# qiaozhijian/LPD-Net-Pytorch

Hardware: AMD Instinct MI355X
Metric: global descriptors/sec (4096-pt clouds) (higher is better)
Workload: dtype f32; 1 GPU; BASELINE configs[1]: LPD-Net (featnet=lpdnet, emb_dims=1024, no T-Nets) eval forward, N=4096, k=20, eval_batch_size=32 clouds/step/GPU; num_points=4096, batches_in_flight=2, parallelism=shard-by-cloud x1 (one process per GPU, no data-path collective)

## Files before the change

### include/lpd_hip.h

```cpp
#ifndef LPD_HIP_H
#define LPD_HIP_H

#include <stdint.h>

#ifdef __cplusplus
extern "C" {
#endif

#define LPD_OK 0
#define LPD_ERR_ARG (-1)
#define LPD_ERR_LAUNCH (-2)
#define LPD_ERR_UNSUPPORTED (-3)

#define LPD_ACT_NONE 0
#define LPD_ACT_RELU 1
#define LPD_ACT_LEAKY 2
#define LPD_ACT_SIGMOID 3

int lpd_version(void);
const char* lpd_last_error(void);
long long lpd_stat_ws_bytes(void);

int lpd_knn(const float* x, int B, int C, int N, int k, int32_t* idx, float* ws, int impl, void* stream);
long long lpd_knn_workspace_floats(int B, int C, int N, int k);
int lpd_knn_pm(const float* x_pm, int ld, int B, int C, int N, int k, int32_t* idx, float* ws, int impl, void* stream);
#define LPD_KNN_PM_PREPARED 256
int lpd_knn_pm_layout(int B, int C, int N, int k, float* ws, float** xx, float** xp, void** xb, float** tiles);

int lpd_lpdnet_front(const float* xyz, int ldx, const float* W1, const float* s1, const float* b1, const float* W2, const float* s2,
                     const float* b2, int act, float slope, float* F0, int B, int N, int k, float* knn_ws, void* stream);

int lpd_gemm(const float* A, const float* B, float* C, int M, int N, int K, int lda, int ldb, int ldc,
             int a_kmajor, int b_kmajor, int batch, long long sA, long long sB, long long sC, int splits,
             float* splitk_ws, const float* bias, const float* scale, const float* shift, int act, float slope,
             int accumulate, long long a_cloud, long long c_cloud, int panel_n, int panel_ld, void* stream);

int lpd_gemm_bf16x3(const float* A, const float* B, float* C, int M, int N, int K, int lda, int ldb, int ldc,
             int a_kmajor, int b_kmajor, int batch, long long sA, long long sB, long long sC, int splits,
             float* splitk_ws, const float* bias, const float* scale, const float* shift, int act, float slope,
             int accumulate, long long a_cloud, long long c_cloud, int panel_n, int panel_ld, void* stream);

int lpd_gemm_bf16x1(const float* A, const float* B, float* C, int M, int N, int K, int lda, int ldb, int ldc,
             int a_kmajor, int b_kmajor, int batch, long long sA, long long sB, long long sC, int splits,
             float* splitk_ws, const float* bias, const float* scale, const float* shift, int act, float slope,
             int accumulate, long long a_cloud, long long c_cloud, int panel_n, int panel_ld, void* stream);

long long lpd_gemm_prep_b_bytes(int N, int K);
int lpd_gemm_prep_b(const float* B, int ldb, int b_kmajor, int N, int K, void* frags, void* stream);
int lpd_gemm_prep_b_batch(const float* B, int ldb, int b_kmajor, int N, int K, int batch, long long sB, void* frags, void* stream);
int lpd_gemm_x3w(const float* A, int lda, const void* frags, float* C, int ldc, int M, int N, int K, const float* bias,
                 const float* scale, const float* shift, int act, float slope, int accumulate,
                 long long a_cloud, long long c_cloud, int panel_n, int panel_ld, int impl, void* stream);

int lpd_gemm_x3w_batched(const void* A, int lda, int a_bf16, const void* frags, long long frag_bytes, int batch_rows, float* C, int ldc, int M,
                         int N, int K, const float* a_scale, const float* a_shift, int a_act, float a_slope, int impl, void* stream);
int lpd_gemm_x3w_bf16a(const void* A16, int lda, const void* frags, float* C, int ldc, int M, int N, int K, int accumulate, int impl, void* stream);
int lpd_gemm_x3w_stats(const float* A, int lda, const void* frags, void* C, int ldc, int c_bf16, int M, int N, int K, const float* bias,
                       double* stat_sum, double* stat_sumsq, int impl, double* stat_ws, void* stream);
int lpd_gemm_x3w_act(const void* A, int lda, const void* frags, float* C, int ldc, int M, int N, int K, const float* bias,
                     const float* a_scale, const float* a_shift, int a_act, float a_slope, void* a_out, int a_ld, int flags, int impl, void* stream);

int lpd_gemm_x3t_applies(int M, int N, int K, int act, long long a_cloud, long long c_cloud, int panel_n);
int lpd_gemm_x3ts(const void* a_hi, long long a_lo, const void* frags, float* C, int M, int N, int K, const float* bias,
                  const float* scale, const float* shift, int act, float slope, long long a_cloud, long long c_cloud, int panel_n,
                  int panel_ld, void* stream);
int lpd_gemm_x3t_rows_applies(int M, int N, int K, int act, long long lda, long long ldc);
int lpd_gemm_x3t_rows(const float* A, long long lda, const void* frags, void* C, long long ldc, int c_bf16, int M, int N, int K, const float* bias,
                      const float* scale, const float* shift, int act, float slope, int batch, long long sA, long long sC,
                      long long frag_bytes, void* stream);

int lpd_gemm_x3t(const float* A, const void* frags, float* C, int M, int N, int K, const float* bias, const float* scale,
                 const float* shift, int act, float slope, long long a_cloud, long long c_cloud, int panel_n, int panel_ld,
                 void* stream);

int lpd_edge_gather_max(const float* P, int ldp, const float* Q, int ldq, const int32_t* idx, float* out, int ldo,
                        const float* scale, const float* shift, int M, int N, int C, int k, int act, float slope,
                        void* stream);

int lpd_edge_gather_max16(const float* P, int ldp, const float* Q, int ldq, const uint16_t* idx16, float* out, int ldo,
                          const float* scale, const float* shift, int M, int N, int C, int k, int act, float slope, long long p_cloud,
                          long long q_cloud, long long o_cloud, int panel_ld, void* stream);
int lpd_edge_gather_max16s(const float* P, int ldp, const float* Q, int ldq, const uint16_t* idx16, void* out_hi, long long o_lo,
                           const float* scale, const float* shift, int M, int N, int C, int k, int act, float slope, long long p_cloud,
                           long long q_cloud, long long o_cloud, int panel_ld, void* stream);

int lpd_pack_idx16(const int32_t* idx, uint16_t* idx16, long long M, int k, void* stream);

int lpd_pack_idx16w(const int32_t* idx, uint16_t* idx16, long long M, int k, int N, void* stream);
int lpd_edge_gather_maxw(const float* P, int ldp, const float* Q, int ldq, const uint16_t* idx16, float* out, int ldo,
                         const float* scale, const float* shift, int M, int N, int C, int k, int act, float slope, long long p_cloud,
                         long long q_cloud, long long o_cloud, int panel_ld, void* stream);

int lpd_edge_mlp(const float* P, int ldp, const float* Q, int ldq, const int32_t* idx, const float* s1,
                 const float* b1, const float* W2, const float* s2, const float* b2, float* out, int ldo, int M,
                 int N, int CM, int CO, int k, int act, float slope, long long out_cloud, int panel_ld, void* stream);
int lpd_edge_mlp_bf16x3(const float* P, int ldp, const float* Q, int ldq, const int32_t* idx, const float* s1,
                 const float* b1, const float* W2, const float* s2, const float* b2, float* out, int ldo, int M,
                 int N, int CM, int CO, int k, int act, float slope, long long out_cloud, int panel_ld, void* stream);
int lpd_edge_mlp_bf16x3s(const float* P, int ldp, const float* Q, int ldq, const int32_t* idx, const float* s1,
                 const float* b1, const float* W2, const float* s2, const float* b2, void* out_hi, long long out_lo, int M,
                 int N, int CM, int CO, int k, int act, float slope, long long out_cloud, int panel_ld, void* stream);
int lpd_edge_mlp_x1_bf16x3s(const float* P, int ldp, const float* Q, int ldq, const int32_t* idx, const float* s1,
                 const float* b1, const float* W2, const float* s2, const float* b2, void* out_hi, void* x1_hi, long long out_lo,
                 int M, int N, int k, int act, float slope, long long out_cloud, int panel_ld, void* stream);

int lpd_linear_smallk(const float* X, int ldx, const float* W, int w_sn, int w_sk, long long w_sb, int rows_per_w,
                      float* Y, int ldy, int M, int N, int K, const float* bias, const float* scale,
                      const float* shift, int act, float slope, void* stream);

int lpd_transpose(const float* in, float* out, int batch, int R, int C, int ldi, int ldo, long long si,
                  long long so, void* stream);

int lpd_softmax_affine(const float* in, float* out, int rows, int ncols, const float* scale, const float* shift,
                       int group_rows, float* colsum, int colsum_ld, float* part, void* stream);

int lpd_vlad_finalize(const float* vraw, const float* act, const float* cw2, float* out, float* ws, float* part, float* aux_asum,
                      float* aux_inv_c, float* aux_inv_g, int B, int N, int F, int KC, int asum_ready, void* stream);

int lpd_colmax(const float* in, int ldi, float* out, int B, int N, int C, void* stream);

int lpd_gating(const float* h, int ldh, const float* Wg, int ldw, const float* bias, const float* scale, const float* shift,
               float* out, int ldo, int B, int D, void* stream);

int lpd_mul(const float* a, const float* b, float* out, long long n, void* stream);

int lpd_metric_loss(const float* q, long long q_sb, const float* pos, long long pos_sb, long long pos_st,
                    const float* neg, long long neg_sb, long long neg_st, const float* other, long long other_sb,
                    int bq, int P, int Ng, int D, float m1, float m2, int use_min, int lazy, int ignore_zero, int quad,
                    float* loss, float* minmax, float* gq, float* gpos, float* gneg, float* gother, void* stream);

int lpd_best_pos_bwd(const float* q, long long q_sb, const float* pos, long long pos_sb, long long pos_st, const float* gmin,
                     const float* gmax, int bq, int P, int D, float* gq, float* gpos, void* stream);

int lpd_retrieval_topk(const float* S, const float* Q, int ldq, const float* D, int ldd, int nq, int ndb, int dim, int k,
                       int32_t* idx, float* dist, float* ws, void* stream);

int lpd_recall_pairs(const float* Q, int ldq, const float* D, int ldd, int dim, const int32_t* q_off, const int32_t* d_off, int rd,
                     int q_rows, int d_rows, const int32_t* pairs, const int32_t* out_off, int npairs, int max_qtiles,
                     const int32_t* truth_off, const int32_t* truth_idx, int k, int32_t* first, uint8_t* one_pct, float* top1_sim,
                     int32_t* topk_idx, int32_t* hist, int32_t* n_eval, int32_t* n_onepct, float* ws, void* stream);

int lpd_hard_negatives(const float* table, long long ldt, const float* Q, long long ldq, const int32_t* cand, int bq, int nc, int dim,
                       int k, int32_t* pos, float* dist, void* stream);

int lpd_f64_to_f32(const double* in, float* out, long long n, void* stream);

int lpd_morton_sort(const float* xyz, float* out, int32_t* perm, int B, int N, void* stream);

int lpd_local_features(const float* xyz, int ldx, const int32_t* idx, int B, int N, int K, const int32_t* cand, int ncand, unsigned sel,
                       int copy_xyz, float* out, int ldo, int32_t* kopt, void* stream);

int lpd_make_submaps(const float* points, int ld, const int32_t* offsets, int B, int N, int normalize, float* out, int32_t* info,
                     float* xform, int32_t* counts, void* stream);

int lpd_sample_items(const int32_t* off, const int32_t* idx, int n_lists, int nnz, int T, const int32_t* lists, int L, const int32_t* extra,
                     int X, int R, int invert, int m, unsigned long long seed, int32_t* out, int32_t* count, void* stream);
int lpd_gather_tuples(const float* table, int T, int N, const int32_t* items, int B, const float* rot, float sigma, float clip,
                      unsigned long long seed, float* out, void* stream);

int lpd_radius_count(const double* qpos, int Q, const double* dpos, int D, const int32_t* seg_off, int S, double r, const int32_t* skip_seg,
                     const int32_t* self_item, int32_t* counts, void* stream);
int lpd_radius_fill(const double* qpos, int Q, const double* dpos, int D, const int32_t* seg_off, int S, double r, const int32_t* skip_seg,
                    const int32_t* self_item, const int32_t* row_off, int32_t* idx, int nnz, void* stream);

#define LPD_CLEAN_CHUNK 1024
typedef struct LpdCleanParams {
    float r_min, r_max, z_lo, z_hi, seed_z_lo, seed_z_hi, tau, min_det, max_slope, clearance;
    int32_t H, min_inliers, refine;
    uint32_t seed_lo, seed_hi;
    int32_t reserved;
} LpdCleanParams;
long long lpd_road_planes_workspace_bytes(int B, int H);
int lpd_road_planes(const float* points, int ld, int rows, const int32_t* offsets, int B, int max_len, const LpdCleanParams* prm,
                    float* plane, int32_t* info, void* ws, void* stream);
int lpd_clean_count(const float* points, int ld, int rows, const int32_t* offsets, int B, int max_len, const LpdCleanParams* prm,
                    const float* plane, const int32_t* info, int32_t* counts, void* stream);
int lpd_clean_fill(const float* points, int ld, int rows, const int32_t* offsets, int B, int max_len, const LpdCleanParams* prm,
                   const float* plane, const int32_t* info, const int32_t* block_off, float* out, int32_t* out_offsets,
                   unsigned char* mask, void* stream);


int lpd_colstats(const float* X, long long ld, long long R, int C, double* sum, double* sumsq, double* stat_ws, void* stream);

int lpd_bn_finalize(const double* sum, const double* sumsq, double count, int C, const float* gamma, const float* beta,
                    float* running_mean, float* running_var, float momentum, float eps, float* scale, float* shift,
                    float* mean, float* invstd, void* stream);

int lpd_affine_act(const float* X, long long ldx, float* Y, long long ldy, long long R, int C, const float* scale,
                   const float* shift, int act, float slope, void* stream);
int lpd_affine_act2(const float* X, long long ldx, float* Y, long long ldy, void* Y16, long long ld16, long long R, int C, const float* scale,
                    const float* shift, int act, float slope, void* stream);

int lpd_bn_act_bwd(const float* dY, long long lddy, const float* X, long long ldx, float* dX, long long lddx, long long R,
                   int C, const float* scale, const float* shift, const float* mean, const float* invstd, int act,
                   float slope, int has_bn, double* dbeta, double* dgamma, double* stat_ws, void* stream);
int lpd_bn_act_bwd_bf16(const void* dY, long long lddy, const void* X, long long ldx, void* dX, long long lddx, long long R, int C,
                        const float* scale, const float* shift, const float* mean, const float* invstd, int act, float slope, int has_bn,
                        double* dbeta, double* dgamma, double* stat_ws, void* stream);

int lpd_edge_build(const float* P, long long ldp, const float* Q, long long ldq, const int32_t* idx, float* U, long long M,
                   int N, int C, int k, double* sum, double* sumsq, double* stat_ws, void* stream);

int lpd_group_max(const float* X, long long ldx, int k, const float* scale, const float* shift, int act, float slope,
                  float* out, long long ldo, uint8_t* arg, long long M, int C, void* stream);
int lpd_group_max_sel(const float* X, long long ldx, int k, const float* scale, const float* shift, int act, float slope,
                      float* out, long long ldo, uint8_t* arg, float* xsel, long long ldsel, long long M, int C, void* stream);

int lpd_group_max_bwd(const float* dOut, long long ldo, const uint8_t* arg, int k, float* dX, long long M, int C,
                      int accumulate, void* stream);

int lpd_edge_bn_bwd(const float* dOut, long long ldo, const uint8_t* arg, const float* dDense, const float* X, float* dX,
                    float* dQ, long long ldq, int k, long long M, int C, const float* scale, const float* shift,
                    const float* mean, const float* invstd, int act, float slope, float inv_ns, double* dbeta, double* dgamma,
                    double* stat_ws, void* stream);
int lpd_edge_bn_bwd_sel(const float* dOut, long long ldo, const uint8_t* arg, const float* X, const float* Xsel, long long ldsel,
                        float* dX, int k, long long M, int C, const float* scale, const float* shift, const float* mean,
                        const float* invstd, int act, float slope, double* dbeta, double* dgamma, double* stat_ws, void* stream);

int lpd_group_sum(const float* dU, int k, float* dQ, long long ldq, long long M, int C, void* stream);

int lpd_scatter_add_rows(const float* dU, const int32_t* idx, float* dP, long long ldp, long long M, int N, int k, int C,
                         void* stream);

int lpd_graph_transpose(const int32_t* idx, long long M, int N, int k, int32_t* rowptr, int32_t* edges, int32_t* ws,
                        void* stream);
int lpd_gather_sum_rows(const float* dU, const int32_t* rowptr, const int32_t* edges, float* dP, long long ldp, long long M,
                        int C, int accumulate, void* stream);

int lpd_dw_smallk(const float* dY, long long lddy, const float* X, long long ldx, long long M, int Co, int Kin, float* dW,
                  void* stream);

int lpd_colmax_arg(const float* in, long long ld, float* out, int32_t* arg, int B, int N, int C, void* stream);

int lpd_colmax_bwd(const float* dOut, const int32_t* arg, float* dIn, long long ld, int B, int N, int C, void* stream);

int lpd_cloud_outer(const float* X, long long ldx, const float* dY, long long ldy, float* dT, int B, int N, int KD, void* stream);

int lpd_softmax_bwd(const float* A, const float* dA, const float* dasum, float* dS, long long rows, int ncols,
                    int rows_per_cloud, void* stream);

int lpd_vlad_finalize_bwd(const float* dOut, const float* v, const float* inv_c, const float* inv_g, const float* asum,
                          const float* cw2, float* dVraw, float* dasum, float* dcw2, int B, int F, int KC, void* stream);


int lpd_edge_split_fwd(const float* P, long long ldp, const float* Q, long long ldq, const int32_t* idx, const float* gamma,
                       float* S, float* usel, uint8_t* arg, long long M, int N, int C, int k, double* sum, double* sumsq,
                       double* stat_ws, void* stream);
int lpd_edge_mlp_train(const float* P, int ldp, const float* Q, int ldq, const int32_t* idx, const float* s1, const float* b1,
                       const float* W2, const float* gamma2, void* Y1e, void* Z, int bf16, int z_bf16, float* zsel, int ldsel, uint8_t* arg2,
                       double* sum, double* sumsq, int M, int N, int k, int act, float slope, double* stat_ws, void* stream);
int lpd_edge_mlp_train_bwd(const void* Z, const uint8_t* arg2, const void* dpre2, const float* W2, const float* scale2, const float* mean2,
                           const float* invstd2, const double* dbeta2, const double* dgamma2, const void* Y1e, const uint8_t* arg1,
                           const float* dx1, int lddx1, const float* beta1, const float* rgamma1, int bf16, int z_bf16, void* G, float* gsum,
                           double* dbeta1, double* dgamma1, int M, int k, int act, float slope, float inv_ns, float* kws, double* stat_ws, void* stream);
int lpd_edge_dense_bwd_apply(const void* G, int bf16, const float* gsum, const float* S, const float* P, long long ldp, const float* Q,
                             long long ldq, const int32_t* rowptr, const int32_t* edges, float* dP, long long lddp, float* dQ, long long lddq,
                             long long M, int C, int k, const float* scale, const float* mean, const float* invstd, const double* dbeta,
                             const double* dgamma, void* stream);
int lpd_edge_split_fwd16_applies(int N, int C, int k);
int lpd_edge_split_fwd16(const float* P, long long ldp, const float* Q, long long ldq, const uint16_t* idx16, const float* gamma, float* S,
                         float* usel, uint8_t* arg, long long M, int N, int C, int k, double* sum, double* sumsq, double* stat_ws, void* stream);

int lpd_edge_split_bwd(const float* dOut, long long ldo, const float* usel, const uint8_t* arg, const float* S, const float* P,
                       long long ldp, const float* Q, long long ldq, const int32_t* rowptr, const int32_t* edges, float* G,
                       float* dP, long long lddp, float* dQ, long long lddq, long long M, int C, int k, const float* scale,
                       const float* shift, const float* mean, const float* invstd, int act, float slope, int half, double* dbeta,
                       double* dgamma, double* stat_ws, void* stream);

int lpd_edge_build_bf16(const float* P, long long ldp, const float* Q, long long ldq, const int32_t* idx, uint16_t* U, long long M,
                        int N, int C, int k, double* sum, double* sumsq, double* stat_ws, void* stream);
int lpd_edge_act_max(const float* U, int k, const float* scale, const float* shift, int act, float slope, float* Y, float* out,
                     long long ldo, uint8_t* arg, long long M, int C, void* stream);
int lpd_edge_act_max_bf16(const uint16_t* U, int k, const float* scale, const float* shift, int act, float slope, uint16_t* Y,
                          float* out, long long ldo, uint8_t* arg, long long M, int C, void* stream);
int lpd_group_sel_stats_bf16(const uint16_t* Z, int k, const float* gamma, float* sel, long long lds, uint8_t* arg, long long M, int C,
                             double* sum, double* sumsq, double* stat_ws, void* stream);
int lpd_edge_bn_bwd_bf16(const float* dOut, long long ldo, const uint8_t* arg, const uint16_t* dDense, const uint16_t* X, uint16_t* dX,
                         float* dQ, long long ldq, int k, long long M, int C, const float* scale, const float* shift,
                         const float* mean, const float* invstd, int act, float slope, float inv_ns, double* dbeta, double* dgamma,
                         double* stat_ws, void* stream);
int lpd_edge_bn_bwd_bf16_sel(const float* dOut, long long ldo, const uint8_t* arg, const uint16_t* X, const float* Xsel, long long ldsel,
                             uint16_t* dX, int k, long long M, int C, const float* scale, const float* shift, const float* mean,
                             const float* invstd, int act, float slope, double* dbeta, double* dgamma, double* stat_ws, void* stream);
int lpd_bn_sel_bwd_reduce(const float* dOut, long long ldo, const float* Xsel, long long ldsel, long long M, int C, const float* scale,
                          const float* shift, const float* mean, const float* invstd, int act, float slope, uint16_t* dpre16,
                          double* dbeta, double* dgamma, double* stat_ws, void* stream);
long long lpd_edge_dw_sel_bf16_ws_bytes(long long E);
int lpd_edge_dw_sel_bf16(const uint16_t* Y, const uint8_t* arg, const uint16_t* dpre16, int k, long long M, const float* W2, long long ldw,
                         const float* scale, const float* mean, const float* invstd, const double* dbeta, const double* dgamma, float* dW2,
                         void* ws, void* stream);
int lpd_gemm_bf16s_bnbwd(const uint16_t* Z, const uint8_t* arg, const uint16_t* dpre16, int k, long long M, const float* W2, int ldw,
                         const float* scale, const float* mean, const float* invstd, const double* dbeta, const double* dgamma, uint16_t* dY,
                         void* stream);
int lpd_bn_sel_bwd_reduce_f32(const float* dOut, long long ldo, const float* Xsel, long long ldsel, long long M, int C, const float* scale,
                              const float* shift, const float* mean, const float* invstd, int act, float slope, float* dpre, double* dbeta,
                              double* dgamma, double* stat_ws, void* stream);
int lpd_edge_dw_sel_f32(const float* Y, const uint8_t* arg, const float* dpre, int k, long long M, const float* W2, long long ldw,
                        const float* scale, const float* mean, const float* invstd, const double* dbeta, const double* dgamma, float* dW2,
                        void* ws, void* stream);
int lpd_gemm_f32s_bnbwd(const float* Z, const uint8_t* arg, const float* dpre, int k, long long M, const float* W2, int ldw,
// ... 32 lines not shown
```

### lpd-net-pytorch_amd/csrc/lpd_knn.hip

```cpp
#include "lpd_common.h"
#include <math.h>
#include <type_traits>

namespace {

constexpr int KNN_WAVES = 4;
constexpr int KNN_THREADS = KNN_WAVES * 64;
constexpr int KNN_QPB = KNN_WAVES * 32;

template <int CP>
struct KnnCfg {
    static constexpr int CHUNK = (CP <= 32) ? 128 : (CP <= 64 ? 64 : 32);
    static constexpr int ROWS = 2 * CP;
    static constexpr int FLOATS = ROWS * CHUNK;
    static constexpr int PER_THREAD = FLOATS / KNN_THREADS;
};

__global__ void knn_sumsq_kernel(const float* __restrict__ x, float* __restrict__ xx, int C, int N)
{
    int n = blockIdx.x * blockDim.x + threadIdx.x;
    int b = blockIdx.y;
    if (n >= N) return;
    const float* p = x + (size_t)b * C * N + n;
    float total = 0.0f;
// ... 955 lines not shown
#define KNN_SUB_(n)  "v_sub_co_u32_e64 %[t], %[m" #n "], %[xl" #n "], %[yl" #n "]\n\t"
#define KNN_SBB_(n)  "v_subb_co_u32_e64 %[t], %[m" #n "], %[xh" #n "], %[yh" #n "], %[m" #n "]\n\t"
#define KNN_SELX_(n) "v_cndmask_b32_e64 %[nl" #n "], %[xl" #n "], %[yl" #n "], %[m" #n "]\n\t" \
                     "v_cndmask_b32_e64 %[nh" #n "], %[xh" #n "], %[yh" #n "], %[m" #n "]\n\t"
#define KNN_SELY_(n) "v_cndmask_b32_e64 %[yl" #n "], %[yl" #n "], %[xl" #n "], %[m" #n "]\n\t" \
                     "v_cndmask_b32_e64 %[yh" #n "], %[yh" #n "], %[xh" #n "], %[m" #n "]\n\t"
#define KNN_SELM_(n) "v_cndmask_b32_e64 %[xl" #n "], %[xl" #n "], %[yl" #n "], %[m" #n "]\n\t" \
                     "v_cndmask_b32_e64 %[xh" #n "], %[xh" #n "], %[yh" #n "], %[m" #n "]\n\t"
#define KNN_CXOUT_(n) [nl##n] "=&v"(nl##n), [nh##n] "=&v"(nh##n), [yl##n] "+v"(yl##n), [yh##n] "+v"(yh##n), [m##n] "=&s"(m##n)
#define KNN_CXIN_(n)  [xl##n] "v"(xl##n), [xh##n] "v"(xh##n)
#define KNN_MXOUT_(n) [xl##n] "+v"(xl##n), [xh##n] "+v"(xh##n), [m##n] "=&s"(m##n)
#define KNN_MXIN_(n)  [yl##n] "v"(yl##n), [yh##n] "v"(yh##n)
#define KNN_KEYREF_(n) unsigned &xh##n, unsigned &xl##n, unsigned &yh##n, unsigned &yl##n

__device__ __forceinline__ void knn_cx3(KNN_KEYREF_(0), KNN_KEYREF_(1), KNN_KEYREF_(2))
{
    unsigned long long m0, m1, m2;
    unsigned t, nl0, nh0, nl1, nh1, nl2, nh2;
    asm(KNN_SUB_(0) KNN_SUB_(1) KNN_SUB_(2) KNN_SBB_(0) KNN_SBB_(1) KNN_SBB_(2)
        KNN_SELX_(0) KNN_SELY_(0) KNN_SELX_(1) KNN_SELY_(1) KNN_SELX_(2) KNN_SELY_(2)
        : KNN_CXOUT_(0), KNN_CXOUT_(1), KNN_CXOUT_(2), [t] "=&v"(t)
        : KNN_CXIN_(0), KNN_CXIN_(1), KNN_CXIN_(2));
    xl0 = nl0; xh0 = nh0; xl1 = nl1; xh1 = nh1; xl2 = nl2; xh2 = nh2;
}
__device__ __forceinline__ void knn_cx2(KNN_KEYREF_(0), KNN_KEYREF_(1))
{
    unsigned long long m0, m1;
    unsigned t, nl0, nh0, nl1, nh1;
    asm(KNN_SUB_(0) KNN_SUB_(1) "s_nop 0\n\t" KNN_SBB_(0) KNN_SBB_(1) "s_nop 0\n\t"
        KNN_SELX_(0) KNN_SELY_(0) KNN_SELX_(1) KNN_SELY_(1)
        : KNN_CXOUT_(0), KNN_CXOUT_(1), [t] "=&v"(t)
        : KNN_CXIN_(0), KNN_CXIN_(1));
    xl0 = nl0; xh0 = nh0; xl1 = nl1; xh1 = nh1;
}
__device__ __forceinline__ void knn_cx1(KNN_KEYREF_(0))
{
    unsigned long long m0;
    unsigned t, nl0, nh0;
    asm(KNN_SUB_(0) "s_nop 1\n\t" KNN_SBB_(0) "s_nop 1\n\t" KNN_SELX_(0) KNN_SELY_(0)
        : KNN_CXOUT_(0), [t] "=&v"(t)
        : KNN_CXIN_(0));
    xl0 = nl0; xh0 = nh0;
}
__device__ __forceinline__ void knn_mx3(KNN_KEYREF_(0), KNN_KEYREF_(1), KNN_KEYREF_(2))
{
    unsigned long long m0, m1, m2;
    unsigned t;
    asm(KNN_SUB_(0) KNN_SUB_(1) KNN_SUB_(2) KNN_SBB_(0) KNN_SBB_(1) KNN_SBB_(2) KNN_SELM_(0) KNN_SELM_(1) KNN_SELM_(2)
        : KNN_MXOUT_(0), KNN_MXOUT_(1), KNN_MXOUT_(2), [t] "=&v"(t)
        : KNN_MXIN_(0), KNN_MXIN_(1), KNN_MXIN_(2));
}
__device__ __forceinline__ void knn_mx2(KNN_KEYREF_(0), KNN_KEYREF_(1))
{
    unsigned long long m0, m1;
    unsigned t;
    asm(KNN_SUB_(0) KNN_SUB_(1) "s_nop 0\n\t" KNN_SBB_(0) KNN_SBB_(1) "s_nop 0\n\t" KNN_SELM_(0) KNN_SELM_(1)
        : KNN_MXOUT_(0), KNN_MXOUT_(1), [t] "=&v"(t)
        : KNN_MXIN_(0), KNN_MXIN_(1));
}
__device__ __forceinline__ void knn_mx1(KNN_KEYREF_(0))
{
    unsigned long long m0;
    unsigned t;
    asm(KNN_SUB_(0) "s_nop 1\n\t" KNN_SBB_(0) "s_nop 1\n\t" KNN_SELM_(0)
        : KNN_MXOUT_(0), [t] "=&v"(t)
        : KNN_MXIN_(0));
}
#define KNN_K_(a, i) a##h[i], a##l[i]
#define KNN_CX3(a, i, b, j, c, k, d, l, e, m, f, n) knn_cx3(KNN_K_(a, i), KNN_K_(b, j), KNN_K_(c, k), KNN_K_(d, l), KNN_K_(e, m), KNN_K_(f, n))
#define KNN_CX2(a, i, b, j, c, k, d, l) knn_cx2(KNN_K_(a, i), KNN_K_(b, j), KNN_K_(c, k), KNN_K_(d, l))
#define KNN_CX1(a, i, b, j) knn_cx1(KNN_K_(a, i), KNN_K_(b, j))
#define KNN_MX3(a, i, b, j, c, k, d, l, e, m, f, n) knn_mx3(KNN_K_(a, i), KNN_K_(b, j), KNN_K_(c, k), KNN_K_(d, l), KNN_K_(e, m), KNN_K_(f, n))
#define KNN_MX2(a, i, b, j, c, k, d, l) knn_mx2(KNN_K_(a, i), KNN_K_(b, j), KNN_K_(c, k), KNN_K_(d, l))
#define KNN_MX1(a, i, b, j) knn_mx1(KNN_K_(a, i), KNN_K_(b, j))
#define KNN_PLACE(...) { constexpr int pl[20] = {__VA_ARGS__}; unsigned th[20], tl[20]; \
    _Pragma("unroll") for (int s = 0; s < 20; ++s) { th[s] = kh[pl[s]]; tl[s] = kl[pl[s]]; } \
    _Pragma("unroll") for (int s = 0; s < 20; ++s) { kh[s] = th[s]; kl[s] = tl[s]; } }

template <int NB> __device__ __forceinline__ void knn_merge_batch(unsigned (&kh)[20], unsigned (&kl)[20], unsigned (&bh)[NB], unsigned (&bl)[NB]);
template <> __device__ __forceinline__ void knn_merge_batch<8>(unsigned (&kh)[20], unsigned (&kl)[20], unsigned (&bh)[8], unsigned (&bl)[8])
{
    KNN_CX3(b, 0, b, 1,  b, 2, b, 3,  b, 4, b, 5);
    KNN_CX3(b, 6, b, 7,  b, 0, b, 2,  b, 1, b, 3);
    KNN_CX3(b, 4, b, 6,  b, 5, b, 7,  b, 1, b, 2);
    KNN_CX3(b, 5, b, 6,  b, 0, b, 4,  b, 3, b, 7);
    KNN_CX2(b, 1, b, 5,  b, 2, b, 6);
    KNN_CX2(b, 2, b, 4,  b, 3, b, 5);
    KNN_CX3(b, 1, b, 2,  b, 3, b, 4,  b, 5, b, 6);
    KNN_MX3(k, 12, b, 7,  k, 13, b, 6,  k, 14, b, 5);
    KNN_MX3(k, 15, b, 4,  k, 16, b, 3,  k, 17, b, 2);
    KNN_MX2(k, 18, b, 1,  k, 19, b, 0);
    KNN_CX3(k, 0, k, 16,  k, 1, k, 17,  k, 2, k, 18);
    KNN_CX3(k, 3, k, 19,  k, 16, k, 8,  k, 17, k, 9);
    KNN_CX3(k, 18, k, 10,  k, 19, k, 11,  k, 4, k, 12);
    KNN_CX3(k, 5, k, 13,  k, 6, k, 14,  k, 7, k, 15);
    KNN_CX3(k, 16, k, 4,  k, 17, k, 5,  k, 18, k, 6);
    KNN_CX3(k, 19, k, 7,  k, 8, k, 12,  k, 9, k, 13);
    KNN_CX3(k, 10, k, 14,  k, 11, k, 15,  k, 0, k, 2);
    KNN_CX3(k, 1, k, 3,  k, 16, k, 18,  k, 17, k, 19);
    KNN_CX3(k, 4, k, 6,  k, 5, k, 7,  k, 8, k, 10);
    KNN_CX3(k, 9, k, 11,  k, 12, k, 14,  k, 13, k, 15);
    KNN_CX3(k, 0, k, 1,  k, 2, k, 3,  k, 16, k, 17);
    KNN_CX3(k, 18, k, 19,  k, 4, k, 5,  k, 6, k, 7);
    KNN_CX3(k, 8, k, 9,  k, 10, k, 11,  k, 12, k, 13);
    KNN_CX1(k, 14, k, 15);
    KNN_PLACE(0, 1, 2, 3, 16, 17, 18, 19, 4, 5, 6, 7, 8, 9, 10, 11, 12, 13, 14, 15);
}
template <> __device__ __forceinline__ void knn_merge_batch<16>(unsigned (&kh)[20], unsigned (&kl)[20], unsigned (&bh)[16], unsigned (&bl)[16])
{
    KNN_CX3(b, 0, b, 1,  b, 2, b, 3,  b, 4, b, 5);
    KNN_CX3(b, 6, b, 7,  b, 8, b, 9,  b, 10, b, 11);
    KNN_CX3(b, 12, b, 13,  b, 14, b, 15,  b, 0, b, 2);
    KNN_CX3(b, 1, b, 3,  b, 4, b, 6,  b, 5, b, 7);
    KNN_CX3(b, 8, b, 10,  b, 9, b, 11,  b, 12, b, 14);
    KNN_CX3(b, 13, b, 15,  b, 1, b, 2,  b, 5, b, 6);
    KNN_CX3(b, 9, b, 10,  b, 13, b, 14,  b, 0, b, 4);
    KNN_CX3(b, 1, b, 5,  b, 2, b, 6,  b, 3, b, 7);
    KNN_CX3(b, 8, b, 12,  b, 9, b, 13,  b, 10, b, 14);
    KNN_CX3(b, 11, b, 15,  b, 2, b, 4,  b, 3, b, 5);
    KNN_CX3(b, 10, b, 12,  b, 11, b, 13,  b, 1, b, 2);
    KNN_CX3(b, 3, b, 4,  b, 5, b, 6,  b, 9, b, 10);
    KNN_CX3(b, 11, b, 12,  b, 13, b, 14,  b, 0, b, 8);
    KNN_CX3(b, 1, b, 9,  b, 2, b, 10,  b, 3, b, 11);
    KNN_CX3(b, 4, b, 12,  b, 5, b, 13,  b, 6, b, 14);
    KNN_CX3(b, 7, b, 15,  b, 4, b, 8,  b, 5, b, 9);
    KNN_CX3(b, 6, b, 10,  b, 7, b, 11,  b, 2, b, 4);
    KNN_CX3(b, 3, b, 5,  b, 6, b, 8,  b, 7, b, 9);
    KNN_CX3(b, 10, b, 12,  b, 11, b, 13,  b, 1, b, 2);
    KNN_CX3(b, 3, b, 4,  b, 5, b, 6,  b, 7, b, 8);
    KNN_CX3(b, 9, b, 10,  b, 11, b, 12,  b, 13, b, 14);
    KNN_MX3(k, 4, b, 15,  k, 5, b, 14,  k, 6, b, 13);
    KNN_MX3(k, 7, b, 12,  k, 8, b, 11,  k, 9, b, 10);
    KNN_MX3(k, 10, b, 9,  k, 11, b, 8,  k, 12, b, 7);
    KNN_MX3(k, 13, b, 6,  k, 14, b, 5,  k, 15, b, 4);
    KNN_MX3(k, 16, b, 3,  k, 17, b, 2,  k, 18, b, 1);
    KNN_MX1(k, 19, b, 0);
    KNN_CX3(k, 0, k, 16,  k, 1, k, 17,  k, 2, k, 18);
    KNN_CX3(k, 3, k, 19,  k, 16, k, 8,  k, 17, k, 9);
    KNN_CX3(k, 18, k, 10,  k, 19, k, 11,  k, 4, k, 12);
    KNN_CX3(k, 5, k, 13,  k, 6, k, 14,  k, 7, k, 15);
    KNN_CX3(k, 16, k, 4,  k, 17, k, 5,  k, 18, k, 6);
    KNN_CX3(k, 19, k, 7,  k, 8, k, 12,  k, 9, k, 13);
    KNN_CX3(k, 10, k, 14,  k, 11, k, 15,  k, 0, k, 2);
    KNN_CX3(k, 1, k, 3,  k, 16, k, 18,  k, 17, k, 19);
    KNN_CX3(k, 4, k, 6,  k, 5, k, 7,  k, 8, k, 10);
    KNN_CX3(k, 9, k, 11,  k, 12, k, 14,  k, 13, k, 15);
    KNN_CX3(k, 0, k, 1,  k, 2, k, 3,  k, 16, k, 17);
    KNN_CX3(k, 18, k, 19,  k, 4, k, 5,  k, 6, k, 7);
    KNN_CX3(k, 8, k, 9,  k, 10, k, 11,  k, 12, k, 13);
    KNN_CX1(k, 14, k, 15);
    KNN_PLACE(0, 1, 2, 3, 16, 17, 18, 19, 4, 5, 6, 7, 8, 9, 10, 11, 12, 13, 14, 15);
}

template <int CP, int KMAX, int WAVES, bool ONFLY, bool FULLT = false, int SPLIT = 1>
__global__ __launch_bounds__(WAVES * SPLIT * 64, ((SPLIT > 1 && CP == 2) ? 3 : Knn7Cfg<CP, KMAX, ONFLY>::WAVES_PER_SIMD)) void knn7_kernel(const float* __restrict__ xp, const float* __restrict__ xx,
                                                             const float* __restrict__ cenp, const float* __restrict__ cnorm,
                                                             const float* __restrict__ rad, const float* __restrict__ txmax,
                                                             int32_t* __restrict__ idx, const int32_t* __restrict__ order,
                                                             int N, int k, int nt, int C, int blocks_per_cloud, int dbg,
                                                             const uint16_t* __restrict__ ubq)
{
    extern __shared__ __attribute__((aligned(16))) unsigned char smem7[];
    if constexpr (FULLT) dbg = 0;
    const int tid = threadIdx.x;
    const int lane = tid & 63;
    const int wave = __builtin_amdgcn_readfirstlane(tid >> 6);
    const int h = lane >> 5;
    const int col = lane & 31;
    int vb = lpd_xcd_remap(blockIdx.x, gridDim.x);
    if (order) vb = order[vb];
    const int b = vb / blocks_per_cloud;
    const int qb = vb - b * blocks_per_cloud;
    static_assert(SPLIT == 1 || (WAVES == 1 && FULLT && KMAX <= 20 && !(ONFLY && CP == 32)), "SPLIT: whole tiles, short lists, bounds from the LDS table or from centroids");
    const int sw = SPLIT > 1 ? wave : 0;
    const int q0 = SPLIT > 1 ? qb * 32 : qb * (WAVES * 32) + wave * 32;
    const int W = q0 >> 5;
    const bool wave_ok = q0 < N;
    const int q = q0 + col;
    const bool q_ok = q < N;
    const float* xpb = xp + (size_t)b * N * (2 * CP);
    const float* xxb = xx + (size_t)b * N;
    const float* cenb = cenp + (size_t)b * nt * (2 * CP);
    const float* cnb = cnorm + (size_t)b * nt;
    const float* radb = rad + (size_t)b * nt;
    const bool vec_ok = (N & 3) == 0;
    const bool vec_ok_t = (nt & 3) == 0;
    using L = Knn7Cfg<CP, KMAX, ONFLY>;
    static_assert(CP != 2 || ONFLY, "three coordinates: bounds on the fly");
    uint16_t* ubt = reinterpret_cast<uint16_t*>(smem7 + (SPLIT > 1 ? (size_t)0 : (size_t)wave * L::WAVE));
    unsigned char* qreg_base = SPLIT > 1 ? smem7 + L::TBYTES + (size_t)wave * L::QBYTES : smem7 + (size_t)wave * L::WAVE + L::QOFF;
    float2* myq = reinterpret_cast<float2*>(qreg_base) + lane;
    volatile float* thr_sh = reinterpret_cast<volatile float*>(smem7 + L::TBYTES + (size_t)SPLIT * L::QBYTES);
    static_assert(SPLIT == 1 || L::QBYTES >= 64 * KMAX * 8, "SPLIT: a wave's queue region holds its two half-lists for the merge");
    if constexpr (SPLIT > 1) {
        thr_sh[(sw * 2 + 0) * 64 + lane] = -INFINITY;
        thr_sh[(sw * 2 + 1) * 64 + lane] = -INFINITY;
    }

    float qreg[CP];
    knn3_ld_ops<CP>(xpb, N, q, h, qreg);
    const float xq = xxb[min(q, N - 1)];

    float smax = 0.f;
    for (int t = lane; t < nt; t += 64) smax = fmaxf(smax, txmax[(size_t)b * nt + t]);
#pragma unroll
    for (int m = 32; m >= 1; m >>= 1) smax = fmaxf(smax, __shfl_xor(smax, m, 64));
    const float E0 = 8.0f * (float)(C + 8) * 1.1920929e-7f * smax + 1e-30f;
    float4 qc3 = make_float4(0.f, 0.f, 0.f, 0.f);
    if constexpr (CP == 2) qc3 = *reinterpret_cast<const float4*>(xpb + (size_t)min(q, N - 1) * 4);

    float a[CP];
    float4 x4[4];
    float pd[16];

    if (wave_ok && !ONFLY && ubq) {
        const uint16_t* src = ubq + ((size_t)b * nt + W) * nt * 32;
        for (int e = (SPLIT > 1 ? tid : lane) * 8; e < nt * 32; e += SPLIT * 64 * 8)
            *reinterpret_cast<uint4*>(ubt + e) = *reinterpret_cast<const uint4*>(src + e);
    }
    if (wave_ok && !ONFLY && !ubq) {
        const int nct = (nt + 31) / 32;
        for (int ct = sw; ct < nct; ct += SPLIT) {
            float4 r4[4];
            knn3_ld_ops<CP>(cenb, nt, ct * 32 + col, h, a);
            knn3_ld_xx(cnb, nt, ct * 32, h, vec_ok_t, x4);
            knn3_ld_xx(radb, nt, ct * 32, h, vec_ok_t, r4);
            knn3_tile<CP>(a, x4, qreg, xq, cenb, cnb, nt, 0, false, col, h, vec_ok_t, pd);
#pragma unroll
            for (int r = 0; r < 16; ++r) {
                const int T = ct * 32 + (r & 3) + 8 * (r >> 2) + 4 * h;
                const float4 rv = r4[r >> 2];
                const float rT = (r & 3) == 0 ? rv.x : (r & 3) == 1 ? rv.y : (r & 3) == 2 ? rv.z : rv.w;
                const float dq = sqrtf(fmaxf(-pd[r] - E0, 0.0f)) * 0.99999f;
                const float lb = fmaxf(dq - rT, 0.0f);
                const float ub = -(lb * lb) * 0.99999f + E0;
                uint32_t bits = __float_as_uint(ub);
                bits = (ub <= 0.0f) ? (bits >> 16) : 0x7f80u;
                if (T < nt) ubt[T * 32 + col] = (uint16_t)bits;
            }
        }
    }

    if constexpr (SPLIT > 1) __syncthreads();

    float lv[KMAX];
    int li[KMAX];
#pragma unroll
    for (int s = 0; s < KMAX; ++s) {
        lv[s] = -INFINITY;
        li[s] = 0x7fffffff;
    }
    constexpr bool BATCHED = KMAX <= 20;
    constexpr int NB = CP == 2 ? 8 : 16;
    static_assert(!BATCHED || KMAX == 20, "the generated networks merge into a list of 20");
    unsigned kh[20], kl[20];
#pragma unroll
    for (int s = 0; s < 20; ++s) { kh[s] = KNN_IMG_EMPTY; kl[s] = KNN_LOW_EMPTY; }
    bool drained = false;
    float t3v = -INFINITY;
    float thrv = q_ok ? -INFINITY : INFINITY;
    int cnt = 0;
    constexpr int M3 = (KMAX + 2 * SPLIT - 1) / (2 * SPLIT);
    auto refresh = [&]() {
        if constexpr (SPLIT > 1) {
            float best = thr_sh[(sw * 2 + 0) * 64 + lane];
            const float t3 = t3v;
            float m3 = fminf(t3, __shfl_xor(t3, 32, 64));
#pragma unroll
            for (int o = 1; o < SPLIT; ++o) {
                const int s2 = (sw + o) % SPLIT;
                best = fmaxf(best, thr_sh[(s2 * 2 + 0) * 64 + lane]);
                m3 = fminf(m3, fminf(thr_sh[(s2 * 2 + 1) * 64 + lane], thr_sh[(s2 * 2 + 1) * 64 + (lane ^ 32)]));
            }
            thrv = q_ok ? fmaxf(best, m3) : INFINITY;
        }
    };
    int stat_tiles = 0, stat_it = 0, stat_adm = 0, stat_drains = 0, stat_fn = 0, stat_pass = 0;

    int spos = 0;
    int vcount = 0;
    auto find_next_walk = [&]() -> int {
        while (spos < 2 * nt) {
            const int T = (spos & 1) ? W + ((spos + 1) >> 1) : W - (spos >> 1);
            ++spos;
            if (T < 0 || T >= nt) continue;
            if constexpr (SPLIT > 1) {
                const bool mine = (vcount % SPLIT) == sw;
                ++vcount;
                if (!mine) continue;
            }
            if constexpr ((CP == 32) && !ONFLY && !FULLT) ++stat_fn;
            float ub;
            if constexpr (CP == 2) {
                const float4 cen = *reinterpret_cast<const float4*>(cenb + (size_t)T * 4);
                const float e0 = qc3.x - cen.x, e1 = qc3.y - cen.y, e2 = qc3.z - cen.z;
                const float d2 = fmaf(e2, e2, fmaf(e1, e1, e0 * e0));
                const float dq = sqrtf(fmaxf(d2 - E0, 0.0f)) * 0.99999f;
                const float lb = fmaxf(dq - radb[T], 0.0f);
                ub = -(lb * lb) * 0.99999f + E0;
            } else if constexpr (ONFLY) {
                if (ubq) {
                    ub = __uint_as_float((uint32_t)ubq[(((size_t)b * nt + W) * nt + T) * 32 + col] << 16);
                    if (__any(ub >= thrv)) return T;
                    continue;
                }
                const float* ct = cenb + (size_t)T * (2 * CP) + h * CP;
                float part = 0.0f;
#pragma unroll
                for (int g4 = 0; g4 < CP / 4; ++g4) {
                    const float4 cv = *reinterpret_cast<const float4*>(ct + 4 * g4);
                    const float e0 = qreg[4 * g4] - cv.x, e1 = qreg[4 * g4 + 1] - cv.y, e2 = qreg[4 * g4 + 2] - cv.z, e3 = qreg[4 * g4 + 3] - cv.w;
                    part = fmaf(e3, e3, fmaf(e2, e2, fmaf(e1, e1, fmaf(e0, e0, part))));
                }
// ... 178 lines not shown
            make_room();
            if (BATCHED || cur >= W) {
#pragma unroll
                for (int r = 0; r < 16; ++r) {
                    if (pd[r] >= thrv) {
                        const int row = (r & 3) + 8 * (r >> 2) + 4 * h;
                        myq[cnt * 64] = make_float2(pd[r], __int_as_float(cur * 32 + row));
                        ++cnt;
                    }
                }
            } else {
#pragma unroll
                for (int r = 15; r >= 0; --r) {
                    if (pd[r] >= thrv) {
                        const int row = (r & 3) + 8 * (r >> 2) + 4 * h;
                        myq[cnt * 64] = make_float2(pd[r], __int_as_float(cur * 32 + row));
                        ++cnt;
                    }
                }
            }
            if (TIMERS && dbg) { const long long t = tick(); tm_sel += t - tm0; tm0 = t; }
            if (__any(cnt > L::QCAP - 16) && !(LAZY && drained)) drain();
            if (TIMERS && dbg) { const long long t = tick(); tm_drain += t - tm0; tm0 = t; }
        }
        cur = nxt;
        if constexpr (TWO_AHEAD) {
            nxt = nxt2;
            nxt2 = nxt >= 0 ? find_next() : -1;
        } else nxt = cur >= 0 ? find_next() : -1;
        if (TIMERS && dbg) { const long long t = tick(); tm_adv += t - tm0; tm0 = t; }
    };
    if constexpr (TWO_AHEAD) {
        while (cur >= 0) {
            visit(a, x4);
            if (cur < 0) break;
            visit(a2, x42);
        }
    } else {
        while (cur >= 0) {
            if constexpr (!FULLT) ++stat_tiles;
            tm0 = tick();
            const int pf = nxt;
            knn3_tile<CP, FULLT>(a, x4, qreg, xq, xpb, xxb, N, (pf >= 0 ? pf : 0) * 32, pf >= 0, col, h, vec_ok, pd);
            float mx = fmaxf(fmaxf(fmaxf(pd[0], pd[1]), fmaxf(pd[2], pd[3])), fmaxf(fmaxf(pd[4], pd[5]), fmaxf(pd[6], pd[7])));
            mx = fmaxf(mx, fmaxf(fmaxf(fmaxf(pd[8], pd[9]), fmaxf(pd[10], pd[11])), fmaxf(fmaxf(pd[12], pd[13]), fmaxf(pd[14], pd[15]))));
            if (TIMERS && dbg) { const long long t = tick(); tm_tile += t - tm0; tm0 = t; }
            refresh();
            if (__any(mx >= thrv)) {
                make_room();
                if (BATCHED || cur >= W) {
    #pragma unroll
                    for (int r = 0; r < 16; ++r) {
                        if (pd[r] >= thrv) {
                            const int row = (r & 3) + 8 * (r >> 2) + 4 * h;
                            myq[cnt * 64] = make_float2(pd[r], __int_as_float(cur * 32 + row));
                            ++cnt;
                        }
                    }
                } else {
    #pragma unroll
                    for (int r = 15; r >= 0; --r) {
                        if (pd[r] >= thrv) {
                            const int row = (r & 3) + 8 * (r >> 2) + 4 * h;
                            myq[cnt * 64] = make_float2(pd[r], __int_as_float(cur * 32 + row));
                            ++cnt;
                        }
                    }
                }
                if (TIMERS && dbg) { const long long t = tick(); tm_sel += t - tm0; tm0 = t; }
                if (__any(cnt > L::QCAP - 16) && !(LAZY && drained)) drain();
                if (TIMERS && dbg) { const long long t = tick(); tm_drain += t - tm0; tm0 = t; }
            }
            cur = nxt;
            nxt = cur >= 0 ? find_next() : -1;
            if (TIMERS && dbg) { const long long t = tick(); tm_adv += t - tm0; tm0 = t; }
    }
    }
    tm0 = tick();
    drain();
    tm_drain += tick() - tm0;
    if constexpr (BATCHED) {
#pragma unroll
        for (int s = 0; s < KMAX; ++s) {
            lv[s] = knn_img_inv(kh[KMAX > 20 ? 0 : s]);
            li[s] = kh[KMAX > 20 ? 0 : s] == KNN_IMG_EMPTY ? 0x7fffffff : (int)~kl[KMAX > 20 ? 0 : s];
        }
    }
    if constexpr (KMAX == 64) {
        if (dbg && q_ok) {
            int32_t* o = idx + ((size_t)b * N + q) * k;
            if (h == 0) { o[0] = stat_tiles; o[1] = stat_it; o[2] = stat_adm; o[3] = stat_drains; }
            else o[4] = stat_adm;
            return;
        }
        knn_merge_halves_bitonic(lv, li);
        if (h == 0 && q_ok) {
            int32_t* out = idx + ((size_t)b * N + q) * k;
#pragma unroll
            for (int s = 0; s < 64; ++s)
                if (s < k) out[s] = li[s];
        }
        return;
    } else {
    float* mv = reinterpret_cast<float*>(SPLIT > 1 ? qreg_base : smem7 + (size_t)wave * L::WAVE);
    int* mi = reinterpret_cast<int*>(mv + 64 * KMAX);
#pragma unroll
    for (int s = 0; s < KMAX; ++s) {
        mv[lane * KMAX + s] = lv[s];
        mi[lane * KMAX + s] = li[s];
    }
    __syncthreads();
    if constexpr (SPLIT > 1) {
        {
            const float* av = mv + lane * KMAX;
            const int* ai = mi + lane * KMAX;
            const float* bv = mv + (lane ^ 32) * KMAX;
            const int* bi = mi + (lane ^ 32) * KMAX;
            int pa = 0, pb = 0;
#pragma unroll
            for (int s = 0; s < KMAX; ++s) {
                const float va = av[pa], vb2 = bv[pb];
                const int ia = ai[pa], ib = bi[pb];
                const bool take_a = knn_before(va, ia, vb2, ib);
                lv[s] = take_a ? va : vb2;
                li[s] = take_a ? ia : ib;
                pa += take_a ? 1 : 0;
                pb += take_a ? 0 : 1;
                pa = min(pa, KMAX - 1);
                pb = min(pb, KMAX - 1);
            }
        }
        float* gv = mv;
        int* gi = reinterpret_cast<int*>(gv + 32 * KMAX);
        if (h == 0) {
#pragma unroll
            for (int s = 0; s < KMAX; ++s) {
                gv[col * KMAX + s] = lv[s];
                gi[col * KMAX + s] = li[s];
            }
        }
        __syncthreads();
        if (wave == 0 && h == 0 && q_ok) {
            float hv[SPLIT];
            int hi[SPLIT], pos[SPLIT];
            const float* mbase = reinterpret_cast<const float*>(smem7 + L::TBYTES) + col * KMAX;
            constexpr int WSTRIDE = L::QBYTES / 4, IOFF = 32 * KMAX;
#pragma unroll
            for (int w2 = 0; w2 < SPLIT; ++w2) {
                hv[w2] = mbase[w2 * WSTRIDE];
                hi[w2] = __float_as_int(mbase[w2 * WSTRIDE + IOFF]);
                pos[w2] = 0;
            }
            int32_t* out = idx + ((size_t)b * N + q) * k;
            for (int s = 0; s < k; ++s) {
                int bw = 0;
                float bvv = hv[0];
                int bii = hi[0];
#pragma unroll
                for (int w2 = 1; w2 < SPLIT; ++w2) {
                    const bool better = knn_before(hv[w2], hi[w2], bvv, bii);
                    bw = better ? w2 : bw;
                    bvv = better ? hv[w2] : bvv;
                    bii = better ? hi[w2] : bii;
                }
                out[s] = bii;
#pragma unroll
                for (int w2 = 0; w2 < SPLIT; ++w2) {
                    if (bw == w2) {
                        pos[w2] += 1;
                        const bool more = pos[w2] < KMAX;
                        const int pp = pos[w2] < KMAX ? pos[w2] : KMAX - 1;
                        hv[w2] = more ? mbase[w2 * WSTRIDE + pp] : -INFINITY;
                        hi[w2] = more ? __float_as_int(mbase[w2 * WSTRIDE + IOFF + pp]) : 0x7fffffff;
                    }
                }
            }
        }
        return;
    }
    if (dbg && q_ok) {
        int32_t* o = idx + ((size_t)b * N + q) * k;
        if (h == 0) {
            o[0] = stat_tiles; o[1] = stat_it; o[2] = stat_adm; o[3] = stat_drains;
            if (k >= 12) { o[5] = stat_pass; o[6] = (int)tm_adv; o[7] = (int)tm_tile; o[8] = (int)tm_sel; o[9] = (int)tm_drain; o[10] = (int)(tick() - tm_start); o[11] = stat_fn; }
        } else o[4] = stat_adm;
    } else
    if (h == 0 && q_ok) {
        const float* av = mv + lane * KMAX;
        const int* ai = mi + lane * KMAX;
        const float* bv = mv + (lane + 32) * KMAX;
        const int* bi = mi + (lane + 32) * KMAX;
        int pa = 0, pb = 0;
        int32_t* out = idx + ((size_t)b * N + q) * k;
        for (int s = 0; s < k; ++s) {
            bool take_a;
            if (pa >= KMAX) take_a = false;
            else if (pb >= KMAX) take_a = true;
            else {
                const float va = av[pa], vb2 = bv[pb];
                take_a = (va > vb2) || (va == vb2 && ai[pa] < bi[pb]);
            }
            if (take_a) out[s] = ai[pa++];
            else out[s] = bi[pb++];
        }
    }
    }
}

template <int CP, int KMAX>
int knn3_launch(const float* x, const float* xx, int32_t* idx, int B, int C, int N, int k, hipStream_t stream, int dbg = 0)
{
    float* xp = const_cast<float*>(xx) + (size_t)B * N;
    if (x) {
        hipLaunchKernelGGL(knn_pack_kernel<CP>, dim3((N + 255) / 256, B), dim3(256), 0, stream, x, xp, C, N);
        LPD_CHECK_LAUNCH("lpd_knn(pack)");
    }
    size_t lds = (size_t)KNN3_WAVES * knn3_wave_floats<KMAX>() * sizeof(float);
    const int bpc = (N + KNN3_WAVES * 32 - 1) / (KNN3_WAVES * 32);
    auto kern = knn3_kernel<CP, KMAX>;
    (void)hipFuncSetAttribute((const void*)kern, hipFuncAttributeMaxDynamicSharedMemorySize, (int)lds);
    hipLaunchKernelGGL(kern, dim3(bpc * B), dim3(KNN3_THREADS), lds, stream, (const float*)xp, xx, idx, N, k, bpc, dbg);
    LPD_CHECK_LAUNCH("lpd_knn");
    return LPD_OK;
}

inline bool knn7_tight();
inline size_t knn7_extra_floats(int B, int N, int CP)
{
    const size_t nt = (size_t)(N + 31) / 32;
    size_t n = (size_t)B * nt * (2 * CP + 3 + 2) + 16;
    if (CP == 32 && nt <= (size_t)KNN7_PRE_MAXT && knn7_tight())
        n += (size_t)B * nt * 32 * (KNN7_XB / 2) + (size_t)B * nt * nt * 16 + 16;
    return n;
}

inline bool knn7_tight()
{
    static const bool tight = lpd_debug("knn-pre", 1) != 0;
    return tight;
}
inline __bf16* knn7_xb_of(const float* xx, int B, int N)
{
    const int nt = (N + 31) / 32;
    const float* txmax = xx + (size_t)B * N * (1 + 64) + (size_t)B * nt * (64 + 2);
    const int32_t* order = reinterpret_cast<const int32_t*>(txmax + (size_t)B * nt + 4) + (size_t)B * nt;
    const uintptr_t a0 = (reinterpret_cast<uintptr_t>(order + (size_t)nt * B + 4) + 15) & ~(uintptr_t)15;
    return reinterpret_cast<__bf16*>(a0);
}

template <int CP, int KMAX, bool ONFLY>
int knn7_launch(const float* x, const float* xx, int32_t* idx, int B, int C, int N, int k, hipStream_t stream, int dbg = 0, bool xb_ready = false,
                bool stats_ready = false)
{
    using L = Knn7Cfg<CP, KMAX, ONFLY>;
    static_assert(L::WAVE >= L::MERGE, "merge region must fit the wave's LDS region");
    const int nt = (N + 31) / 32;
    float* xp = const_cast<float*>(xx) + (size_t)B * N;
    float* cenp = xp + (size_t)B * N * 2 * CP;
    float* cnorm = cenp + (size_t)B * nt * 2 * CP;
    float* rad = cnorm + (size_t)B * nt;
    float* txmax = rad + (size_t)B * nt;
    if (x) hipLaunchKernelGGL(knn_pack_kernel<CP>, dim3((N + 255) / 256, B), dim3(256), 0, stream, x, xp, C, N);
    if (!stats_ready)
        hipLaunchKernelGGL(knn7_tile_stats_kernel<CP>, dim3(nt, B), dim3(64), 0, stream, (const float*)xp, xx, cenp, cnorm, rad, txmax, N, nt);
    LPD_CHECK_LAUNCH("lpd_knn(tile pre-pass)");
    constexpr int WAVES = 1;
    const int bpc = (N + WAVES * 32 - 1) / (WAVES * 32);
    static const bool lpt = lpd_debug("knn-order", 1) != 0;
    int32_t* pred = reinterpret_cast<int32_t*>(txmax + (size_t)B * nt + 4);
    int32_t* order = pred + (size_t)B * nt;
    const int nitems = bpc * B;
    uint16_t* ubq = nullptr;
    if constexpr (CP == 32) {
        if (knn7_tight() && nt <= KNN7_PRE_MAXT) {
            __bf16* xb = knn7_xb_of(xx, B, N);
            ubq = reinterpret_cast<uint16_t*>(xb + (size_t)B * nt * 32 * KNN7_XB);
            if (!xb_ready) hipLaunchKernelGGL(knn7_bf16_kernel, dim3((nt * 64 + 255) / 256, B), dim3(256), 0, stream, (const float*)xp, xx, xb, N, nt);
            const int bx = (nt + 4 * KNN7_BQT - 1) / (4 * KNN7_BQT);
            int zs = 1;
            while (zs < 8 && (long long)bx * B * zs < 512 && (nt + 2 * zs - 1) / (2 * zs) >= 8) zs *= 2;
            const int tchunk = (((nt + zs - 1) / zs) + 3) & ~3;
            hipLaunchKernelGGL(knn7_bound_kernel, dim3(bx, B, (nt + tchunk - 1) / tchunk), dim3(256), 0, stream, (const __bf16*)xb, xx,
                               (const float*)txmax, ubq, N, nt, C, tchunk);
            LPD_CHECK_LAUNCH("lpd_knn(low-precision bounds)");
        }
    }
    static const bool branchy = lpd_debug("knn-fullt", 1) == 0;
    constexpr int KNN7_SPLIT = 4;
    constexpr bool split_built = KMAX <= 20 && !(ONFLY && CP == 32);
    static const int split_env = lpd_debug("knn-split", -1);
    const int split_wps = CP == 2 ? 3 : L::WAVES_PER_SIMD;
    const bool split = split_built && N % 32 == 0 && !branchy && !dbg && split_env != 0 &&
                       (split_env == 1 || (long long)nitems * KNN7_SPLIT <= 1024ll * split_wps);
    const bool use_order = lpt && !(split && (long long)nitems * KNN7_SPLIT <= 1024ll * split_wps);
    if (use_order) {
        const size_t plds = ((size_t)nt * (2 * CP + 1) + nt) * sizeof(float);
        if (plds <= 65536) {
            auto pk = knn7_predict_lds_kernel<CP>;
            (void)hipFuncSetAttribute((const void*)pk, hipFuncAttributeMaxDynamicSharedMemorySize, (int)plds);
            hipLaunchKernelGGL(pk, dim3((nt + KNN7_PRED_WPB - 1) / KNN7_PRED_WPB, B), dim3(256), plds, stream, (const float*)cenp, (const float*)rad, pred, nt);
        } else
            hipLaunchKernelGGL(knn7_predict_kernel<CP>, dim3(nt, B), dim3(128), 0, stream, (const float*)cenp, (const float*)rad, pred, nt);
        hipLaunchKernelGGL(knn7_order_kernel, dim3((nitems / 8 + 1 + 1023) / 1024, 8), dim3(1024), 0, stream, (const int32_t*)pred, order, nitems);
        LPD_CHECK_LAUNCH("lpd_knn(launch order)");
    }
    {
        size_t lds = (size_t)WAVES * L::WAVE;
        int threads = WAVES * 64;
        auto go = [&](auto kern) {
            (void)hipFuncSetAttribute((const void*)kern, hipFuncAttributeMaxDynamicSharedMemorySize, (int)lds);
            hipLaunchKernelGGL(kern, dim3(bpc * B), dim3(threads), lds, stream, (const float*)xp, xx, (const float*)cenp,
                               (const float*)cnorm, (const float*)rad, (const float*)txmax, idx, (const int32_t*)(use_order ? order : nullptr),
                               N, k, nt, C, bpc, dbg, (const uint16_t*)ubq);
        };
        if constexpr (split_built) {
            if (split) {
                lds = (size_t)L::TBYTES + (size_t)KNN7_SPLIT * L::QBYTES + (size_t)KNN7_SPLIT * 2 * 64 * sizeof(float);
                threads = KNN7_SPLIT * 64;
                go(knn7_kernel<CP, KMAX, WAVES, ONFLY, true, KNN7_SPLIT>);
                LPD_CHECK_LAUNCH("lpd_knn(best-first, split)");
                return LPD_OK;
            }
        }
        if (N % 32 == 0 && !branchy && !dbg) go(knn7_kernel<CP, KMAX, WAVES, ONFLY, true>);
        else go(knn7_kernel<CP, KMAX, WAVES, ONFLY, false>);
        LPD_CHECK_LAUNCH("lpd_knn(best-first)");
    }
    return LPD_OK;
}

constexpr int KNN7_MAXN = 65536;
inline bool knn7_applies(int C, int N, int k) { return C <= 64 && k <= 64 && N <= KNN7_MAXN; }
inline int knn7_dispatch(const float* x, const float* xx, int32_t* idx, int B, int C, int N, int k, hipStream_t stream, int dbg, bool xb_ready = false,
                         bool stats_ready = false)
{
    const bool small = k <= 20 && N <= KNN7_MAXT * 32;
    if (C <= 4) return k <= 20 ? knn7_launch<2, 20, true>(x, xx, idx, B, C, N, k, stream, dbg) : knn7_launch<2, 64, true>(x, xx, idx, B, C, N, k, stream, dbg);
    if (small) return knn7_launch<32, 20, false>(x, xx, idx, B, C, N, k, stream, dbg, xb_ready, stats_ready);
    return k <= 20 ? knn7_launch<32, 20, true>(x, xx, idx, B, C, N, k, stream, dbg, xb_ready, stats_ready)
                   : knn7_launch<32, 64, true>(x, xx, idx, B, C, N, k, stream, dbg, xb_ready, stats_ready);
}

template <int CP>
int knn_dispatch_k(const float* x, const float* xx, int32_t* idx, int B, int C, int N, int k, int impl, hipStream_t stream);

template <int CP>
int knn3_dispatch_k(const float* x, const float* xx, int32_t* idx, int B, int C, int N, int k, hipStream_t stream)
{
    if (k <= 20) return knn3_launch<CP, 20>(x, xx, idx, B, C, N, k, stream);
    if (k <= 32) return knn3_launch<CP, 32>(x, xx, idx, B, C, N, k, stream);
    if (k <= 64) return knn3_launch<CP, 64>(x, xx, idx, B, C, N, k, stream);
    if (!x) { lpd_set_error("lpd_knn_pm: k=%d > 64 unsupported on the point-major entry", k); return LPD_ERR_UNSUPPORTED; }
    return knn_dispatch_k<CP>(x, xx, idx, B, C, N, k, 0, stream);
}

template <int CP, int KMAX>
int knn_launch(const float* x, const float* xx, int32_t* idx, int B, int C, int N, int k, int impl,
               hipStream_t stream)
{
    using Cfg = KnnCfg<CP>;
    size_t stage_bytes = (size_t)(2 * Cfg::FLOATS + 2 * Cfg::CHUNK) * sizeof(float);
    size_t merge_bytes = (size_t)KNN_WAVES * 2 * 32 * KMAX * sizeof(float);
    size_t lds = stage_bytes > merge_bytes ? stage_bytes : merge_bytes;
    dim3 grid((N + KNN_QPB - 1) / KNN_QPB, B);
    if (impl == 1) {
        if constexpr (KMAX == 20) {
            auto kern = knn_kernel<CP, KMAX, false>;
            (void)hipFuncSetAttribute((const void*)kern, hipFuncAttributeMaxDynamicSharedMemorySize, (int)lds);
            hipLaunchKernelGGL(kern, grid, dim3(KNN_THREADS), lds, stream, x, xx, idx, C, N, k);
        } else {
            lpd_set_error("lpd_knn: impl=1 (VALU cross-check) supports k <= 20 only");
            return LPD_ERR_UNSUPPORTED;
        }
    } else {
        auto kern = knn_kernel<CP, KMAX, true>;
        (void)hipFuncSetAttribute((const void*)kern, hipFuncAttributeMaxDynamicSharedMemorySize, (int)lds);
        hipLaunchKernelGGL(kern, grid, dim3(KNN_THREADS), lds, stream, x, xx, idx, C, N, k);
    }
    LPD_CHECK_LAUNCH("lpd_knn");
    return LPD_OK;
}

template <int CP>
int knn_dispatch_k(const float* x, const float* xx, int32_t* idx, int B, int C, int N, int k, int impl,
                   hipStream_t stream)
{
    if (k <= 20) return knn_launch<CP, 20>(x, xx, idx, B, C, N, k, impl, stream);
    if (k <= 32) return knn_launch<CP, 32>(x, xx, idx, B, C, N, k, impl, stream);
    if (k <= 64) return knn_launch<CP, 64>(x, xx, idx, B, C, N, k, impl, stream);
    lpd_set_error("lpd_knn: k=%d > 64 unsupported", k);
    return LPD_ERR_UNSUPPORTED;
}

}

extern "C" long long lpd_knn_workspace_floats(int B, int C, int N, int k)
{
    (void)k;
    if (B <= 0 || C <= 0 || N <= 0) return 0;
    const int cp = C <= 4 ? 2 : (C <= 64 ? 32 : 0);
    long long n = (long long)B * N * (1 + 2 * cp);
    if (cp) n += (long long)knn7_extra_floats(B, N, cp);
    return n;
}

extern "C" int lpd_knn(const float* x, int B, int C, int N, int k, int32_t* idx, float* xx_ws, int impl,
                       void* stream_)
{
    hipStream_t stream = (hipStream_t)stream_;
    LPD_CHECK_ARG(x && idx && xx_ws, "lpd_knn: null pointer");
    LPD_CHECK_ARG(B > 0 && C > 0 && N > 0, "lpd_knn: bad dims B=%d C=%d N=%d", B, C, N);
    LPD_CHECK_ARG(k > 0 && k <= N, "lpd_knn: need 0 < k <= N (k=%d N=%d)", k, N);
    LPD_CHECK_ARG(B <= 65535, "lpd_knn: B=%d exceeds grid.y", B);
    LPD_CHECK_ARG(impl == 0 || impl == 1 || impl == 2 || impl == 4 || impl == 5 || impl == 6, "lpd_knn: impl=%d (0 product; 4 / 6 force the ascending / best-first kernel; 5 statistics; 1 VALU cross-check; 2 first-generation kernel)", impl);
    hipLaunchKernelGGL(knn_sumsq_kernel, dim3((N + 255) / 256, B), dim3(256), 0, stream, x, xx_ws, C, N);
    LPD_CHECK_LAUNCH("lpd_knn(sumsq)");
    if (((impl == 0 && KNN7_DEFAULT) || (impl == 5 || impl == 6)) && knn7_applies(C, N, k))
        return knn7_dispatch(x, xx_ws, idx, B, C, N, k, stream, impl == 5);
    if (impl == 0 || impl == 4) {
        if (C <= 4) return knn3_dispatch_k<2>(x, xx_ws, idx, B, C, N, k, stream);
        if (C <= 64) return knn3_dispatch_k<32>(x, xx_ws, idx, B, C, N, k, stream);
        if (C <= 256) return knn_dispatch_k<128>(x, xx_ws, idx, B, C, N, k, 0, stream);
    } else {
        const int v1impl = impl == 1 ? 1 : 0;
        if (C <= 4) return knn_dispatch_k<2>(x, xx_ws, idx, B, C, N, k, v1impl, stream);
        if (C <= 64) return knn_dispatch_k<32>(x, xx_ws, idx, B, C, N, k, v1impl, stream);
        if (C <= 256) return knn_dispatch_k<128>(x, xx_ws, idx, B, C, N, k, v1impl, stream);
    }
    lpd_set_error("lpd_knn: C=%d > 256 unsupported", C);
    return LPD_ERR_UNSUPPORTED;
}

namespace {
inline bool knn_pm_wants_xb(int C, int N, int k, int impl)
{
    const bool best_first = ((impl == 0 && KNN7_DEFAULT) || (impl == 5 || impl == 6)) && knn7_applies(C, N, k);
    return best_first && C == 64 && knn7_tight() && N <= KNN7_PRE_MAXT * 32 && N % 32 == 0;
}
}

extern "C" int lpd_knn_pm_layout(int B, int C, int N, int k, float* ws, float** xx, float** xp, void** xb, float** tiles)
{
    LPD_CHECK_ARG(ws && xx && xp && xb && tiles && B > 0 && N > 0 && C > 0 && C <= 64, "lpd_knn_pm_layout: bad arguments");
    const int cp = C <= 4 ? 2 : 32;
    *xx = ws;
    *xp = ws + (size_t)B * N;
    *xb = (C == 64 && knn_pm_wants_xb(C, N, k, 0)) ? (void*)knn7_xb_of(ws, B, N) : nullptr;
    *tiles = (KNN7_DEFAULT && knn7_applies(C, N, k)) ? *xp + (size_t)B * N * 2 * cp : nullptr;
    return LPD_OK;
}

extern "C" int lpd_knn_pm(const float* x_pm, int ld, int B, int C, int N, int k, int32_t* idx, float* ws, int impl, void* stream_)
{
    hipStream_t stream = (hipStream_t)stream_;
    LPD_CHECK_ARG((x_pm || (impl & LPD_KNN_PM_PREPARED)) && idx && ws, "lpd_knn_pm: null pointer");
    LPD_CHECK_ARG(B > 0 && C > 0 && N > 0 && ld >= C, "lpd_knn_pm: bad dims B=%d C=%d N=%d ld=%d", B, C, N, ld);
    LPD_CHECK_ARG(k > 0 && k <= N, "lpd_knn_pm: need 0 < k <= N (k=%d N=%d)", k, N);
    LPD_CHECK_ARG(C <= 64 && k <= 64, "lpd_knn_pm: built for C <= 64, k <= 64 (got C=%d k=%d); use lpd_knn on the channel-major tensor", C, k);
    LPD_CHECK_ARG(C <= 4 || (impl & LPD_KNN_PM_PREPARED) || ((uintptr_t)x_pm & 15) == 0, "lpd_knn_pm: x_pm must be 16-byte aligned");
    const long long M = (long long)B * N;
    float* xp = ws + M;
    const bool prepped = (impl & LPD_KNN_PM_PREPARED) != 0;
    impl &= ~LPD_KNN_PM_PREPARED;
    LPD_CHECK_ARG(impl == 0 || impl == 4 || impl == 5 || impl == 6, "lpd_knn_pm: impl=%d (0 product; 4 / 6 force the ascending / best-first kernel; 5 statistics)", impl);
    const bool best_first = ((impl == 0 && KNN7_DEFAULT) || (impl == 5 || impl == 6)) && knn7_applies(C, N, k);
    const bool xb_ready = knn_pm_wants_xb(C, N, k, impl) && (prepped || ld % 4 == 0);
    LPD_CHECK_ARG(!prepped || C == 64, "lpd_knn_pm: prepared operands are a 64-channel affair (C=%d)", C);
    if (prepped) {  }
    else if (C <= 4) hipLaunchKernelGGL(knn_prep_pm_kernel<2>, dim3((unsigned)((M + 255) / 256)), dim3(256), 0, stream, x_pm, ld, ws, xp, C, M);
    else if (C == 64 && ld % 4 == 0) {
        hipLaunchKernelGGL(knn_prep_pm4_kernel, dim3((unsigned)((4 * M + 255) / 256)), dim3(256), 0, stream, x_pm, ld, ws, xp,
                           xb_ready ? knn7_xb_of(ws, B, N) : (__bf16*)nullptr, M, N, (N + 31) / 32);
    } else hipLaunchKernelGGL(knn_prep_pm_kernel<32>, dim3((unsigned)((M + 255) / 256)), dim3(256), 0, stream, x_pm, ld, ws, xp, C, M);
    LPD_CHECK_LAUNCH("lpd_knn_pm(prep)");
    if (best_first) return knn7_dispatch(nullptr, ws, idx, B, C, N, k, stream, impl == 5, xb_ready, prepped);
    if (C <= 4) return knn3_dispatch_k<2>(nullptr, ws, idx, B, C, N, k, stream);
    return knn3_dispatch_k<32>(nullptr, ws, idx, B, C, N, k, stream);
}
```

### lpd-net-pytorch_amd/csrc/lpd_morton.hip

```cpp
#include "lpd_common.h"
#include <math.h>

namespace {

__device__ __forceinline__ uint32_t spread10(uint32_t v)
{
    v &= 0x3ff;
    v = (v | (v << 16)) & 0x030000ff;
    v = (v | (v << 8)) & 0x0300f00f;
    v = (v | (v << 4)) & 0x030c30c3;
    v = (v | (v << 2)) & 0x09249249;
    return v;
}

__device__ __forceinline__ uint32_t bitonic_keep(uint32_t v, uint32_t o, bool lower, bool up)
{
    const uint32_t mn = v < o ? v : o, mx = v < o ? o : v;
    return (lower == up) ? mn : mx;
}

template <int E, int T = 1024>
__global__ __launch_bounds__(T) void morton_sort_kernel(const float* __restrict__ xyz, float* __restrict__ out,
                                                         int32_t* __restrict__ perm, int N)
{
    constexpr int NP = T * E;
    constexpr int IB = NP == 1024 ? 10 : NP == 2048 ? 11 : NP == 4096 ? 12 : NP == 8192 ? 13 : 14;
    static_assert(NP >= 1024 && NP <= 16384 && (NP & (NP - 1)) == 0, "1024 .. 16384 keys");
    extern __shared__ __attribute__((aligned(16))) uint32_t lds[];
    __shared__ float red[6][16];
    __shared__ float box[6];
    const int b = blockIdx.x, tid = threadIdx.x;
    const float* p = xyz + (size_t)b * N * 3;
    float mn[3] = {INFINITY, INFINITY, INFINITY}, mx[3] = {-INFINITY, -INFINITY, -INFINITY};
    for (int i = tid; i < N; i += T)
#pragma unroll
        for (int c = 0; c < 3; ++c) {
            float v = p[i * 3 + c];
            mn[c] = fminf(mn[c], v);
            mx[c] = fmaxf(mx[c], v);
        }
#pragma unroll
    for (int c = 0; c < 3; ++c) {
#pragma unroll
        for (int o = 32; o > 0; o >>= 1) {
            mn[c] = fminf(mn[c], __shfl_xor(mn[c], o, 64));
            mx[c] = fmaxf(mx[c], __shfl_xor(mx[c], o, 64));
        }
        if ((tid & 63) == 0) { red[c][tid >> 6] = mn[c]; red[3 + c][tid >> 6] = mx[c]; }
    }
    __syncthreads();
    if (tid < 3) {
        float a = red[tid][0], z = red[3 + tid][0];
        for (int w = 1; w < T / 64; ++w) { a = fminf(a, red[tid][w]); z = fmaxf(z, red[3 + tid][w]); }
        box[tid] = a;
        box[3 + tid] = z > a ? 1023.0f / (z - a) : 0.0f;
    }
    __syncthreads();
    uint32_t v[E];
#pragma unroll
    for (int e = 0; e < E; ++e) {
        const int i = tid * E + e;
        uint32_t word = 0xffffffffu;
        if (i < N) {
            uint32_t q[3];
#pragma unroll
            for (int c = 0; c < 3; ++c) {
                float t = (p[i * 3 + c] - box[c]) * box[3 + c];
                t = fminf(fmaxf(t, 0.0f), 1023.0f);
                q[c] = (uint32_t)t;
            }
            const uint32_t key = spread10(q[0]) | (spread10(q[1]) << 1) | (spread10(q[2]) << 2);
            word = ((key >> (IB - 2)) << IB) | (uint32_t)i;
        }
        v[e] = word;
    }
#pragma unroll
    for (int k = 2; k <= NP; k <<= 1) {
#pragma unroll
        for (int j = k >> 1; j > 0; j >>= 1) {
            if (j < E) {
#pragma unroll
                for (int e = 0; e < E; ++e)
                    if ((e & j) == 0) {
                        const bool up = ((tid * E + e) & k) == 0;
                        const uint32_t a = v[e], c = v[e | j];
                        const bool sw = (a > c) == up;
                        v[e] = sw ? c : a;
                        v[e | j] = sw ? a : c;
                    }
            } else if (j < 64 * E) {
                const int lj = j / E;
                const bool lower = (tid & lj) == 0;
#pragma unroll
                for (int e = 0; e < E; ++e)
                    v[e] = bitonic_keep(v[e], __shfl_xor(v[e], lj, 64), lower, ((tid * E + e) & k) == 0);
            } else {
                const int tj = j / E;
                const bool lower = (tid & tj) == 0;
#pragma unroll
                for (int e = 0; e < E; ++e) lds[e * T + tid] = v[e];
                __syncthreads();
#pragma unroll
                for (int e = 0; e < E; ++e)
                    v[e] = bitonic_keep(v[e], lds[e * T + (tid ^ tj)], lower, ((tid * E + e) & k) == 0);
                __syncthreads();
            }
        }
    }
    float* o = out + (size_t)b * N * 3;
#pragma unroll
    for (int e = 0; e < E; ++e) {
        const int r = tid * E + e;
        if (r < N) {
            const uint32_t src = v[e] & ((1u << IB) - 1u);
            o[r * 3 + 0] = p[src * 3 + 0];
            o[r * 3 + 1] = p[src * 3 + 1];
            o[r * 3 + 2] = p[src * 3 + 2];
            if (perm) perm[(size_t)b * N + r] = (int32_t)src;
        }
    }
}

template <int E, int T = 1024>
void morton_launch(const float* xyz, float* out, int32_t* perm, int B, int N, hipStream_t stream)
{
    const size_t lds = (size_t)E * T * sizeof(uint32_t);
    auto kern = morton_sort_kernel<E, T>;
    (void)hipFuncSetAttribute((const void*)kern, hipFuncAttributeMaxDynamicSharedMemorySize, (int)lds);
    hipLaunchKernelGGL(kern, dim3(B), dim3(T), lds, stream, xyz, out, perm, N);
}

}

extern "C" int lpd_morton_sort(const float* xyz, float* out, int32_t* perm, int B, int N, void* stream_)
{
    hipStream_t stream = (hipStream_t)stream_;
    LPD_CHECK_ARG(xyz && out && B > 0 && N > 0, "lpd_morton_sort: bad arguments");
    LPD_CHECK_ARG(xyz != out, "lpd_morton_sort: in-place reordering is not supported");
    if (N > 16384) {
        lpd_set_error("lpd_morton_sort: N=%d > 16384 unsupported", N);
        return LPD_ERR_UNSUPPORTED;
    }
    if (N <= 1024) morton_launch<1>(xyz, out, perm, B, N, stream);
    else if (N <= 2048) morton_launch<2>(xyz, out, perm, B, N, stream);
    else if (N <= 4096) morton_launch<4>(xyz, out, perm, B, N, stream);
    else if (N <= 8192) morton_launch<8>(xyz, out, perm, B, N, stream);
    else morton_launch<16>(xyz, out, perm, B, N, stream);
    LPD_CHECK_LAUNCH("lpd_morton_sort");
    return LPD_OK;
}
```

### lpd-net-pytorch_amd/lpdnet_hip/_lib.py

```python
import ctypes
import os

import torch

_HERE = os.path.dirname(os.path.abspath(__file__))
LIB_PATH = os.environ.get("LPD_HIP_LIB") or os.path.join(_HERE, "liblpd_hip.so")

_c_int = ctypes.c_int
_c_ll = ctypes.c_longlong
_c_f = ctypes.c_float
_c_p = ctypes.c_void_p

SIGNATURES = {
    "lpd_version": [],
    "lpd_last_error": [],
    "lpd_stat_ws_bytes": [],
    "lpd_knn": [_c_p, _c_int, _c_int, _c_int, _c_int, _c_p, _c_p, _c_int, _c_p],
    "lpd_gemm": [_c_p, _c_p, _c_p, _c_int, _c_int, _c_int, _c_int, _c_int, _c_int, _c_int, _c_int, _c_int,
                 _c_ll, _c_ll, _c_ll, _c_int, _c_p, _c_p, _c_p, _c_p, _c_int, _c_f, _c_int, _c_ll, _c_ll, _c_int, _c_int, _c_p],
"lpd_gemm_bf16x3": [_c_p, _c_p, _c_p, _c_int, _c_int, _c_int, _c_int, _c_int, _c_int, _c_int, _c_int, _c_int,
                 _c_ll, _c_ll, _c_ll, _c_int, _c_p, _c_p, _c_p, _c_p, _c_int, _c_f, _c_int, _c_ll, _c_ll, _c_int, _c_int, _c_p],
    "lpd_gemm_bf16x1": [_c_p, _c_p, _c_p, _c_int, _c_int, _c_int, _c_int, _c_int, _c_int, _c_int, _c_int, _c_int,
                 _c_ll, _c_ll, _c_ll, _c_int, _c_p, _c_p, _c_p, _c_p, _c_int, _c_f, _c_int, _c_ll, _c_ll, _c_int, _c_int, _c_p],
    "lpd_gemm_prep_b_bytes": [_c_int, _c_int],
    "lpd_gemm_prep_b": [_c_p, _c_int, _c_int, _c_int, _c_int, _c_p, _c_p],
    "lpd_gemm_prep_b_batch": [_c_p, _c_int, _c_int, _c_int, _c_int, _c_int, _c_ll, _c_p, _c_p],
    "lpd_gemm_x3t_applies": [_c_int, _c_int, _c_int, _c_int, _c_ll, _c_ll, _c_int],
    "lpd_gemm_x3t_rows_applies": [_c_int, _c_int, _c_int, _c_int, _c_ll, _c_ll],
    "lpd_gemm_x3t_rows": [_c_p, _c_ll, _c_p, _c_p, _c_ll, _c_int, _c_int, _c_int, _c_int, _c_p, _c_p, _c_p, _c_int, _c_f, _c_int, _c_ll, _c_ll, _c_ll,
                          _c_p],
    "lpd_gemm_x3t": [_c_p, _c_p, _c_p, _c_int, _c_int, _c_int, _c_p, _c_p, _c_p, _c_int, _c_f, _c_ll, _c_ll, _c_int, _c_int, _c_p],
    "lpd_gemm_x3w": [_c_p, _c_int, _c_p, _c_p, _c_int, _c_int, _c_int, _c_int, _c_p, _c_p, _c_p, _c_int, _c_f, _c_int,
                     _c_ll, _c_ll, _c_int, _c_int, _c_int, _c_p],
    "lpd_gemm_p8_applies": [_c_int, _c_int, _c_int, _c_int],
    "lpd_gemm_p8": [_c_p, _c_p, _c_ll, _c_int, _c_p, _c_p, _c_int, _c_ll, _c_int, _c_int, _c_int, _c_int, _c_int, _c_p,
                    _c_int, _c_f, _c_int, _c_p],
    "lpd_gemm_p8_fused": [_c_p, _c_p, _c_ll, _c_int, _c_p, _c_p, _c_int, _c_ll, _c_int, _c_int, _c_int, _c_int, _c_int, _c_p,
                          _c_int, _c_f, _c_p, _c_p, _c_ll, _c_p],
    "lpd_softmax_affine_parts": [_c_p, _c_int, _c_ll, _c_p, _c_int, _c_p, _c_p, _c_int, _c_p, _c_int, _c_p, _c_p],
    "lpd_split_panels": [_c_p, _c_ll, _c_int, _c_p, _c_p, _c_ll, _c_int, _c_int, _c_int, _c_int, _c_p],
    "lpd_gemm_x3w_batched": [_c_p, _c_int, _c_int, _c_p, _c_ll, _c_int, _c_p, _c_int, _c_int, _c_int, _c_int, _c_p, _c_p, _c_int, _c_f, _c_int, _c_p],
    "lpd_gemm_x3w_bf16a": [_c_p, _c_int, _c_p, _c_p, _c_int, _c_int, _c_int, _c_int, _c_int, _c_int, _c_p],
    "lpd_gemm_x3w_act": [_c_p, _c_int, _c_p, _c_p, _c_int, _c_int, _c_int, _c_int, _c_p, _c_p, _c_p, _c_int, _c_f, _c_p, _c_int, _c_int, _c_int, _c_p],
    "lpd_gemm_x3w_stats": [_c_p, _c_int, _c_p, _c_p, _c_int, _c_int, _c_int, _c_int, _c_int, _c_p, _c_p, _c_p, _c_int, _c_p, _c_p],
    "lpd_retrieval_topk": [_c_p, _c_p, _c_int, _c_p, _c_int, _c_int, _c_int, _c_int, _c_int, _c_p, _c_p, _c_p, _c_p],
    "lpd_recall_pairs": [_c_p, _c_int, _c_p, _c_int, _c_int, _c_p, _c_p, _c_int, _c_int, _c_int, _c_p, _c_p, _c_int, _c_int, _c_p, _c_p,
                         _c_int, _c_p, _c_p, _c_p, _c_p, _c_p, _c_p, _c_p, _c_p, _c_p],
    "lpd_f64_to_f32": [_c_p, _c_p, _c_ll, _c_p],
    "lpd_best_pos_bwd": [_c_p, _c_ll, _c_p, _c_ll, _c_ll, _c_p, _c_p, _c_int, _c_int, _c_int, _c_p, _c_p, _c_p],
    "lpd_hard_negatives": [_c_p, _c_ll, _c_p, _c_ll, _c_p, _c_int, _c_int, _c_int, _c_int, _c_p, _c_p, _c_p],
    "lpd_knn_pm_layout": [_c_int, _c_int, _c_int, _c_int, _c_p, _c_p, _c_p, _c_p, _c_p],
    "lpd_lpdnet_front": [_c_p, _c_int, _c_p, _c_p, _c_p, _c_p, _c_p, _c_p, _c_int, _c_f, _c_p, _c_int, _c_int, _c_int, _c_p, _c_p],
    "lpd_knn_pm": [_c_p, _c_int, _c_int, _c_int, _c_int, _c_int, _c_p, _c_p, _c_int, _c_p],
    "lpd_knn_workspace_floats": [_c_int, _c_int, _c_int, _c_int],
    "lpd_edge_gather_max": [_c_p, _c_int, _c_p, _c_int, _c_p, _c_p, _c_int, _c_p, _c_p, _c_int, _c_int, _c_int,
                            _c_int, _c_int, _c_f, _c_p],
    "lpd_edge_gather_max16": [_c_p, _c_int, _c_p, _c_int, _c_p, _c_p, _c_int, _c_p, _c_p, _c_int, _c_int, _c_int,
                              _c_int, _c_int, _c_f, _c_ll, _c_ll, _c_ll, _c_int, _c_p],
    "lpd_edge_gather_max16s": [_c_p, _c_int, _c_p, _c_int, _c_p, _c_p, _c_ll, _c_p, _c_p, _c_int, _c_int, _c_int,
                               _c_int, _c_int, _c_f, _c_ll, _c_ll, _c_ll, _c_int, _c_p],
    "lpd_edge_mlp_x1_bf16x3s": [_c_p, _c_int, _c_p, _c_int, _c_p, _c_p, _c_p, _c_p, _c_p, _c_p, _c_p, _c_p, _c_ll, _c_int, _c_int, _c_int, _c_int,
                                _c_f, _c_ll, _c_int, _c_p],
    "lpd_edge_mlp_bf16x3s": [_c_p, _c_int, _c_p, _c_int, _c_p, _c_p, _c_p, _c_p, _c_p, _c_p, _c_p, _c_ll, _c_int, _c_int,
                             _c_int, _c_int, _c_int, _c_int, _c_f, _c_ll, _c_int, _c_p],
    "lpd_gemm_x3ts": [_c_p, _c_ll, _c_p, _c_p, _c_int, _c_int, _c_int, _c_p, _c_p, _c_p, _c_int, _c_f, _c_ll, _c_ll, _c_int, _c_int, _c_p],
    "lpd_pack_idx16": [_c_p, _c_p, ctypes.c_longlong, _c_int, _c_p],
    "lpd_pack_idx16w": [_c_p, _c_p, ctypes.c_longlong, _c_int, _c_int, _c_p],
    "lpd_edge_gather_maxw": [_c_p, _c_int, _c_p, _c_int, _c_p, _c_p, _c_int, _c_p, _c_p, _c_int, _c_int, _c_int,
                             _c_int, _c_int, _c_f, _c_ll, _c_ll, _c_ll, _c_int, _c_p],
    "lpd_edge_mlp": [_c_p, _c_int, _c_p, _c_int, _c_p, _c_p, _c_p, _c_p, _c_p, _c_p, _c_p, _c_int, _c_int, _c_int,
                     _c_int, _c_int, _c_int, _c_int, _c_f, _c_ll, _c_int, _c_p],
    "lpd_edge_mlp_bf16x3": [_c_p, _c_int, _c_p, _c_int, _c_p, _c_p, _c_p, _c_p, _c_p, _c_p, _c_p, _c_int, _c_int, _c_int,
                     _c_int, _c_int, _c_int, _c_int, _c_f, _c_ll, _c_int, _c_p],
    "lpd_linear_smallk": [_c_p, _c_int, _c_p, _c_int, _c_int, _c_ll, _c_int, _c_p, _c_int, _c_int, _c_int, _c_int,
                          _c_p, _c_p, _c_p, _c_int, _c_f, _c_p],
    "lpd_transpose": [_c_p, _c_p, _c_int, _c_int, _c_int, _c_int, _c_int, _c_ll, _c_ll, _c_p],
    "lpd_softmax_affine": [_c_p, _c_p, _c_int, _c_int, _c_p, _c_p, _c_int, _c_p, _c_int, _c_p, _c_p],
    "lpd_vlad_finalize": [_c_p, _c_p, _c_p, _c_p, _c_p, _c_p, _c_p, _c_p, _c_p, _c_int, _c_int, _c_int, _c_int, _c_int, _c_p],
    "lpd_colmax": [_c_p, _c_int, _c_p, _c_int, _c_int, _c_int, _c_p],
    "lpd_mul": [_c_p, _c_p, _c_p, _c_ll, _c_p],
    "lpd_gating": [_c_p, _c_int, _c_p, _c_int, _c_p, _c_p, _c_p, _c_p, _c_int, _c_int, _c_int, _c_p],
    "lpd_morton_sort": [_c_p, _c_p, _c_p, _c_int, _c_int, _c_p],
    "lpd_local_features": [_c_p, _c_int, _c_p, _c_int, _c_int, _c_int, _c_p, _c_int, ctypes.c_uint, _c_int, _c_p, _c_int, _c_p, _c_p],
    "lpd_make_submaps": [_c_p, _c_int, _c_p, _c_int, _c_int, _c_int, _c_p, _c_p, _c_p, _c_p, _c_p],
    "lpd_sample_items": [_c_p, _c_p, _c_int, _c_int, _c_int, _c_p, _c_int, _c_p, _c_int, _c_int, _c_int, _c_int, ctypes.c_ulonglong, _c_p, _c_p,
                         _c_p],
    "lpd_gather_tuples": [_c_p, _c_int, _c_int, _c_p, _c_int, _c_p, _c_f, _c_f, ctypes.c_ulonglong, _c_p, _c_p],
    "lpd_radius_count": [_c_p, _c_int, _c_p, _c_int, _c_p, _c_int, ctypes.c_double, _c_p, _c_p, _c_p, _c_p],
    "lpd_radius_fill": [_c_p, _c_int, _c_p, _c_int, _c_p, _c_int, ctypes.c_double, _c_p, _c_p, _c_p, _c_p, _c_int, _c_p],
    "lpd_road_planes_workspace_bytes": [_c_int, _c_int],
    "lpd_road_planes": [_c_p, _c_int, _c_int, _c_p, _c_int, _c_int, _c_p, _c_p, _c_p, _c_p, _c_p],
    "lpd_clean_count": [_c_p, _c_int, _c_int, _c_p, _c_int, _c_int, _c_p, _c_p, _c_p, _c_p, _c_p],
    "lpd_clean_fill": [_c_p, _c_int, _c_int, _c_p, _c_int, _c_int, _c_p, _c_p, _c_p, _c_p, _c_p, _c_p, _c_p, _c_p],
    "lpd_colstats": [_c_p, _c_ll, _c_ll, _c_int, _c_p, _c_p, _c_p, _c_p],
    "lpd_bn_finalize": [_c_p, _c_p, ctypes.c_double, _c_int, _c_p, _c_p, _c_p, _c_p, _c_f, _c_f, _c_p, _c_p, _c_p, _c_p, _c_p],
    "lpd_affine_act": [_c_p, _c_ll, _c_p, _c_ll, _c_ll, _c_int, _c_p, _c_p, _c_int, _c_f, _c_p],
    "lpd_affine_act2": [_c_p, _c_ll, _c_p, _c_ll, _c_p, _c_ll, _c_ll, _c_int, _c_p, _c_p, _c_int, _c_f, _c_p],
    "lpd_bn_act_bwd": [_c_p, _c_ll, _c_p, _c_ll, _c_p, _c_ll, _c_ll, _c_int, _c_p, _c_p, _c_p, _c_p, _c_int, _c_f, _c_int,
                       _c_p, _c_p, _c_p, _c_p],
    "lpd_bn_act_bwd_bf16": [_c_p, _c_ll, _c_p, _c_ll, _c_p, _c_ll, _c_ll, _c_int, _c_p, _c_p, _c_p, _c_p, _c_int, _c_f, _c_int,
                       _c_p, _c_p, _c_p, _c_p],
    "lpd_edge_build": [_c_p, _c_ll, _c_p, _c_ll, _c_p, _c_p, _c_ll, _c_int, _c_int, _c_int, _c_p, _c_p, _c_p, _c_p],
    "lpd_group_max": [_c_p, _c_ll, _c_int, _c_p, _c_p, _c_int, _c_f, _c_p, _c_ll, _c_p, _c_ll, _c_int, _c_p],
    "lpd_group_max_sel": [_c_p, _c_ll, _c_int, _c_p, _c_p, _c_int, _c_f, _c_p, _c_ll, _c_p, _c_p, _c_ll, _c_ll, _c_int, _c_p],
    "lpd_edge_bn_bwd_sel": [_c_p, _c_ll, _c_p, _c_p, _c_p, _c_ll, _c_p, _c_int, _c_ll, _c_int, _c_p, _c_p, _c_p, _c_p, _c_int, _c_f,
                            _c_p, _c_p, _c_p, _c_p],
    "lpd_edge_bn_bwd_bf16_sel": [_c_p, _c_ll, _c_p, _c_p, _c_p, _c_ll, _c_p, _c_int, _c_ll, _c_int, _c_p, _c_p, _c_p, _c_p, _c_int, _c_f,
                                 _c_p, _c_p, _c_p, _c_p],
    "lpd_group_max_bwd": [_c_p, _c_ll, _c_p, _c_int, _c_p, _c_ll, _c_int, _c_int, _c_p],
    "lpd_edge_bn_bwd": [_c_p, _c_ll, _c_p, _c_p, _c_p, _c_p, _c_p, _c_ll, _c_int, _c_ll, _c_int, _c_p, _c_p, _c_p, _c_p, _c_int,
                        _c_f, _c_f, _c_p, _c_p, _c_p, _c_p],
    "lpd_edge_mlp_train_bwd": [_c_p, _c_p, _c_p, _c_p, _c_p, _c_p, _c_p, _c_p, _c_p, _c_p, _c_p, _c_p, _c_int, _c_p, _c_p, _c_int, _c_int, _c_p, _c_p,
                               _c_p, _c_p, _c_int, _c_int, _c_int, _c_f, _c_f, _c_p, _c_p, _c_p],
    "lpd_edge_dense_bwd_apply": [_c_p, _c_int, _c_p, _c_p, _c_p, _c_ll, _c_p, _c_ll, _c_p, _c_p, _c_p, _c_ll, _c_p, _c_ll, _c_ll, _c_int, _c_int,
                                 _c_p, _c_p, _c_p, _c_p, _c_p, _c_p],
    "lpd_edge_mlp_train": [_c_p, _c_int, _c_p, _c_int, _c_p, _c_p, _c_p, _c_p, _c_p, _c_p, _c_p, _c_int, _c_int, _c_p, _c_int, _c_p, _c_p, _c_p,
                           _c_int, _c_int, _c_int, _c_int, _c_f, _c_p, _c_p],
    "lpd_group_sum": [_c_p, _c_int, _c_p, _c_ll, _c_ll, _c_int, _c_p],
    "lpd_scatter_add_rows": [_c_p, _c_p, _c_p, _c_ll, _c_ll, _c_int, _c_int, _c_int, _c_p],
    "lpd_graph_transpose": [_c_p, _c_ll, _c_int, _c_int, _c_p, _c_p, _c_p, _c_p],
    "lpd_gather_sum_rows": [_c_p, _c_p, _c_p, _c_p, _c_ll, _c_ll, _c_int, _c_int, _c_p],
    "lpd_dw_smallk": [_c_p, _c_ll, _c_p, _c_ll, _c_ll, _c_int, _c_int, _c_p, _c_p],
    "lpd_colmax_arg": [_c_p, _c_ll, _c_p, _c_p, _c_int, _c_int, _c_int, _c_p],
    "lpd_colmax_bwd": [_c_p, _c_p, _c_p, _c_ll, _c_int, _c_int, _c_int, _c_p],
    "lpd_cloud_outer": [_c_p, _c_ll, _c_p, _c_ll, _c_p, _c_int, _c_int, _c_int, _c_p],
    "lpd_softmax_bwd": [_c_p, _c_p, _c_p, _c_p, _c_ll, _c_int, _c_int, _c_p],
    "lpd_vlad_finalize_bwd": [_c_p, _c_p, _c_p, _c_p, _c_p, _c_p, _c_p, _c_p, _c_p, _c_int, _c_int, _c_int, _c_p],
    "lpd_edge_split_fwd": [_c_p, _c_ll, _c_p, _c_ll, _c_p, _c_p, _c_p, _c_p, _c_p, _c_ll, _c_int, _c_int, _c_int, _c_p, _c_p, _c_p, _c_p],
    "lpd_edge_split_bwd": [_c_p, _c_ll, _c_p, _c_p, _c_p, _c_p, _c_ll, _c_p, _c_ll, _c_p, _c_p, _c_p, _c_p, _c_ll, _c_p, _c_ll, _c_ll,
                           _c_int, _c_int, _c_p, _c_p, _c_p, _c_p, _c_int, _c_f, _c_int, _c_p, _c_p, _c_p, _c_p],
    "lpd_edge_split_fwd16_applies": [_c_int, _c_int, _c_int],
    "lpd_edge_split_fwd16": [_c_p, _c_ll, _c_p, _c_ll, _c_p, _c_p, _c_p, _c_p, _c_p, _c_ll, _c_int, _c_int, _c_int, _c_p, _c_p, _c_p, _c_p],
    "lpd_edge_build_bf16": [_c_p, _c_ll, _c_p, _c_ll, _c_p, _c_p, _c_ll, _c_int, _c_int, _c_int, _c_p, _c_p, _c_p, _c_p],
    "lpd_edge_act_max": [_c_p, _c_int, _c_p, _c_p, _c_int, _c_f, _c_p, _c_p, _c_ll, _c_p, _c_ll, _c_int, _c_p],
    "lpd_edge_act_max_bf16": [_c_p, _c_int, _c_p, _c_p, _c_int, _c_f, _c_p, _c_p, _c_ll, _c_p, _c_ll, _c_int, _c_p],
    "lpd_group_sel_stats_bf16": [_c_p, _c_int, _c_p, _c_p, _c_ll, _c_p, _c_ll, _c_int, _c_p, _c_p, _c_p, _c_p],
    "lpd_edge_bn_bwd_bf16": [_c_p, _c_ll, _c_p, _c_p, _c_p, _c_p, _c_p, _c_ll, _c_int, _c_ll, _c_int, _c_p, _c_p, _c_p, _c_p, _c_int,
                             _c_f, _c_f, _c_p, _c_p, _c_p, _c_p],
    "lpd_bn_sel_bwd_reduce": [_c_p, _c_ll, _c_p, _c_ll, _c_ll, _c_int, _c_p, _c_p, _c_p, _c_p, _c_int, _c_f, _c_p, _c_p, _c_p, _c_p, _c_p],
    "lpd_edge_dw_sel_bf16": [_c_p, _c_p, _c_p, _c_int, _c_ll, _c_p, _c_ll, _c_p, _c_p, _c_p, _c_p, _c_p, _c_p, _c_p, _c_p],
    "lpd_gemm_bf16s_bnbwd": [_c_p, _c_p, _c_p, _c_int, _c_ll, _c_p, _c_int, _c_p, _c_p, _c_p, _c_p, _c_p, _c_p, _c_p],
    "lpd_bn_sel_bwd_reduce_f32": [_c_p, _c_ll, _c_p, _c_ll, _c_ll, _c_int, _c_p, _c_p, _c_p, _c_p, _c_int, _c_f, _c_p, _c_p, _c_p, _c_p, _c_p],
    "lpd_edge_dw_sel_f32": [_c_p, _c_p, _c_p, _c_int, _c_ll, _c_p, _c_ll, _c_p, _c_p, _c_p, _c_p, _c_p, _c_p, _c_p, _c_p],
    "lpd_gemm_f32s_bnbwd": [_c_p, _c_p, _c_p, _c_int, _c_ll, _c_p, _c_int, _c_p, _c_p, _c_p, _c_p, _c_p, _c_p, _c_p],
    "lpd_gather_sum_rows_bf16": [_c_p, _c_p, _c_p, _c_p, _c_ll, _c_ll, _c_int, _c_int, _c_p],
    "lpd_gemm_bf16s": [_c_p, _c_p, _c_int, _c_int, _c_p, _c_ll, _c_int, _c_int, _c_p],
    "lpd_gemm_tn_bf16_ws_floats": [_c_ll, _c_int, _c_int],
    "lpd_edge_dw_sel_bf16_ws_bytes": [_c_ll],
    "lpd_gemm_tn_bf16": [_c_p, _c_p, _c_p, _c_p, _c_ll, _c_int, _c_int, _c_p],
    "lpd_gemm_tn_ws_floats": [_c_ll, _c_int, _c_int, _c_int],
    "lpd_gemm_tn": [_c_p, _c_ll, _c_p, _c_ll, _c_p, _c_p, _c_ll, _c_int, _c_int, _c_int, _c_ll, _c_ll, _c_int, _c_p],
    "lpd_gemm_tn_act": [_c_p, _c_ll, _c_p, _c_ll, _c_p, _c_p, _c_ll, _c_int, _c_int, _c_int, _c_ll, _c_ll, _c_int, _c_p, _c_p, _c_int, _c_f, _c_p],
    "lpd_gemm_tn_act_ws_floats": [_c_ll, _c_int, _c_int, _c_int, _c_int],
    "lpd_metric_loss": [_c_p, _c_ll, _c_p, _c_ll, _c_ll, _c_p, _c_ll, _c_ll, _c_p, _c_ll, _c_int, _c_int, _c_int,
                        _c_int, _c_f, _c_f, _c_int, _c_int, _c_int, _c_int, _c_p, _c_p, _c_p, _c_p, _c_p, _c_p, _c_p],
}
_RESTYPES = {"lpd_last_error": ctypes.c_char_p, "lpd_stat_ws_bytes": ctypes.c_longlong, "lpd_knn_workspace_floats": ctypes.c_longlong,
             "lpd_gemm_prep_b_bytes": ctypes.c_longlong, "lpd_gemm_tn_bf16_ws_floats": ctypes.c_longlong, "lpd_gemm_tn_ws_floats": ctypes.c_longlong,
             "lpd_gemm_tn_act_ws_floats": ctypes.c_longlong,
             "lpd_edge_dw_sel_bf16_ws_bytes": ctypes.c_longlong, "lpd_road_planes_workspace_bytes": ctypes.c_longlong}

_lib = None


class LpdHipError(RuntimeError):
    pass


def load():
    global _lib
    if _lib is not None:
        return _lib
    if not os.path.exists(LIB_PATH):
        raise LpdHipError(
            f"{LIB_PATH} not found: the HIP extension is not built. Run `python -c 'import __graft_entry__ as g; "
            "g.build()'` at the repo root (needs hipcc). There is no CPU/PyTorch fallback for this path.")
    lib = ctypes.CDLL(LIB_PATH)
    for name, argtypes in SIGNATURES.items():
        fn = getattr(lib, name)
        fn.argtypes = argtypes
        fn.restype = _RESTYPES.get(name, ctypes.c_int)
    _lib = lib
    return lib


def check(rc, what):
    if rc != 0:
        msg = load().lpd_last_error()
        raise LpdHipError(f"{what} failed (rc={rc}): {msg.decode() if msg else '?'}")
```

### lpd-net-pytorch_amd/lpdnet_hip/engine.py

```python
import torch

from . import _debug, ops

LEAKY_SLOPE = 0.01

class _PerThread(__import__("threading").local):
    DEBUG_AUX = None
    MORTON_ORDER = None
    PIPELINED = False


_TLS = _PerThread()
_MORTON_DEFAULT = [True]


def _morton_order():
    v = _TLS.MORTON_ORDER
    return _MORTON_DEFAULT[0] if v is None else v


def _set_morton_order(v):
    th = __import__("threading")
    if th.current_thread() is th.main_thread():
        _MORTON_DEFAULT[0] = bool(v)
    _TLS.MORTON_ORDER = bool(v)


class _EngineModule(__import__("types").ModuleType):
    DEBUG_AUX = property(lambda self: _TLS.DEBUG_AUX, lambda self, v: setattr(_TLS, "DEBUG_AUX", v))
    MORTON_ORDER = property(lambda self: _morton_order(), lambda self, v: _set_morton_order(v))


__import__("sys").modules[__name__].__class__ = _EngineModule
MORTON_MAX_POINTS = 16384
EVAL_CHUNK = int(__import__("os").environ.get("LPD_EVAL_CHUNK", "32"))


def reorder_points(x, reorder=True):
    if reorder and _morton_order() and 64 <= x.shape[2] <= MORTON_MAX_POINTS:
        return ops.morton_sort(x)
    return x


_CACHES = __import__("weakref").WeakKeyDictionary()


def _cache_of(module):
    c = _CACHES.get(module)
    if c is None:
        c = _CACHES[module] = {}
    return c


def _cached(module, key, tensors, build, extra=None):
    sig = tuple((t.data_ptr(), t._version, t.device) for t in tensors) + (extra,)
    c = _cache_of(module)
    hit = c.get(key)
    if hit is not None and hit[0] == sig:
        if hit[2] is not None:
            ops.consumer_sync(hit[2], *(hit[1] if isinstance(hit[1], tuple) else (hit[1],)))
        return hit[1]
    with torch.no_grad():
        val = build()
    if isinstance(val, torch.Tensor):
        val._lpd_stable = True
    cuda = any(t.is_cuda for t in tensors)
    c[key] = (sig, val, ops.producer_mark() if cuda else None)
    return val


def bn_affine(bn):
    def build():
        scale = bn.weight / torch.sqrt(bn.running_var + bn.eps)
        shift = bn.bias - bn.running_mean * scale
        return scale.contiguous(), shift.contiguous()
    src = (bn.weight, bn.bias, bn.running_mean, bn.running_var)
    if bn.num_batches_tracked is not None:
        src = src + (bn.num_batches_tracked,)
    return _cached(bn, "affine", src, build, extra=bn.eps)


def _w2d(conv):
    w = conv.weight
    return w.reshape(w.shape[0], -1)


def split_edge_weight(seq, mode):
    conv = seq[0]

    def build():
        w = _w2d(conv)
        if mode == "nbr":
            return w.contiguous()
        c = w.shape[1] // 2
        if mode == "cat_nc":
            wn, wc = w[:, :c], w[:, c:]
        else:
            wn, wc = w[:, c:], w[:, :c] - w[:, c:]
        return torch.cat((wn, wc), dim=0).contiguous()
    return _cached(seq, "split_" + mode, (conv.weight,), build)


def conv3_folded(net):
    bn, conv = net.bn3_lpd, net.conv3_lpd
    src = (conv.weight, bn.weight, bn.bias, bn.running_mean, bn.running_var)
    if bn.num_batches_tracked is not None:
        src = src + (bn.num_batches_tracked,)
    return _cached(net, "conv3_folded", src, lambda: (_w2d(conv) * bn_affine(bn)[0].unsqueeze(1)).contiguous(), extra=bn.eps)


def _check_input(x, dims=3):
    if not isinstance(x, torch.Tensor) or x.dim() != 4 or x.shape[1] != 1 or x.shape[3] != dims:
        raise ValueError(f"expected input [B,1,N,{dims}], got {tuple(x.shape) if isinstance(x, torch.Tensor) else type(x)}")
    if not x.is_cuda:
        raise ops._lib.LpdHipError(
            f"input is on {x.device}: the LPD-Net HIP path runs on MI355X only (no CPU fallback)")
    return x.float().contiguous()


def _tnet_common(net, h, B, N, kdim, bns):
    with ops.exact_gemm():
        return _tnet_layers(net, h, B, N, kdim, bns)


def _tnet_layers(net, h, B, N, kdim, bns):
    def layer(x, lin, bn):
        sc, sh = bn_affine(bn) if bn is not None else (None, None)
        return ops.linear(x, _w2d(lin), bias=lin.bias, scale=sc, shift=sh, act=ops.ACT_RELU)
    h = layer(h, net.conv1, bns[0])
    h = layer(h, net.conv2, bns[1])
    h = layer(h, net.conv3, bns[2])
    g = ops.colmax(h, B, N)
    g = layer(g, net.fc1, bns[3])
    g = layer(g, net.fc2, bns[4])
    eye_bias = _cached(net, "fc3_bias_eye", (net.fc3.bias,),
                       lambda: (net.fc3.bias + torch.eye(kdim, device=net.fc3.bias.device).flatten()).contiguous())
    t = ops.linear(g, net.fc3.weight, bias=eye_bias)
    return t.view(B, kdim, kdim)


def transform_net_eval(net, h, B, N):
    return _tnet_common(net, h, B, N, net.k, (net.bn1, net.bn2, net.bn3, net.bn4, net.bn5))


def stn3d_eval(net, h, B, N):
    bns = (net.bn1, net.bn2, net.bn3, net.bn4, net.bn5) if net.use_bn else (None,) * 5
    return _tnet_common(net, h, B, N, net.k, bns)


def _knn_rows(rows, B, N, C, k):
    rows = rows.reshape(B * N, C)
    if C <= 64 and k <= 64:
        return ops.knn_pm(rows, B, N, k)
    return ops.knn(ops.transpose(rows.view(B, N, C).contiguous()), k)


PANEL_LAYOUT = _debug.on("panels")
_side_env = __import__("os").environ.get("LPD_SIDE_STREAM", "auto")
SIDE_STREAM = "auto" if _side_env == "auto" else (_side_env != "0")
SIDE_SMALL_POINTS = 24 * 4096


def _dev_key(device):
    return (device.type, device.index if device.index is not None else torch.cuda.current_device())


_SIDE_FORCE = __import__("threading").local()


def _side_mode(device, points=None, light_side=False):
    forced = getattr(_SIDE_FORCE, "mode", None)
    if forced is not None:
        return forced
    if SIDE_STREAM != "auto":
        return bool(SIDE_STREAM)
    if torch.cuda.is_current_stream_capturing():
        return False
    return (light_side and not _TLS.PIPELINED) or (points is not None and points <= SIDE_SMALL_POINTS)


def side_stream_report(device=None):
    if SIDE_STREAM != "auto":
        return "two streams (LPD_SIDE_STREAM=1)" if SIDE_STREAM else "one stream (LPD_SIDE_STREAM=0)"
    return ("two streams: the xyz kNN and the DG1 projection run on a second (high-priority) stream next to the per-point layers and the "
            "feature-space kNN; paths that still launch the DG1 K-agg by itself use it only up to %d points" % SIDE_SMALL_POINTS)


def _join(waiter, signaller):
    waiter.wait_stream(signaller)
    tape = ops._TLS.TAPE
    if tape is not None:
        tape.actions.append((ops.Tape.JOIN, waiter, signaller, torch.cuda.Event()))


# ... 23 lines not shown

for _reg in ("register_module_parameter_registration_hook", "register_module_buffer_registration_hook", "register_module_module_registration_hook"):
    getattr(torch.nn.modules.module, _reg)(_bump_epoch)


def invalidate(model=None):
    with _PLANS_LOCK:
        if model is None:
            _PLANS.clear()
            _SIG_TENSORS.clear()
        else:
            _PLANS.pop(model, None)
            _SIG_TENSORS.pop(model, None)
    _EPOCH[0] += 1


def _model_sig(model):
    ent = _SIG_TENSORS.get(model)
    if ent is None or ent[0] != _EPOCH[0]:
        mods = list(model.modules())
        ent = _SIG_TENSORS[model] = (_EPOCH[0], list(model.parameters()) + list(model.buffers()), mods)
    attrs = tuple((getattr(m, "eps", None), getattr(m, "use_relu", None), getattr(m, "k", None), getattr(m, "training", None)) for m in ent[2])
    return ent[0], tuple((t.data_ptr(), t._version) for t in ent[1]), attrs


def _switch_sig():
    g = globals()
    return (_morton_order(), SIDE_STREAM, getattr(_SIDE_FORCE, "mode", None), _TLS.PIPELINED, PANEL_LAYOUT, g["FUSED_FRONT"], g["FUSE_ASSIGN"], g["CONV3_P8"],
            g["KAGG_WINDOW"], EVAL_CHUNK, ops.GEMM_BF16X3, ops._EXACT.depth, ops._FAST.depth, ops.KNN_IMPL, ops.BF16_SINGLE_PRODUCT,
            ops.X3W_FORWARD, ops.X3W_IMPL, ops.X3W_BATCHED, ops.X3T_PANELS, ops.X3T_ROWS, ops.P8_IMPL, ops.KAGGW_PERMUTE, ops.EDGE_MLP_X1)


def replay_eval(model, x, eager):
    if (not REPLAY or _TLS.DEBUG_AUX is not None or ops._TLS.PROFILE is not None or ops._TLS.TAPE is not None
            or not isinstance(x, torch.Tensor) or not x.is_cuda or x.dtype != torch.float32 or x.dim() != 4
            or x.shape[0] * x.shape[2] > REPLAY_MAX_POINTS or torch.cuda.is_current_stream_capturing()
            or getattr(model, "_is_replica", False) or x.shape[1] != 1 or x.shape[3] != 3
            or getattr(model.emb_nn, "t3d", True) or getattr(model.emb_nn, "tfea", True) or getattr(model.emb_nn, "use_mFea", True)):
        return eager(x)
    stream = torch.cuda.current_stream(x.device)
    key = (tuple(x.shape), x.device.index, stream.cuda_stream)
    with _PLANS_LOCK:
        sig = (_model_sig(model), _switch_sig())
        mp = _PLANS.get(model)
        if mp is None or mp.sig != sig:
            mp = _PLANS[model] = _ModelPlans()
            mp.sig, mp.plans = sig, {}
        ent = mp.plans.get(key)
        if ent is None:
            if len(mp.plans) >= REPLAY_MAX_PLANS:
                mp.plans.pop(next(iter(mp.plans)))
            ent = _Plan()
            ent.actions, ent.keep, ent.x_in, ent.out, ent.hits, ent.lock = None, None, None, None, 0, __import__("threading").Lock()
            mp.plans[key] = ent
            return_eager = True
        else:
            return_eager = False
    if return_eager:
        return eager(x)
    if not ent.lock.acquire(blocking=False):
        return eager(x)
    try:
        if ent.actions is not None:
            return _replay(ent, x)
        return _record(ent, x, eager)
    finally:
        ent.lock.release()


def _record(ent, x, eager):
    x_in = x.detach().clone().contiguous()
    tape = ops.Tape()
    ops._TLS.TAPE = tape
    try:
        out = eager(x_in)
    finally:
        ops._TLS.TAPE = None
    ent.x_in, ent.out, ent.actions, ent.keep = x_in, out, tape.actions, tape.keep
    return out.clone()


def _replay(ent, x):
    ent.x_in.copy_(x)
    CALL, ZERO = ops.Tape.CALL, ops.Tape.ZERO
    for a in ent.actions:
        kind = a[0]
        if kind == CALL:
            rc = a[1](*a[2])
            if rc != 0:
                ent.actions = None
                ops._lib.check(rc, a[1].__name__)
        elif kind == ZERO:
            a[1].zero_()
        else:
            a[3].record(a[2])
            a[1].wait_event(a[3])
    ent.hits += 1
    return ent.out.clone()


FUSED_FRONT = _debug.on("fused-front")
_SIDE = {}
_SIDE_LOCK = __import__("threading").Lock()


def _side_stream(device):
    key = _dev_key(device) + (torch.cuda.current_stream(device).cuda_stream,)
    with _SIDE_LOCK:
        st = _SIDE.get(key)
        if st is None:
            if len(_SIDE) >= 32:
                _SIDE.pop(next(iter(_SIDE)))
            st = _SIDE[key] = torch.cuda.Stream(device=device, priority=_debug.value("side-prio", -1))
    return st


def _resident_shape(k, N, M, act):
    return k == 20 and N <= 4096 and act in (ops.ACT_NONE, ops.ACT_RELU, ops.ACT_LEAKY) and M * 512 * 4 < 2 ** 32


def _kagg_cloud_resident(idx, N, M, act):
    return _resident_shape(idx.shape[-1], N, M, act)


KAGG_WINDOW = _debug.on("kagg-window")
CONV3_P8 = _debug.on("p8")


def _kagg_windowed(idx, N, act):
    return (KAGG_WINDOW and idx.shape[-1] in (20, 32, 64) and 64 <= N <= 57344
            and act in (ops.ACT_NONE, ops.ACT_RELU, ops.ACT_LEAKY))


def kagg(P, Q, idx, N, *, scale, shift, act, slope, out, idx16w=None):
    if _kagg_cloud_resident(idx, N, P.shape[0], act):
        return ops.edge_gather_max16(P, Q, ops.pack_idx16(idx), N, scale=scale, shift=shift, act=act, slope=slope, out=out)
    if _kagg_windowed(idx, N, act):
        if idx16w is None:
            idx16w = ops.pack_idx16w(idx)
        return ops.edge_gather_maxw(P, Q, idx16w, N, scale=scale, shift=shift, act=act, slope=slope, out=out)
    return ops.edge_gather_max(P, Q, idx, N, scale=scale, shift=shift, act=act, slope=slope, out=out)


def split_mfea(x):
    rows = x.view(-1, 8)
    return rows[:, :3].contiguous(), rows


FUSE_ASSIGN = _debug.on("fuse-assign")


def lpdnet_features_eval(net, x, reorder=True, assign=None):
    mfea = getattr(net, "use_mFea", False)
    x = _check_input(x, 8) if mfea else reorder_points(_check_input(x), reorder)
    B, N = x.shape[0], x.shape[2]
    act = ops.ACT_RELU if net.use_relu else ops.ACT_LEAKY
    side_ok = PANEL_LAYOUT and N % 128 == 0 and _resident_shape(net.k, N, B * N, act)
    light = side_ok and _x1_rides(net, B * N, N)
    out = _lpdnet_features_eval_body(net, x, mfea, side_ok and _side_mode(x.device, B * N, light), assign)
    return out if assign is not None else out[:3]


def _split_planes(net, N):
    return bool(CONV3_P8 and ops.GEMM_BF16X3 and ops._EXACT.depth == 0 and N % 256 == 0 and net.conv3_lpd.weight.shape[0] % 256 == 0)


def _x1_rides(net, M, N):
    return bool(net.k == 20 and N <= 4096 and _split_planes(net, N) and ops.edge_mlp_x1_applies(M, N, 128, net.convDG2[0].weight.shape[0]))


def _lpdnet_features_eval_body(net, x, mfea, use_side, assign=None):
    B, N = x.shape[0], x.shape[2]
    M = B * N
    k = net.k
    act, slope = (ops.ACT_RELU, 0.0) if net.use_relu else (ops.ACT_LEAKY, LEAKY_SLOPE)
    if mfea:
        xyz, p = split_mfea(x)
        x = xyz.view(B, 1, N, 3)
    else:
        xyz = x.view(M, 3)
        p = xyz
    side_job = None
    if use_side:
        main, side = torch.cuda.current_stream(), _side_stream(x.device)
        _join(side, main)
        with torch.cuda.stream(side):
            idx_x = _knn_rows(xyz, B, N, 3, k)
            i16_x = ops.pack_idx16(idx_x)
        side_job = (side, idx_x, i16_x)
    knn_ws = None
    if FUSED_FRONT and not (mfea or net.t3d or net.tfea) and N % 128 == 0 and k <= 64:
        s, b = bn_affine(net.bn1_lpd)
        s2_, b2_ = bn_affine(net.bn2_lpd)
        f, knn_ws = ops.lpdnet_front(xyz, _w2d(net.conv1_lpd), s, b, _w2d(net.conv2_lpd), s2_, b2_, B, N, k, act=act, slope=slope)
    else:
        with ops.exact_gemm():
            if net.t3d:
                trans = transform_net_eval(net.t_net3d, xyz, B, N)
                p = _aligned_input(ops.apply_transform(xyz, trans, N), p, mfea)
            s, b = bn_affine(net.bn1_lpd)
            f = ops.linear(p, _w2d(net.conv1_lpd), scale=s, shift=b, act=act, slope=slope)
            s, b = bn_affine(net.bn2_lpd)
            f = ops.linear(f, _w2d(net.conv2_lpd), scale=s, shift=b, act=act, slope=slope)
            if net.tfea:
                tf = transform_net_eval(net.t_net_fea, f, B, N)
                f = ops.apply_transform(f, tf, N)
    s1, b1 = bn_affine(net.convDG1[1])
    s2, b2 = bn_affine(net.convDG2[1])
    s3, b3 = bn_affine(net.convSN1[1])
    sc, bc = bn_affine(net.bn3_lpd)
    wdg1 = split_edge_weight(net.convDG1, "cat_nc")
    pq = None
    if side_job is not None:
        main, side = torch.cuda.current_stream(), side_job[0]
        _join(side, main)
        f.record_stream(side)
        with torch.cuda.stream(side):
            pq = ops.linear(f, wdg1)
    idx_f = ops.knn_prepared(knn_ws, B, N, k) if knn_ws is not None else _knn_rows(f, B, N, 64, k)
    if pq is None:
        pq = ops.linear(f, wdg1)
    resident = _kagg_cloud_resident(idx_f, N, M, act)
    if PANEL_LAYOUT and N % 128 == 0 and (resident or _kagg_windowed(idx_f, N, act)):
        pack = ops.pack_idx16 if resident else ops.pack_idx16w
        kagg_p = ops.edge_gather_max16 if resident else ops.edge_gather_maxw
        split = resident and _split_planes(net, N)
        if split:
            cat = ops.split_panels_empty(B, N, 512, x.device)
            x1v, x2v, x3v = cat[:, :, 0:16], cat[:, :, 16:32], cat[:, :, 32:64]
        else:
            cat = ops.panels_empty(B, N, 512, x.device)
            x1v, x2v, x3v = cat[:, 0:16], cat[:, 16:32], cat[:, 32:64]
        x1_fused = split and _x1_rides(net, M, N)
        if x1_fused:
            if side_job is not None:
                main, side = torch.cuda.current_stream(), side_job[0]
                _join(main, side)
                pq.record_stream(main)
        elif side_job is not None:
            main, side = torch.cuda.current_stream(), side_job[0]
            _join(main, side)
            pq.record_stream(main)
            _join(side, main)
            for t in (idx_f, cat):
                t.record_stream(side)
            with torch.cuda.stream(side):
                kagg_p(pq[:, :128], pq[:, 128:], pack(idx_f), N, scale=s1, shift=b1, act=act, slope=slope, out=x1v)
        else:
            kagg_p(pq[:, :128], pq[:, 128:], pack(idx_f), N, scale=s1, shift=b1, act=act, slope=slope, out=x1v)
        ops.edge_mlp(pq[:, :128], pq[:, 128:], idx_f, N, s1, b1, _w2d(net.convDG2[0]), s2, b2, act=act, slope=slope, out=x2v,
                     x1_out=x1v if x1_fused else None)
        if split:
            pq3 = ops.gemm_x3t_split(x2v, split_edge_weight(net.convSN1, "cat_nc"))
        else:
            pq3 = ops.gemm(x2v, split_edge_weight(net.convSN1, "cat_nc"), b_kmajor=False, a_panels=True, out_panels=True)
        if side_job is not None:
            side, idx_x, i16_x = side_job
            main = torch.cuda.current_stream()
            _join(main, side)
            idx_x.record_stream(main)
            i16_x.record_stream(main)
        else:
            idx_x = _knn_rows(xyz, B, N, 3, k)
            i16_x = pack(idx_x)
        kagg_p(pq3[:, 0:32], pq3[:, 32:64], i16_x, N, scale=s3, shift=b3, act=act, slope=slope, out=x3v)
        if _TLS.DEBUG_AUX is not None:
            _TLS.DEBUG_AUX.update(F0=f, idx_feat=idx_f, idx_xyz=idx_x, cat=ops.split_to_rows(cat) if split else ops.panels_to_rows(cat))
        parts = None
        if split:
            if (FUSE_ASSIGN and assign is not None and assign.cluster_size == 64 and N % 64 == 0
                    and assign.feature_size == net.conv3_lpd.weight.shape[0] and net.conv3_lpd.weight.shape[0] // 256 in (1, 2, 4, 8)):
                feat, parts = ops.gemm_p8(cat, conv3_folded(net), shift=bc, act=act, slope=slope, assign_w=assign.cluster_weights)
            else:
                feat = ops.gemm_p8(cat, conv3_folded(net), shift=bc, act=act, slope=slope)
        else:
            feat = ops.gemm(cat, _w2d(net.conv3_lpd), b_kmajor=False, a_panels=True, scale=sc, shift=bc, act=act, slope=slope)
        return feat, B, N, parts
    if side_job is not None:
        _join(torch.cuda.current_stream(), side_job[0])
        pq.record_stream(torch.cuda.current_stream())
    cat = torch.empty((M, 512), dtype=torch.float32, device=x.device)
    kagg(pq[:, :128], pq[:, 128:], idx_f, N, scale=s1, shift=b1, act=act, slope=slope, out=cat[:, 0:128])
    ops.edge_mlp(pq[:, :128], pq[:, 128:], idx_f, N, s1, b1, _w2d(net.convDG2[0]), s2, b2, act=act, slope=slope,
                 out=cat[:, 128:256])
    if side_job is not None:
        side, idx_x, _ = side_job
        _join(torch.cuda.current_stream(), side)
        idx_x.record_stream(torch.cuda.current_stream())
    else:
        idx_x = _knn_rows(x.view(B * N, 3), B, N, 3, k)
    pq = ops.linear(cat[:, 128:256], split_edge_weight(net.convSN1, "cat_nc"))
    kagg(pq[:, :256], pq[:, 256:], idx_x, N, scale=s3, shift=b3, act=act, slope=slope, out=cat[:, 256:512])
    if _TLS.DEBUG_AUX is not None:
        _TLS.DEBUG_AUX.update(F0=f, idx_feat=idx_f, idx_xyz=idx_x, cat=cat)
    return ops.linear(cat, _w2d(net.conv3_lpd), scale=sc, shift=bc, act=act, slope=slope), B, N, None


def _aligned_input(xyz_t, p_all, mfea):
    return torch.cat((xyz_t, p_all[:, 3:]), dim=1).contiguous() if mfea else xyz_t


def lpdnet_origin_features_eval(net, x, reorder=True):
    mfea = getattr(net, "use_mFea", False)
    x = _check_input(x, 8) if mfea else reorder_points(_check_input(x), reorder)
    B, N = x.shape[0], x.shape[2]
    M = B * N
    k = net.k
    act, slope = (ops.ACT_RELU, 0.0) if net.use_relu else (ops.ACT_LEAKY, LEAKY_SLOPE)

    def seq(h, block):
        s, b = bn_affine(block[1])
        return ops.linear(h, _w2d(block[0]), scale=s, shift=b, act=act, slope=slope)
    if mfea:
        xyz, p = split_mfea(x)
        x = xyz.view(B, 1, N, 3)
    else:
        xyz = x.view(M, 3)
        p = xyz
    with ops.exact_gemm():
        if net.t3d:
            trans = transform_net_eval(net.t_net3d, xyz, B, N)
            p = _aligned_input(ops.apply_transform(xyz, trans, N), p, mfea)
        f = seq(seq(p, net.conv1_lpd), net.conv2_lpd)
        if net.tfea:
            tf = transform_net_eval(net.t_net_fea, f, B, N)
            f = ops.apply_transform(f, tf, N)
    idx_f = _knn_rows(f, B, N, 64, k)
    pq = ops.linear(f, split_edge_weight(net.convDG1, "cat_cd"))
    s1, b1 = bn_affine(net.convDG1[1])
    s2, b2 = bn_affine(net.convDG2[1])
    g = ops.edge_mlp(pq[:, :64], pq[:, 64:], idx_f, N, s1, b1, _w2d(net.convDG2[0]), s2, b2, act=act, slope=slope)
    idx_x = _knn_rows(x.view(B * N, 3), B, N, 3, k)
    pn = ops.linear(g, split_edge_weight(net.convSN1, "nbr"))
    s1, b1 = bn_affine(net.convSN1[1])
    s2, b2 = bn_affine(net.convSN2[1])
    h = ops.edge_mlp(pn, None, idx_x, N, s1, b1, _w2d(net.convSN2[0]), s2, b2, act=act, slope=slope)
    if _TLS.DEBUG_AUX is not None:
        _TLS.DEBUG_AUX.update(F0=f, idx_feat=idx_f, idx_xyz=idx_x)
    h = seq(seq(seq(h, net.conv3_lpd), net.conv4_lpd), net.conv5_lpd)
    return h, B, N


def pointnet_features_eval(net, x):
    x = _check_input(x)
    B, N = x.shape[0], x.shape[2]
    if N != net.num_points:
        raise ValueError(f"PointNetfeat was built for num_points={net.num_points}, got N={N} (MaxPool2d((num_points,1)))")
    M = B * N
    xyz = x.view(M, 3)
    trans = stn3d_eval(net.stn, xyz, B, N)
    p = ops.apply_transform(xyz, trans, N)

    def layer(h, conv, bn, act):
        s, b = bn_affine(bn)
        return ops.linear(h, _w2d(conv), bias=conv.bias, scale=s, shift=b, act=act)
    h = layer(p, net.conv1, net.bn1, ops.ACT_RELU)
    h = layer(h, net.conv2, net.bn2, ops.ACT_RELU)
    if net.apply_feature_trans:
        ft = stn3d_eval(net.feature_trans, h, B, N)
        h = ops.apply_transform(h, ft, N)
    h = layer(h, net.conv3, net.bn3, ops.ACT_RELU)
    h = layer(h, net.conv4, net.bn4, ops.ACT_RELU)
    h = layer(h, net.conv5, net.bn5, ops.ACT_NONE)
    return h, B, N, trans


def _head_splits(K):
    s = 1
    while s < 512 and K // (s * 2) >= 128:
        s *= 2
    return s


def _pool_splits(B, N, E):
    blocks = B * ((E + 127) // 128)
    s = 1
    while blocks * s < 1024 and N // (s * 2) >= 256:
        s *= 2
    return s


def netvlad_eval(vlad, feat, B, N, logit_parts=None):
    if N != vlad.max_samples:
        raise ValueError(f"NetVLADLoupe was built for max_samples={vlad.max_samples}, got N={N}")
    E, K = vlad.feature_size, vlad.cluster_size
    if vlad.add_batch_norm:
        s, b = bn_affine(vlad.bn1)
    else:
        s = _cached(vlad, "ones", (vlad.cluster_biases,), lambda: torch.ones_like(vlad.cluster_biases))
        b = vlad.cluster_biases
    ws = None
    if logit_parts is not None:
        a, ws = ops.softmax_affine_parts(logit_parts, s, b, colsum_rows=N)
    else:
        a = ops.gemm(feat, vlad.cluster_weights, b_kmajor=True)
        if N % 16 == 0:
            a, ws = ops.softmax_affine(a, s, b, out=a, colsum_rows=N)
        else:
            a = ops.softmax_affine(a, s, b, out=a)
    vraw = ops.pool_tn(feat.view(B, N, E), a.view(B, N, K))
    if vraw is None:
        vraw = ops.gemm(feat.view(B, N, E), a.view(B, N, K), a_kmajor=True, b_kmajor=True, splits=_pool_splits(B, N, E))
    v = ops.vlad_finalize(vraw, a.view(B, N, K), vlad.cluster_weights2.view(E, K), ws=ws)
    s, b = bn_affine(vlad.bn2)
    h = ops.gemm(v, vlad.hidden1_weights, b_kmajor=True, scale=s, shift=b, splits=_head_splits(E * K))
    if not vlad.gating:
        return h
    return gating_eval(vlad.context_gating, h)


def gating_eval(gc, h):
    if gc.add_batch_norm:
        s, b = bn_affine(gc.bn1)
        return ops.gating(h, gc.gating_weights, scale=s, shift=b)
    return ops.gating(h, gc.gating_weights, bias=gc.gating_biases)


def to_channel_major(feat, B, N):
    return ops.transpose(feat.view(B, N, feat.shape[1])).unsqueeze(-1)


def to_point_major(x4):
    B, E, N = x4.shape[0], x4.shape[1], x4.shape[2]
    return ops.transpose(x4.reshape(B, E, N).float().contiguous()).view(B * N, E), B, N
```

### lpd-net-pytorch_amd/lpdnet_hip/ops.py

```python
import ctypes
import os

import torch

from . import _debug, _lib

ACT_NONE, ACT_RELU, ACT_LEAKY, ACT_SIGMOID = 0, 1, 2, 3

class _PerThread(__import__("threading").local):
    PROFILE = None
    PROFILE_ONLY = None
    TAPE = None


class Tape:
    CALL, ZERO, JOIN = 0, 1, 2

    def __init__(self):
        self.actions = []
        self.keep = []


_TLS = _PerThread()

# ... 1 lines not shown
class _OpsModule(__import__("types").ModuleType):
    PROFILE = property(lambda self: _TLS.PROFILE, lambda self, v: setattr(_TLS, "PROFILE", v))
    PROFILE_ONLY = property(lambda self: _TLS.PROFILE_ONLY, lambda self, v: setattr(_TLS, "PROFILE_ONLY", v))


__import__("sys").modules[__name__].__class__ = _OpsModule


def _call(label, fn, *args):
    if _TLS.TAPE is not None:
        _TLS.TAPE.actions.append((Tape.CALL, fn, args))
    prof, only = _TLS.PROFILE, _TLS.PROFILE_ONLY
    if prof is None or (only is not None and not label.startswith(only)):
        rc = fn(*args)
        if rc != 0:
            _stat_ws_drop()
        _lib.check(rc, fn.__name__)
        return
    a = torch.cuda.Event(enable_timing=True)
    b = torch.cuda.Event(enable_timing=True)
    a.record()
    rc = fn(*args)
    b.record()
    if rc != 0:
        _stat_ws_drop()
    _lib.check(rc, fn.__name__)
    prof.setdefault(label, []).append((a, b))


def _ptr(t):
    if t is None:
        return None
    if _TLS.TAPE is not None:
        _TLS.TAPE.keep.append(t)
    return ctypes.c_void_p(t.data_ptr())


def _zeros(shape, dtype, device):
    t = torch.zeros(shape, dtype=dtype, device=device)
    if _TLS.TAPE is not None:
        _TLS.TAPE.actions.append((Tape.ZERO, t))
    return t


_raw_stream = getattr(torch._C, "_cuda_getCurrentRawStream", None)
_cur_device = getattr(torch._C, "_cuda_getDevice", None)


def _stream():
    if _raw_stream is not None and _cur_device is not None:
        return ctypes.c_void_p(_raw_stream(_cur_device()))
    return ctypes.c_void_p(torch.cuda.current_stream().cuda_stream)


_STAT_WS = {}
_STAT_LOCK = __import__("threading").Lock()


def _stat_ws():
    dev = _cur_device() if _cur_device is not None else torch.cuda.current_device()
    raw = _raw_stream(dev) if _raw_stream is not None else torch.cuda.current_stream().cuda_stream
    t = _STAT_WS.get((dev, raw))
    if t is None:
        n = int(_lib.load().lpd_stat_ws_bytes()) // 8
        t = torch.zeros(n, dtype=torch.float64, device=torch.device("cuda", dev))
        if torch.cuda.is_current_stream_capturing():
            keep = _TLS.__dict__.setdefault("capture_keep", [])
            keep.append(t)
            return ctypes.c_void_p(t.data_ptr())
        with _STAT_LOCK:
            t = _STAT_WS.setdefault((dev, raw), t)
    if _TLS.__dict__.get("capture_keep") and not torch.cuda.is_current_stream_capturing():
        _TLS.__dict__["capture_keep"] = []
    return ctypes.c_void_p(t.data_ptr())


def _stat_ws_drop():
    dev = _cur_device() if _cur_device is not None else torch.cuda.current_device()
    raw = _raw_stream(dev) if _raw_stream is not None else torch.cuda.current_stream().cuda_stream
    with _STAT_LOCK:
        _STAT_WS.pop((dev, raw), None)


def _req(t, name, dtype=torch.float32):
    if t is None:
        return
    if not isinstance(t, torch.Tensor):
        raise TypeError(f"{name}: expected a tensor")
    if not t.is_cuda:
        raise _lib.LpdHipError(
            f"{name}: tensor is on {t.device}; the LPD-Net HIP path runs on MI355X only (no CPU fallback)")
    if t.dtype != dtype:
        raise TypeError(f"{name}: expected {dtype}, got {t.dtype}")


def _rows(t, name):
    _req(t, name)
    if t.dim() != 2 or t.stride(1) != 1:
        raise ValueError(f"{name}: expected a 2-D tensor with contiguous rows, got shape {tuple(t.shape)} strides {t.stride()}")
    return t.stride(0)


def _vec(t, name, n):
    if t is None:
        return None
    _req(t, name)
    if t.numel() != n:
        raise ValueError(f"{name}: expected {n} elements, got {t.numel()}")
    return t.contiguous()


KNN_IMPL = _debug.value("knn-impl", 0)


def knn_workspace_floats(B, C, N, k=20):
    return int(_lib.load().lpd_knn_workspace_floats(B, C, N, k))


def knn(x_cm, k, impl=None):
    if impl is None:
        impl = KNN_IMPL
    _req(x_cm, "x")
    if x_cm.dim() != 3:
        raise ValueError("knn: expected [B,C,N]")
    x_cm = x_cm.contiguous()
    B, C, N = x_cm.shape
    idx = torch.empty((B, N, k), dtype=torch.int32, device=x_cm.device)
    ws = torch.empty((knn_workspace_floats(B, C, N),), dtype=torch.float32, device=x_cm.device)
    lib = _lib.load()
    _call(f"knn[C={C},k={k}]", lib.lpd_knn, _ptr(x_cm), B, C, N, k, _ptr(idx), _ptr(ws), impl, _stream())
    return idx


def lpdnet_front(xyz, W1, s1, b1, W2, s2, b2, B, N, k, act=ACT_NONE, slope=0.01):
    _req(xyz, "xyz")
    ldx = _rows(xyz, "xyz")
    M = xyz.shape[0]
    if M != B * N or N % 128:
        raise ValueError("lpdnet_front: rows != B*N or N % 128 != 0")
    W1 = W1.reshape(64, 3).contiguous()
    W2 = W2.reshape(64, 64).contiguous()
    f0 = torch.empty((M, 64), dtype=torch.float32, device=xyz.device)
    ws = torch.empty((knn_workspace_floats(B, 64, N),), dtype=torch.float32, device=xyz.device)
    lib = _lib.load()
    s1, b1, s2, b2 = _vec(s1, "s1", 64), _vec(b1, "b1", 64), _vec(s2, "s2", 64), _vec(b2, "b2", 64)
    _call("lpdnet_front", lib.lpd_lpdnet_front, _ptr(xyz), ldx, _ptr(W1), _ptr(s1), _ptr(b1), _ptr(W2),
          _ptr(s2), _ptr(b2), act, float(slope), _ptr(f0), B, N, k, _ptr(ws), _stream())
    return f0, ws


KNN_PM_PREPARED = 256


def knn_prepared(ws, B, N, k, impl=None):
    if impl is None:
        impl = KNN_IMPL
    idx = torch.empty((B, N, k), dtype=torch.int32, device=ws.device)
    lib = _lib.load()
    _call(f"knn[C=64,k={k}]", lib.lpd_knn_pm, None, 64, B, 64, N, k, _ptr(idx), _ptr(ws), impl | KNN_PM_PREPARED, _stream())
    return idx


def knn_pm(x_pm, B, N, k, impl=None):
    if impl is None:
        impl = KNN_IMPL
    ld = _rows(x_pm, "x_pm")
    M, C = x_pm.shape
    if M != B * N:
        raise ValueError("knn_pm: rows != B*N")
    idx = torch.empty((B, N, k), dtype=torch.int32, device=x_pm.device)
    ws = torch.empty((knn_workspace_floats(B, C, N),), dtype=torch.float32, device=x_pm.device)
    lib = _lib.load()
    _call(f"knn[C={C},k={k}]", lib.lpd_knn_pm, _ptr(x_pm), ld, B, C, N, k, _ptr(idx), _ptr(ws), impl, _stream())
    return idx


GEMM_BF16X3 = __import__("os").environ.get("LPD_GEMM_FP32", "0") != "1"


class _ExactState(__import__("threading").local):
    depth = 0


_EXACT = _ExactState()


_tfx = _debug.value("train-fwd-x3", "auto")
TRAIN_FWD_BF16X3 = "auto" if _tfx == "auto" else (_tfx == "1")
TRAIN_FWD_X3_MIN_CLOUDS = 32


class _FastState(__import__("threading").local):
    depth = 0


_FAST = _FastState()


BF16_SINGLE_PRODUCT = _debug.on("bf16-x1", False)


class bf16_gemm:

    def __enter__(self):
        self.on = BF16_SINGLE_PRODUCT
        if self.on:
            _FAST.depth += 1

    def __exit__(self, *exc):
        if self.on:
            _FAST.depth -= 1
        return False


class exact_gemm:

    def __enter__(self):
        _EXACT.depth += 1

    def __exit__(self, *exc):
        _EXACT.depth -= 1
        return False


class train_forward_gemm(exact_gemm):

    def __init__(self, clouds=None):
        self.clouds = clouds

    def __enter__(self):
        x3 = (self.clouds is not None and self.clouds >= TRAIN_FWD_X3_MIN_CLOUDS) if TRAIN_FWD_BF16X3 == "auto" else bool(TRAIN_FWD_BF16X3)
        self.on = not x3
        if self.on:
            super().__enter__()

    def __exit__(self, *exc):
        if self.on:
            super().__exit__(*exc)
        return False


_FRAG_CACHE = {}
_FRAG_LOCK = __import__("threading").Lock()
X3W_FORWARD = _debug.on("x3w-fwd")
X3W_IMPL = _debug.value("x3w-impl", 0)
X3W_BATCHED = _debug.on("x3w-batched")
X3T_PANELS = _debug.on("x3t")
X3T_ROWS = _debug.on("x3t-rows")


def _weight_frags(B2, b_kmajor, N, K):
    base = B2._base if B2._base is not None else B2
    cacheable = isinstance(base, torch.nn.Parameter) or bool(getattr(base, "_lpd_stable", False))
    key = (B2.data_ptr(), base._version, tuple(B2.shape), B2.stride(0), bool(b_kmajor)) if cacheable else None
    if cacheable:
        with _FRAG_LOCK:
            hit = _FRAG_CACHE.get(key)
        if hit is not None:
            consumer_sync(hit[2], hit[0])
            return hit[0]
    lib = _lib.load()
    frags = torch.empty((int(lib.lpd_gemm_prep_b_bytes(N, K)),), dtype=torch.uint8, device=B2.device)
    _call("gemm_prep_b", lib.lpd_gemm_prep_b, _ptr(B2), B2.stride(0), int(bool(b_kmajor)), N, K, _ptr(frags), _stream())
    if cacheable:
        mark = producer_mark()
        with _FRAG_LOCK:
            if len(_FRAG_CACHE) > 256:
                _FRAG_CACHE.clear()
            _FRAG_CACHE[key] = (frags, base, mark)
    return frags


def producer_mark():
    if torch.cuda.is_current_stream_capturing():
        return None
    ev = torch.cuda.Event()
    ev.record()
    return (_stream().value, ev)


def consumer_sync(mark, *tensors):
    if mark is not None and mark[0] != _stream().value:
        cur = torch.cuda.current_stream()
        cur.wait_event(mark[1])
        for t in tensors:
            if isinstance(t, torch.Tensor):
                t.record_stream(cur)


def gemm(A, B, *, a_kmajor=False, b_kmajor=True, bias=None, scale=None, shift=None, act=ACT_NONE, slope=0.01,
         out=None, splits=1, accumulate=False, exact=False, a_panels=False, out_panels=False, out_bf16=False, a_affine=None):
    a16 = isinstance(A, torch.Tensor) and A.dtype == torch.bfloat16
    _req(A, "A", torch.bfloat16 if a16 else torch.float32)
    _req(B, "B")
    if a_panels or out_panels:
        return _gemm_panels(A, B, a_kmajor, b_kmajor, bias, scale, shift, act, slope, out, accumulate, exact, a_panels, out_panels)
    batched = A.dim() == 3
    if batched:
        if B.dim() != 3 or A.shape[0] != B.shape[0]:
            raise ValueError("gemm: batched A needs batched B with the same batch")
        nb = A.shape[0]
        A2, B2 = A[0], B[0]
        sA, sB = A.stride(0), B.stride(0)
    else:
        nb, A2, B2, sA, sB = 1, A, B, 0, 0
    if a16 and (A2.dim() != 2 or A2.stride(1) != 1):
        raise ValueError("gemm: bf16 A needs contiguous rows")
    lda, ldb = A2.stride(0) if a16 else _rows(A2, "A"), _rows(B2, "B")
    M, K = (A2.shape[1], A2.shape[0]) if a_kmajor else (A2.shape[0], A2.shape[1])
    Kb, N = (B2.shape[0], B2.shape[1]) if b_kmajor else (B2.shape[1], B2.shape[0])
    if K != Kb:
        raise ValueError(f"gemm: inner dims differ ({K} vs {Kb})")
    if out is None:
        out = torch.empty((nb, M, N) if batched else (M, N), dtype=torch.bfloat16 if out_bf16 else torch.float32, device=A.device)
    _req(out, "out", torch.bfloat16 if out_bf16 else torch.float32)
    O2 = out[0] if batched else out
    if O2.dim() != 2 or O2.stride(1) != 1:
        raise ValueError("gemm: out needs contiguous rows")
    ldc = O2.stride(0)
    if O2.shape[0] != M or O2.shape[1] != N:
        raise ValueError("gemm: out has the wrong shape")
    sC = out.stride(0) if batched else 0
    ws = None
    if splits > 1:
        ws = torch.empty((nb * splits * M * N,), dtype=torch.float32, device=A.device)
    bias, scale, shift = _vec(bias, "bias", N), _vec(scale, "scale", N), _vec(shift, "shift", N)
    lib = _lib.load()
# ... 423 lines not shown
            raise ValueError("edge_mlp: split out must be a [2, B, CO/8, N, 8] view")
        if not (GEMM_BF16X3 and not exact and _EXACT.depth == 0):
            raise ValueError("edge_mlp: split output is written by the split-bf16 kernel only")
        s1, b1 = _vec(s1, "s1", CM), _vec(b1, "b1", CM)
        s2, b2 = _vec(s2, "s2", CO), _vec(b2, "b2", CO)
        lib = _lib.load()
        if x1_out is not None:
            if (not _is_split(x1_out) or tuple(x1_out.shape) != tuple(out.shape) or tuple(x1_out.stride()) != tuple(out.stride())
                    or not edge_mlp_x1_applies(M, N, CM, CO, exact)):
                raise ValueError("edge_mlp: x1_out must be split planes with the shape and strides of `out` (128 -> 128, M % 32 == 0, N % 64 == 0)")
            _call(f"edge_mlpx3+x1[{CM}->{CO}]", lib.lpd_edge_mlp_x1_bf16x3s, _ptr(P), ldp, _ptr(Q), ldq, _ptr(idx), _ptr(s1), _ptr(b1), _ptr(W2),
                  _ptr(s2), _ptr(b2), _ptr(out[0]), _ptr(x1_out[0]), out.stride(0), M, N, k, act, float(slope), out.stride(1), out.stride(2) // 8,
                  _stream())
            return out
        _call(f"edge_mlpx3[{CM}->{CO}]", lib.lpd_edge_mlp_bf16x3s, _ptr(P), ldp, _ptr(Q), ldq, _ptr(idx), _ptr(s1), _ptr(b1), _ptr(W2), _ptr(s2),
              _ptr(b2), _ptr(out[0]), out.stride(0), M, N, CM, CO, k, act, float(slope), out.stride(1), out.stride(2) // 8, _stream())
        return out
    if x1_out is not None:
        raise ValueError("edge_mlp: x1_out is written by the split-plane form only")
    if out.dim() == 4:
        if not _is_panels(out) or out.shape[1] * 8 != CO or out.shape[0] * out.shape[2] != M or out.shape[2] != N:
            raise ValueError("edge_mlp: cloud-panel out must be a [B, CO/8, N, 8] view")
        _req(out, "out")
        ldo, out_cloud = 8, out.stride(0)
    else:
        ldo = _rows(out, "out")
    s1, b1 = _vec(s1, "s1", CM), _vec(b1, "b1", CM)
    s2, b2 = _vec(s2, "s2", CO), _vec(b2, "b2", CO)
    lib = _lib.load()
    x3 = GEMM_BF16X3 and not exact and _EXACT.depth == 0
    _call(f"edge_mlp{'x3' if x3 else ''}[{CM}->{CO}]", lib.lpd_edge_mlp_bf16x3 if x3 else lib.lpd_edge_mlp, _ptr(P), ldp, _ptr(Q), ldq, _ptr(idx), _ptr(s1), _ptr(b1), _ptr(W2), _ptr(s2),
                                _ptr(b2), _ptr(out), ldo, M, N, CM, CO, k, act, float(slope), out_cloud, _panel_ld(out), _stream())
    return out


def transpose(x):
    _req(x, "x")
    if x.dim() != 3:
        raise ValueError("transpose: expected a 3-D tensor")
    x = x.contiguous()
    nb, R, C = x.shape
    out = torch.empty((nb, C, R), dtype=torch.float32, device=x.device)
    lib = _lib.load()
    _call("transpose", lib.lpd_transpose, _ptr(x), _ptr(out), nb, R, C, C, R, R * C, R * C, _stream())
    return out


def softmax_affine(x, scale=None, shift=None, out=None, colsum_rows=None):
    _rows(x, "x")
    x = x.contiguous()
    rows, n = x.shape
    if out is None:
        out = torch.empty_like(x)
    scale, shift = _vec(scale, "scale", n), _vec(shift, "shift", n)
    lib = _lib.load()
    if colsum_rows is None:
        _call("softmax_affine", lib.lpd_softmax_affine, _ptr(x), _ptr(out), rows, n, _ptr(scale), _ptr(shift), 0, None, 0, None, _stream())
        return out
    if colsum_rows % 16 or rows % colsum_rows:
        raise ValueError("softmax_affine: colsum_rows must be a multiple of 16 that divides the row count")
    ws = torch.empty((rows // colsum_rows, 2 * n), dtype=torch.float32, device=x.device)
    part = torch.empty((rows // 16, 64), dtype=torch.float32, device=x.device)
    _call("softmax_affine", lib.lpd_softmax_affine, _ptr(x), _ptr(out), rows, n, _ptr(scale), _ptr(shift), colsum_rows, _ptr(ws), 2 * n,
          _ptr(part), _stream())
    return out, ws


def softmax_affine_parts(parts, scale=None, shift=None, colsum_rows=None):
    _req(parts, "parts")
    if parts.dim() != 3 or parts.shape[2] != 64 or not parts[0].is_contiguous():
        raise ValueError("softmax_affine_parts: expected [P, rows, 64]")
    P, rows, n = parts.shape
    if colsum_rows is None or colsum_rows % 64 or rows % colsum_rows:
        raise ValueError("softmax_affine_parts: colsum_rows must be a multiple of 64 that divides the row count")
    out = torch.empty((rows, n), dtype=torch.float32, device=parts.device)
    scale, shift = _vec(scale, "scale", n), _vec(shift, "shift", n)
    ws = torch.empty((rows // colsum_rows, 2 * n), dtype=torch.float32, device=parts.device)
    part = torch.empty((rows // 64, 64), dtype=torch.float32, device=parts.device)
    lib = _lib.load()
    _call("softmax_affine", lib.lpd_softmax_affine_parts, _ptr(parts), P, parts.stride(0), _ptr(out), rows, _ptr(scale), _ptr(shift),
          colsum_rows, _ptr(ws), 2 * n, _ptr(part), _stream())
    return out, ws


def vlad_finalize(vraw, act, cw2, out=None, aux=None, ws=None):
    _req(vraw, "vraw"), _req(act, "act"), _req(cw2, "cw2")
    vraw, act, cw2 = vraw.contiguous(), act.contiguous(), cw2.contiguous()
    B, F, KC = vraw.shape
    N = act.shape[1]
    if out is None:
        out = torch.empty((B, F * KC), dtype=torch.float32, device=vraw.device)
    a1 = a2 = a3 = None
    if aux is not None:
        a1 = torch.empty((B, KC), dtype=torch.float32, device=vraw.device)
        a2 = torch.empty((B, KC), dtype=torch.float32, device=vraw.device)
        a3 = torch.empty((B,), dtype=torch.float32, device=vraw.device)
        aux.update(asum=a1, inv_c=a2, inv_g=a3)
    ready = ws is not None
    if ready:
        if ws.shape != (B, 2 * KC) or not ws.is_contiguous():
            raise ValueError("vlad_finalize: ws must be the [B, 2*KC] workspace of softmax_affine(colsum_rows=N)")
    else:
        ws = torch.empty((B, 2 * KC), dtype=torch.float32, device=vraw.device)
    part = torch.empty((B, 16 + (F + 63) // 64, KC), dtype=torch.float32, device=vraw.device)
    lib = _lib.load()
    _call("vlad_finalize", lib.lpd_vlad_finalize, _ptr(vraw), _ptr(act), _ptr(cw2), _ptr(out), _ptr(ws), _ptr(part), _ptr(a1), _ptr(a2),
          _ptr(a3), B, N, F, KC, int(ready), _stream())
    return out


def colmax(x, B, N):
    ldi = _rows(x, "x")
    C = x.shape[1]
    if x.shape[0] != B * N:
        raise ValueError("colmax: rows != B*N")
    out = torch.empty((B, C), dtype=torch.float32, device=x.device)
    lib = _lib.load()
    _call("colmax", lib.lpd_colmax, _ptr(x), ldi, _ptr(out), B, N, C, _stream())
    return out


def gating(h, Wg, bias=None, scale=None, shift=None):
    ldh, ldw = _rows(h, "h"), _rows(Wg, "Wg")
    B, D = h.shape
    if Wg.shape != (D, D):
        raise ValueError("gating: Wg must be [D, D]")
    out = torch.empty((B, D), dtype=torch.float32, device=h.device)
    bias, scale, shift = _vec(bias, "bias", D), _vec(scale, "scale", D), _vec(shift, "shift", D)
    lib = _lib.load()
    _call("gating", lib.lpd_gating, _ptr(h), ldh, _ptr(Wg), ldw, _ptr(bias), _ptr(scale), _ptr(shift), _ptr(out), D, B, D, _stream())
    return out


def mul(a, b):
    _req(a, "a"), _req(b, "b")
    a, b = a.contiguous(), b.contiguous()
    out = torch.empty_like(a)
    lib = _lib.load()
    _call("mul", lib.lpd_mul, _ptr(a), _ptr(b), _ptr(out), a.numel(), _stream())
    return out


def morton_sort(x, want_perm=False):
    _req(x, "x")
    shape = x.shape
    x3 = x.reshape(-1, shape[-2], 3).contiguous()
    B, N = x3.shape[0], x3.shape[1]
    out = torch.empty_like(x3)
    perm = torch.empty((B, N), dtype=torch.int32, device=x.device) if want_perm else None
    lib = _lib.load()
    _call("morton_sort", lib.lpd_morton_sort, _ptr(x3), _ptr(out), _ptr(perm), B, N, _stream())
    out = out.view(shape)
    return (out, perm) if want_perm else out


def local_features(xyz_rows, idx, B, N, *, candidates=None, columns=range(10), copy_xyz=False, want_k=False, out=None):
    _req(xyz_rows, "xyz_rows")
    _req(idx, "idx", torch.int32)
    ldx = _rows(xyz_rows, "xyz_rows")
    if xyz_rows.shape[0] != B * N or xyz_rows.shape[1] < 3:
        raise ValueError("local_features: xyz_rows must be [B*N, >=3]")
    if idx.dim() != 3 or idx.shape[0] != B or idx.shape[1] != N:
        raise ValueError(f"local_features: idx must be [B,N,K], got {tuple(idx.shape)}")
    idx = idx.contiguous()
    K = idx.shape[2]
    sel = 0
    for c in columns:
        if not 0 <= int(c) < 10 or sel >> int(c) & 1:
            raise ValueError(f"local_features: columns must be distinct and in 0..9, got {list(columns)}")
        sel |= 1 << int(c)
    if list(columns) != sorted(columns):
        raise ValueError("local_features: columns are written in ascending order; pass them sorted")
    width = (3 if copy_xyz else 0) + bin(sel).count("1")
    if out is None:
        out = torch.empty((B * N, width), dtype=torch.float32, device=xyz_rows.device)
    ldo = _rows(out, "out")
    if out.shape[0] != B * N:
        raise ValueError("local_features: out must have B*N rows")
    cand = None
    ncand = 0
    if candidates is not None:
        ncand = len(candidates)
        cand = (ctypes.c_int32 * max(1, ncand))(*[int(c) for c in candidates])
    kopt = torch.empty((B * N,), dtype=torch.int32, device=xyz_rows.device) if want_k else None
    lib = _lib.load()
    _call(f"local_features[k={K}]", lib.lpd_local_features, _ptr(xyz_rows), ldx, _ptr(idx), B, N, K, cand, ncand, sel, int(bool(copy_xyz)),
          _ptr(out), ldo, _ptr(kopt), _stream())
    return (out, kopt) if want_k else out


SUBMAP_MIN_N, SUBMAP_MAX_N, SUBMAP_MAX_POINTS = 128, 4096, 1 << 20


def check_submap_lengths(lengths, rows=None, what="make_submaps"):
    total = 0
    for b, n in enumerate(lengths):
        n = int(n)
        if n < 1:
            raise ValueError(f"{what}: cloud {b} has {n} points (offsets must ascend and no scan may be empty)")
        if n > SUBMAP_MAX_POINTS:
            raise ValueError(f"{what}: cloud {b} has {n} points; at most 2^20 per cloud")
        total += n
    if rows is not None and total > rows:
        raise ValueError(f"{what}: the clouds hold {total} rows, the points tensor {rows}")
    return total


def _make_submaps(points, offsets, B, N, normalize, want_counts, out):
    dev = points.device
    if out is None:
        out = torch.empty((B, N, 3), dtype=torch.float32, device=dev)
    info = torch.empty((B, 4), dtype=torch.int32, device=dev)
    xform = torch.empty((B, 4), dtype=torch.float32, device=dev)
    counts = torch.empty((B, N), dtype=torch.int32, device=dev) if want_counts else None
    lib = _lib.load()
    _call(f"make_submaps[n={N}]", lib.lpd_make_submaps, _ptr(points), points.stride(0), _ptr(offsets), B, N, int(bool(normalize)), _ptr(out),
          _ptr(info), _ptr(xform), _ptr(counts), _stream())
    return out, info, xform, counts


def make_submaps(points, offsets, B, N, normalize=True, want_counts=False, out=None):
    _req(points, "points")
    _req(offsets, "offsets", torch.int32)
    B, N = int(B), int(N)
    if not SUBMAP_MIN_N <= N <= SUBMAP_MAX_N:
        raise ValueError(f"make_submaps: N={N} outside {SUBMAP_MIN_N} .. {SUBMAP_MAX_N}")
    ld = _rows(points, "points")
    if points.shape[1] < 3 or ld < 3:
        raise ValueError(f"make_submaps: points must be [rows, >=3], got {tuple(points.shape)}")
    if B < 1 or offsets.dim() != 1 or offsets.numel() != B + 1:
        raise ValueError(f"make_submaps: offsets must hold B+1 = {B + 1} entries, got {tuple(offsets.shape)}")
    offsets = offsets.contiguous()
    host = offsets.cpu().tolist()
    if host[0] < 0:
        raise ValueError(f"make_submaps: offsets[0] = {host[0]} < 0")
    check_submap_lengths([host[b + 1] - host[b] for b in range(B)])
    if host[B] > points.shape[0]:
        raise ValueError(f"make_submaps: offsets end at row {host[B]}, the points tensor has {points.shape[0]}")
    if out is not None:
        _req(out, "out")
        if out.numel() != B * N * 3 or not out.is_contiguous():
            raise ValueError(f"make_submaps: out must be a contiguous [B,N,3] tensor, got {tuple(out.shape)}")
    return _make_submaps(points, offsets, B, N, normalize, want_counts, out)


TUPLE_MAX_ITEMS, TUPLE_MAX_SAMPLES, TUPLE_MAX_LISTS, TUPLE_MAX_ROWS = 262144, 4096, 64, 65535


def sample_items(off, idx, T, lists, extra, m, invert, seed):
    _req(off, "off", torch.int32)
    _req(idx, "idx", torch.int32)
    _req(lists, "lists", torch.int32)
    _req(extra, "extra", torch.int32)
    T, m = int(T), int(m)
    if off is None or idx is None or lists is None:
        raise TypeError("sample_items: off, idx and lists are tensors (an empty lists tensor is [R, 0])")
    if off.dim() != 1 or off.numel() < 1 or idx.dim() != 1:
        raise ValueError(f"sample_items: off must be [n_lists+1] and idx [nnz], got {tuple(off.shape)} and {tuple(idx.shape)}")
    if lists.dim() != 2 or not 1 <= lists.shape[0] <= TUPLE_MAX_ROWS or lists.shape[1] > TUPLE_MAX_LISTS:
        raise ValueError(f"sample_items: lists must be [R, L] with 1 <= R <= {TUPLE_MAX_ROWS}, L <= {TUPLE_MAX_LISTS}, got {tuple(lists.shape)}")
    R, L = lists.shape
    X = 0
    if extra is not None:
        if extra.dim() != 2 or extra.shape[0] != R or extra.shape[1] > TUPLE_MAX_LISTS:
            raise ValueError(f"sample_items: extra must be [R, X] with R = {R}, X <= {TUPLE_MAX_LISTS}, got {tuple(extra.shape)}")
        X = extra.shape[1]
        extra = extra.contiguous() if X else None
    if not 1 <= T <= TUPLE_MAX_ITEMS:
        raise ValueError(f"sample_items: T={T} outside 1 .. {TUPLE_MAX_ITEMS}")
    if not 1 <= m <= TUPLE_MAX_SAMPLES:
        raise ValueError(f"sample_items: m={m} outside 1 .. {TUPLE_MAX_SAMPLES}")
    if invert not in (0, 1, False, True):
        raise ValueError(f"sample_items: invert={invert!r} (0 or 1)")
    off, idx = off.contiguous(), idx.contiguous()
    lists = lists.contiguous() if L else None
    out = torch.empty((R, m), dtype=torch.int32, device=off.device)
    count = torch.empty((R,), dtype=torch.int32, device=off.device)
    lib = _lib.load()
    _call("sample_items", lib.lpd_sample_items, _ptr(off), _ptr(idx) if idx.numel() else None, off.numel() - 1, idx.numel(), T, _ptr(lists), L,
          _ptr(extra), X, R, int(invert), m, int(seed) & 0xFFFFFFFFFFFFFFFF, _ptr(out), _ptr(count), _stream())
    return out, count


def gather_tuples(table, items, rot=None, sigma=0.0, clip=0.05, seed=0, out=None):
    _req(table, "table")
    _req(items, "items", torch.int32)
    _req(rot, "rot")
    if table.dim() != 3 or table.shape[2] != 3 or not table.is_contiguous() or table.shape[0] < 1 or table.shape[1] < 1:
        raise ValueError(f"gather_tuples: table must be a contiguous [T, N, 3] tensor, got {tuple(table.shape)}")
    T, N = table.shape[:2]
    if items.dim() != 1 or not 1 <= items.numel() <= TUPLE_MAX_ROWS:
        raise ValueError(f"gather_tuples: items must be [B] with 1 <= B <= {TUPLE_MAX_ROWS}, got {tuple(items.shape)}")
    items = items.contiguous()
    B = items.numel()
    if rot is not None:
        if tuple(rot.shape) != (B, 2):
            raise ValueError(f"gather_tuples: rot must be [B, 2] = ({B}, 2), got {tuple(rot.shape)}")
        rot = rot.contiguous()
    sigma, clip = float(sigma), float(clip)
    if not sigma >= 0.0 or not clip > 0.0:
        raise ValueError(f"gather_tuples: sigma={sigma} clip={clip} (sigma >= 0, clip > 0)")
    if out is None:
        out = torch.empty((B, N, 3), dtype=torch.float32, device=table.device)
    else:
        _req(out, "out")
        if out.numel() != B * N * 3 or not out.is_contiguous():
# ... 1074 lines not shown
```

Before: 20210 descriptors/s.

## Fuse xyz kNN prep into Morton sort and emit packed int16 neighbor lists

The Morton sort kernel now also writes the xyz kNN workspace (squared norms, padded points, tile centroids, radii), so the xyz kNN skips its own prep launch. The best-first kNN kernel writes the packed 16-bit neighbor layout directly when k=20, which removes both the int32 index write and the separate pack_idx16 launch on the eval path. This adds more work and register pressure to the sort kernel, plus new layout code paths that must match the existing packer exactly.

```diff
diff --git a/include/lpd_hip.h b/include/lpd_hip.h
--- a/include/lpd_hip.h
+++ b/include/lpd_hip.h
@@ -26,6 +26,9 @@
 int lpd_knn_pm(const float* x_pm, int ld, int B, int C, int N, int k, int32_t* idx, float* ws, int impl, void* stream);
 #define LPD_KNN_PM_PREPARED 256
 int lpd_knn_pm_layout(int B, int C, int N, int k, float* ws, float** xx, float** xp, void** xb, float** tiles);
+int lpd_knn_pm16_fused(int C, int N, int k, int impl);
+long long lpd_idx16_offset(long long m, int s);
+int lpd_knn_pm16(const float* x_pm, int ld, int B, int C, int N, int k, int32_t* idx, uint16_t* idx16, float* ws, int impl, void* stream);
 
 int lpd_lpdnet_front(const float* xyz, int ldx, const float* W1, const float* s1, const float* b1, const float* W2, const float* s2,
                      const float* b2, int act, float slope, float* F0, int B, int N, int k, float* knn_ws, void* stream);
@@ -146,6 +149,8 @@
 int lpd_f64_to_f32(const double* in, float* out, long long n, void* stream);
 
 int lpd_morton_sort(const float* xyz, float* out, int32_t* perm, int B, int N, void* stream);
+int lpd_morton_sort_knn_applies(int N, int k);
+int lpd_morton_sort_knn(const float* xyz, float* out, int32_t* perm, int B, int N, int k, float* knn_ws, void* stream);
 
 int lpd_local_features(const float* xyz, int ldx, const int32_t* idx, int B, int N, int K, const int32_t* cand, int ncand, unsigned sel,
                        int copy_xyz, float* out, int ldo, int32_t* kopt, void* stream);
diff --git a/lpd-net-pytorch_amd/csrc/lpd_knn.hip b/lpd-net-pytorch_amd/csrc/lpd_knn.hip
--- a/lpd-net-pytorch_amd/csrc/lpd_knn.hip
+++ b/lpd-net-pytorch_amd/csrc/lpd_knn.hip
@@ -1131,13 +1131,28 @@
     KNN_PLACE(0, 1, 2, 3, 16, 17, 18, 19, 4, 5, 6, 7, 8, 9, 10, 11, 12, 13, 14, 15);
 }
 
+__host__ __device__ inline size_t knn_idx16_offset(size_t m, int s)
+{
+    const size_t blk = (m >> 5) * 1280, p = m & 31;
+    return blk + (s < 16 ? (size_t)(s >> 3) * 512 + p * 16 + (size_t)(s & 7) * 2 : 1024 + p * 8 + (size_t)(s - 16) * 2);
+}
+__device__ __forceinline__ void knn7_store_idx16(uint16_t* __restrict__ idx16, size_t m0, int p, const int (&o)[20])
+{
+    unsigned char* base = reinterpret_cast<unsigned char*>(idx16);
+    const size_t m = m0 + (size_t)p;
+    auto pk = [](int a, int b) { return (uint32_t)((a << 4) & 0xffff) | ((uint32_t)b << 20); };
+    *reinterpret_cast<uint4*>(base + knn_idx16_offset(m, 0)) = make_uint4(pk(o[0], o[1]), pk(o[2], o[3]), pk(o[4], o[5]), pk(o[6], o[7]));
+    *reinterpret_cast<uint4*>(base + knn_idx16_offset(m, 8)) = make_uint4(pk(o[8], o[9]), pk(o[10], o[11]), pk(o[12], o[13]), pk(o[14], o[15]));
+    *reinterpret_cast<uint2*>(base + knn_idx16_offset(m, 16)) = make_uint2(pk(o[16], o[17]), pk(o[18], o[19]));
+}
+
 template <int CP, int KMAX, int WAVES, bool ONFLY, bool FULLT = false, int SPLIT = 1>
 __global__ __launch_bounds__(WAVES * SPLIT * 64, ((SPLIT > 1 && CP == 2) ? 3 : Knn7Cfg<CP, KMAX, ONFLY>::WAVES_PER_SIMD)) void knn7_kernel(const float* __restrict__ xp, const float* __restrict__ xx,
                                                              const float* __restrict__ cenp, const float* __restrict__ cnorm,
                                                              const float* __restrict__ rad, const float* __restrict__ txmax,
                                                              int32_t* __restrict__ idx, const int32_t* __restrict__ order,
                                                              int N, int k, int nt, int C, int blocks_per_cloud, int dbg,
-                                                             const uint16_t* __restrict__ ubq)
+                                                             const uint16_t* __restrict__ ubq, uint16_t* __restrict__ idx16)
 {
     extern __shared__ __attribute__((aligned(16))) unsigned char smem7[];
     if constexpr (FULLT) dbg = 0;
@@ -1622,7 +1637,7 @@
                 pos[w2] = 0;
             }
             int32_t* out = idx + ((size_t)b * N + q) * k;
-            for (int s = 0; s < k; ++s) {
+            auto next = [&]() {
                 int bw = 0;
                 float bvv = hv[0];
                 int bii = hi[0];
@@ -1633,7 +1648,6 @@
                     bvv = better ? hv[w2] : bvv;
                     bii = better ? hi[w2] : bii;
                 }
-                out[s] = bii;
 #pragma unroll
                 for (int w2 = 0; w2 < SPLIT; ++w2) {
                     if (bw == w2) {
@@ -1644,7 +1658,20 @@
                         hi[w2] = more ? __float_as_int(mbase[w2 * WSTRIDE + IOFF + pp]) : 0x7fffffff;
                     }
                 }
-            }
+                return bii;
+            };
+            static_assert(KMAX == 20, "the packed block holds lists of 20");
+            if (idx16) {
+                int o[KMAX];
+#pragma unroll
+                for (int s = 0; s < KMAX; ++s) o[s] = next();
+                knn7_store_idx16(idx16, (size_t)b * N + q0, col, o);
+                if (idx) {
+#pragma unroll
+                    for (int s = 0; s < KMAX; ++s) out[s] = o[s];
+                }
+            } else
+                for (int s = 0; s < k; ++s) out[s] = next();
         }
         return;
     }
@@ -1662,6 +1689,28 @@
         const int* bi = mi + (lane + 32) * KMAX;
         int pa = 0, pb = 0;
         int32_t* out = idx + ((size_t)b * N + q) * k;
+        if constexpr (KMAX == 20) {
+            if (idx16) {
+                int o[KMAX];
+#pragma unroll
+                for (int s = 0; s < KMAX; ++s) {
+                    const float va = av[pa], vb2 = bv[pb];
+                    const int ia = ai[pa], ib = bi[pb];
+                    const bool take_a = (va > vb2) || (va == vb2 && ia < ib);
+                    o[s] = take_a ? ia : ib;
+                    pa += take_a ? 1 : 0;
+                    pb += take_a ? 0 : 1;
+                    pa = min(pa, KMAX - 1);
+                    pb = min(pb, KMAX - 1);
+                }
+                knn7_store_idx16(idx16, (size_t)b * N + q0, col, o);
+                if (idx) {
+#pragma unroll
+                    for (int s = 0; s < KMAX; ++s) out[s] = o[s];
+                }
+                return;
+            }
+        }
         for (int s = 0; s < k; ++s) {
             bool take_a;
             if (pa >= KMAX) take_a = false;
@@ -1704,6 +1753,16 @@
     return n;
 }
 
+inline bool knn7_branchy()
+{
+    static const bool branchy = lpd_debug("knn-fullt", 1) == 0;
+    return branchy;
+}
+inline bool knn7_packs16(int N, int k, int dbg)
+{
+    static const bool on = lpd_debug("knn-pack16", 1) != 0;
+    return on && k == 20 && N % 32 == 0 && !knn7_branchy() && !dbg;
+}
 inline bool knn7_tight()
 {
     static const bool tight = lpd_debug("knn-pre", 1) != 0;
@@ -1720,7 +1779,7 @@
 
 template <int CP, int KMAX, bool ONFLY>
 int knn7_launch(const float* x, const float* xx, int32_t* idx, int B, int C, int N, int k, hipStream_t stream, int dbg = 0, bool xb_ready = false,
-                bool stats_ready = false)
+                bool stats_ready = false, uint16_t* idx16 = nullptr)
 {
     using L = Knn7Cfg<CP, KMAX, ONFLY>;
     static_assert(L::WAVE >= L::MERGE, "merge region must fit the wave's LDS region");
@@ -1755,7 +1814,8 @@
             LPD_CHECK_LAUNCH("lpd_knn(low-precision bounds)");
         }
     }
-    static const bool branchy = lpd_debug("knn-fullt", 1) == 0;
+    const bool branchy = knn7_branchy();
+    uint16_t* const out16 = (idx16 && knn7_packs16(N, k, dbg)) ? idx16 : nullptr;
     constexpr int KNN7_SPLIT = 4;
     constexpr bool split_built = KMAX <= 20 && !(ONFLY && CP == 32);
     static const int split_env = lpd_debug("knn-split", -1);
@@ -1781,7 +1841,7 @@
             (void)hipFuncSetAttribute((const void*)kern, hipFuncAttributeMaxDynamicSharedMemorySize, (int)lds);
             hipLaunchKernelGGL(kern, dim3(bpc * B), dim3(threads), lds, stream, (const float*)xp, xx, (const float*)cenp,
                                (const float*)cnorm, (const float*)rad, (const float*)txmax, idx, (const int32_t*)(use_order ? order : nullptr),
-                               N, k, nt, C, bpc, dbg, (const uint16_t*)ubq);
+                               N, k, nt, C, bpc, dbg, (const uint16_t*)ubq, KMAX == 20 ? out16 : (uint16_t*)nullptr);
         };
         if constexpr (split_built) {
             if (split) {
@@ -1802,12 +1862,13 @@
 constexpr int KNN7_MAXN = 65536;
 inline bool knn7_applies(int C, int N, int k) { return C <= 64 && k <= 64 && N <= KNN7_MAXN; }
 inline int knn7_dispatch(const float* x, const float* xx, int32_t* idx, int B, int C, int N, int k, hipStream_t stream, int dbg, bool xb_ready = false,
-                         bool stats_ready = false)
+                         bool stats_ready = false, uint16_t* idx16 = nullptr)
 {
     const bool small = k <= 20 && N <= KNN7_MAXT * 32;
-    if (C <= 4) return k <= 20 ? knn7_launch<2, 20, true>(x, xx, idx, B, C, N, k, stream, dbg) : knn7_launch<2, 64, true>(x, xx, idx, B, C, N, k, stream, dbg);
-    if (small) return knn7_launch<32, 20, false>(x, xx, idx, B, C, N, k, stream, dbg, xb_ready, stats_ready);
-    return k <= 20 ? knn7_launch<32, 20, true>(x, xx, idx, B, C, N, k, stream, dbg, xb_ready, stats_ready)
+    if (C <= 4) return k <= 20 ? knn7_launch<2, 20, true>(x, xx, idx, B, C, N, k, stream, dbg, false, stats_ready, idx16)
+                               : knn7_launch<2, 64, true>(x, xx, idx, B, C, N, k, stream, dbg, false, stats_ready);
+    if (small) return knn7_launch<32, 20, false>(x, xx, idx, B, C, N, k, stream, dbg, xb_ready, stats_ready, idx16);
+    return k <= 20 ? knn7_launch<32, 20, true>(x, xx, idx, B, C, N, k, stream, dbg, xb_ready, stats_ready, idx16)
                    : knn7_launch<32, 64, true>(x, xx, idx, B, C, N, k, stream, dbg, xb_ready, stats_ready);
 }
 
@@ -1920,10 +1981,47 @@
     return LPD_OK;
 }
 
+namespace {
+inline bool knn_pm_packs16(int C, int N, int k, int impl)
+{
+    impl &= ~LPD_KNN_PM_PREPARED;
+    return ((impl == 0 && KNN7_DEFAULT) || impl == 6) && C <= 64 && knn7_applies(C, N, k) && knn7_packs16(N, k, 0);
+}
+int knn_pm_run(const float* x_pm, int ld, int B, int C, int N, int k, int32_t* idx, uint16_t* idx16, float* ws, int impl, void* stream_);
+}
+
 extern "C" int lpd_knn_pm(const float* x_pm, int ld, int B, int C, int N, int k, int32_t* idx, float* ws, int impl, void* stream_)
 {
+    LPD_CHECK_ARG(idx, "lpd_knn_pm: null pointer");
+    return knn_pm_run(x_pm, ld, B, C, N, k, idx, nullptr, ws, impl, stream_);
+}
+
+extern "C" int lpd_knn_pm16_fused(int C, int N, int k, int impl) { return knn_pm_packs16(C, N, k, impl) ? 1 : 0; }
+
+extern "C" long long lpd_idx16_offset(long long m, int s)
+{
+    if (m < 0 || s < 0 || s >= 20) return -1;
+    return (long long)knn_idx16_offset((size_t)m, s);
+}
+
+extern "C" int lpd_knn_pm16(const float* x_pm, int ld, int B, int C, int N, int k, int32_t* idx, uint16_t* idx16, float* ws, int impl,
+                            void* stream_)
+{
+    LPD_CHECK_ARG(idx16 && ((uintptr_t)idx16 & 15) == 0, "lpd_knn_pm16: idx16 must be a 16-byte aligned pointer");
+    LPD_CHECK_ARG(k == 20 && N > 0 && N % 32 == 0, "lpd_knn_pm16: the packed lists are built for k = 20 and whole 32-point tiles (k=%d N=%d)", k, N);
+    const bool fused = knn_pm_packs16(C, N, k, impl);
+    LPD_CHECK_ARG(idx || fused, "lpd_knn_pm16: these sizes pack in a launch of their own and need the int32 lists (lpd_knn_pm16_fused)");
+    LPD_CHECK_ARG(!idx || ((uintptr_t)idx & 15) == 0, "lpd_knn_pm16: idx must be 16-byte aligned");
+    const int rc = knn_pm_run(x_pm, ld, B, C, N, k, idx, fused ? idx16 : nullptr, ws, impl, stream_);
+    if (rc != LPD_OK || fused) return rc;
+    return lpd_pack_idx16(idx, idx16, (long long)B * N, k, stream_);
+}
+
+namespace {
+int knn_pm_run(const float* x_pm, int ld, int B, int C, int N, int k, int32_t* idx, uint16_t* idx16, float* ws, int impl, void* stream_)
+{
     hipStream_t stream = (hipStream_t)stream_;
-    LPD_CHECK_ARG((x_pm || (impl & LPD_KNN_PM_PREPARED)) && idx && ws, "lpd_knn_pm: null pointer");
+    LPD_CHECK_ARG((x_pm || (impl & LPD_KNN_PM_PREPARED)) && (idx || idx16) && ws, "lpd_knn_pm: null pointer");
     LPD_CHECK_ARG(B > 0 && C > 0 && N > 0 && ld >= C, "lpd_knn_pm: bad dims B=%d C=%d N=%d ld=%d", B, C, N, ld);
     LPD_CHECK_ARG(k > 0 && k <= N, "lpd_knn_pm: need 0 < k <= N (k=%d N=%d)", k, N);
     LPD_CHECK_ARG(C <= 64 && k <= 64, "lpd_knn_pm: built for C <= 64, k <= 64 (got C=%d k=%d); use lpd_knn on the channel-major tensor", C, k);
@@ -1935,7 +2033,7 @@
     LPD_CHECK_ARG(impl == 0 || impl == 4 || impl == 5 || impl == 6, "lpd_knn_pm: impl=%d (0 product; 4 / 6 force the ascending / best-first kernel; 5 statistics)", impl);
     const bool best_first = ((impl == 0 && KNN7_DEFAULT) || (impl == 5 || impl == 6)) && knn7_applies(C, N, k);
     const bool xb_ready = knn_pm_wants_xb(C, N, k, impl) && (prepped || ld % 4 == 0);
-    LPD_CHECK_ARG(!prepped || C == 64, "lpd_knn_pm: prepared operands are a 64-channel affair (C=%d)", C);
+    LPD_CHECK_ARG(!prepped || C == 64 || (C == 3 && N % 32 == 0), "lpd_knn_pm: prepared operands come with 64 channels, or 3 and whole tiles (C=%d N=%d)", C, N);
     if (prepped) {  }
     else if (C <= 4) hipLaunchKernelGGL(knn_prep_pm_kernel<2>, dim3((unsigned)((M + 255) / 256)), dim3(256), 0, stream, x_pm, ld, ws, xp, C, M);
     else if (C == 64 && ld % 4 == 0) {
@@ -1943,7 +2041,8 @@
                            xb_ready ? knn7_xb_of(ws, B, N) : (__bf16*)nullptr, M, N, (N + 31) / 32);
     } else hipLaunchKernelGGL(knn_prep_pm_kernel<32>, dim3((unsigned)((M + 255) / 256)), dim3(256), 0, stream, x_pm, ld, ws, xp, C, M);
     LPD_CHECK_LAUNCH("lpd_knn_pm(prep)");
-    if (best_first) return knn7_dispatch(nullptr, ws, idx, B, C, N, k, stream, impl == 5, xb_ready, prepped);
+    if (best_first) return knn7_dispatch(nullptr, ws, idx, B, C, N, k, stream, impl == 5, xb_ready, prepped, idx16);
     if (C <= 4) return knn3_dispatch_k<2>(nullptr, ws, idx, B, C, N, k, stream);
     return knn3_dispatch_k<32>(nullptr, ws, idx, B, C, N, k, stream);
 }
+}
diff --git a/lpd-net-pytorch_amd/csrc/lpd_morton.hip b/lpd-net-pytorch_amd/csrc/lpd_morton.hip
--- a/lpd-net-pytorch_amd/csrc/lpd_morton.hip
+++ b/lpd-net-pytorch_amd/csrc/lpd_morton.hip
@@ -19,9 +19,18 @@
     return (lower == up) ? mn : mx;
 }
 
-template <int E, int T = 1024>
+struct MortonWs {
+    float* xx;
+    float* xp;
+    float* cenp;
+    float* cnorm;
+    float* rad;
+    float* txmax;
+};
+
+template <int E, int T = 1024, bool WS = false>
 __global__ __launch_bounds__(T) void morton_sort_kernel(const float* __restrict__ xyz, float* __restrict__ out,
-                                                         int32_t* __restrict__ perm, int N)
+                                                         int32_t* __restrict__ perm, int N, MortonWs ws = MortonWs())
 {
     constexpr int NP = T * E;
     constexpr int IB = NP == 1024 ? 10 : NP == 2048 ? 11 : NP == 4096 ? 12 : NP == 8192 ? 13 : 14;
@@ -108,26 +117,99 @@
         }
     }
     float* o = out + (size_t)b * N * 3;
+    float px[E], py[E], pz[E];
 #pragma unroll
     for (int e = 0; e < E; ++e) {
         const int r = tid * E + e;
+        px[e] = py[e] = pz[e] = 0.0f;
         if (r < N) {
             const uint32_t src = v[e] & ((1u << IB) - 1u);
-            o[r * 3 + 0] = p[src * 3 + 0];
-            o[r * 3 + 1] = p[src * 3 + 1];
-            o[r * 3 + 2] = p[src * 3 + 2];
+            o[r * 3 + 0] = px[e] = p[src * 3 + 0];
+            o[r * 3 + 1] = py[e] = p[src * 3 + 1];
+            o[r * 3 + 2] = pz[e] = p[src * 3 + 2];
             if (perm) perm[(size_t)b * N + r] = (int32_t)src;
         }
     }
+    if constexpr (WS) {
+        static_assert(E <= 16 && 32 % E == 0, "a tile inside one wave");
+        constexpr int TL = 32 / E;
+        const int lane = tid & 63;
+        const int tl0 = lane & ~(TL - 1);
+        const int r0 = tid * E;
+        const bool live = r0 < N;
+        float sq[E];
+#pragma unroll
+        for (int e = 0; e < E; ++e) {
+            sq[e] = __fadd_rn(__fadd_rn(__fmul_rn(px[e], px[e]), __fmul_rn(py[e], py[e])), __fmul_rn(pz[e], pz[e]));
+            if (live) {
+                ws.xx[(size_t)b * N + r0 + e] = sq[e];
+                *reinterpret_cast<float4*>(ws.xp + ((size_t)b * N + r0 + e) * 4) = make_float4(px[e], pz[e], py[e], 0.0f);
+            }
+        }
+        float sx = 0.f, sy = 0.f, sz = 0.f;
+#pragma unroll
+        for (int i = 0; i < 32; ++i) {
+            sx += __shfl(px[i % E], tl0 + i / E, 64);
+            sy += __shfl(py[i % E], tl0 + i / E, 64);
+            sz += __shfl(pz[i % E], tl0 + i / E, 64);
+        }
+        const float cnt = (float)min(32, N - (r0 & ~31));
+        const float c0 = sx / cnt, c1 = sz / cnt, c2 = sy / cnt, c3 = 0.0f / cnt;
+        float d2 = 0.f, nx = 0.f;
+        bool bad = false;
+#pragma unroll
+        for (int e = 0; e < E; ++e) {
+            const float dx = px[e] - c0, dz = pz[e] - c1, dy = py[e] - c2, d0 = 0.0f - c3;
+            float t = fmaf(dx, dx, 0.f);
+            t = fmaf(dz, dz, t);
+            t = fmaf(dy, dy, t);
+            t = fmaf(d0, d0, t);
+            d2 = fmaxf(d2, t);
+            nx = fmaxf(nx, sq[e]);
+            bad = bad || !(fabsf(sq[e]) <= 3.0e38f);
+        }
+        int badi = bad ? 1 : 0;
+#pragma unroll
+        for (int m = TL >> 1; m >= 1; m >>= 1) {
+            d2 = fmaxf(d2, __shfl_xor(d2, m, 64));
+            nx = fmaxf(nx, __shfl_xor(nx, m, 64));
+            badi |= __shfl_xor(badi, m, 64);
+        }
+        if (live && lane == tl0) {
+            const int nt = N >> 5;
+            const size_t t = (size_t)b * nt + (r0 >> 5);
+            *reinterpret_cast<float4*>(ws.cenp + t * 4) = make_float4(c0, c1, c2, c3);
+            ws.cnorm[t] = __fadd_rn(__fadd_rn(fmaf(c0, c0, 0.f), fmaf(c2, c2, 0.f)), __fadd_rn(fmaf(c1, c1, 0.f), fmaf(c3, c3, 0.f)));
+            ws.rad[t] = sqrtf(d2) * 1.0001f + 1e-30f;
+            ws.txmax[t] = badi ? INFINITY : nx;
+        }
+    }
 }
 
 template <int E, int T = 1024>
-void morton_launch(const float* xyz, float* out, int32_t* perm, int B, int N, hipStream_t stream)
+void morton_launch(const float* xyz, float* out, int32_t* perm, int B, int N, hipStream_t stream, const MortonWs* ws = nullptr)
 {
     const size_t lds = (size_t)E * T * sizeof(uint32_t);
-    auto kern = morton_sort_kernel<E, T>;
+    if (ws) {
+        auto kern = morton_sort_kernel<E, T, true>;
+        (void)hipFuncSetAttribute((const void*)kern, hipFuncAttributeMaxDynamicSharedMemorySize, (int)lds);
+        hipLaunchKernelGGL(kern, dim3(B), dim3(T), lds, stream, xyz, out, perm, N, *ws);
+        return;
+    }
+    auto kern = morton_sort_kernel<E, T, false>;
     (void)hipFuncSetAttribute((const void*)kern, hipFuncAttributeMaxDynamicSharedMemorySize, (int)lds);
-    hipLaunchKernelGGL(kern, dim3(B), dim3(T), lds, stream, xyz, out, perm, N);
+    hipLaunchKernelGGL(kern, dim3(B), dim3(T), lds, stream, xyz, out, perm, N, MortonWs());
+}
+
+int morton_dispatch(const float* xyz, float* out, int32_t* perm, int B, int N, hipStream_t stream, const MortonWs* ws)
+{
+    if (N <= 1024) morton_launch<1>(xyz, out, perm, B, N, stream, ws);
+    else if (N <= 2048) morton_launch<2>(xyz, out, perm, B, N, stream, ws);
+    else if (N <= 4096) morton_launch<4>(xyz, out, perm, B, N, stream, ws);
+    else if (N <= 8192) morton_launch<8>(xyz, out, perm, B, N, stream, ws);
+    else morton_launch<16>(xyz, out, perm, B, N, stream, ws);
+    LPD_CHECK_LAUNCH("lpd_morton_sort");
+    return LPD_OK;
 }
 
 }
@@ -141,11 +223,38 @@
         lpd_set_error("lpd_morton_sort: N=%d > 16384 unsupported", N);
         return LPD_ERR_UNSUPPORTED;
     }
-    if (N <= 1024) morton_launch<1>(xyz, out, perm, B, N, stream);
-    else if (N <= 2048) morton_launch<2>(xyz, out, perm, B, N, stream);
-    else if (N <= 4096) morton_launch<4>(xyz, out, perm, B, N, stream);
-    else if (N <= 8192) morton_launch<8>(xyz, out, perm, B, N, stream);
-    else morton_launch<16>(xyz, out, perm, B, N, stream);
-    LPD_CHECK_LAUNCH("lpd_morton_sort");
-    return LPD_OK;
-}
+    return morton_dispatch(xyz, out, perm, B, N, stream, nullptr);
+}
+
+extern "C" int lpd_morton_sort_knn_applies(int N, int k)
+{
+    static const bool on = lpd_debug("sort-knn", 1) != 0;
+    if (!on || N % 32 != 0 || N < 64 || N > 16384 || k <= 0 || k > 64 || k > N) return 0;
+    float dummy[4];
+    float *xx = nullptr, *xp = nullptr, *tiles = nullptr;
+    void* xb = nullptr;
+    return lpd_knn_pm_layout(1, 3, N, k, dummy, &xx, &xp, &xb, &tiles) == LPD_OK && tiles != nullptr;
+}
+
+extern "C" int lpd_morton_sort_knn(const float* xyz, float* out, int32_t* perm, int B, int N, int k, float* knn_ws, void* stream_)
+{
+    hipStream_t stream = (hipStream_t)stream_;
+    LPD_CHECK_ARG(xyz && out && knn_ws && B > 0 && N > 0, "lpd_morton_sort_knn: bad arguments");
+    LPD_CHECK_ARG(xyz != out, "lpd_morton_sort_knn: in-place reordering is not supported");
+    LPD_CHECK_ARG(((uintptr_t)knn_ws & 15) == 0, "lpd_morton_sort_knn: knn_ws must be 16-byte aligned");
+    if (!lpd_morton_sort_knn_applies(N, k)) {
+        lpd_set_error("lpd_morton_sort_knn: built for N %% 32 == 0, 64 <= N <= 16384 and the best-first search (N=%d k=%d)", N, k);
+        return LPD_ERR_UNSUPPORTED;
+    }
+    MortonWs ws;
+    float* tiles = nullptr;
+    void* xb = nullptr;
+    const int rc = lpd_knn_pm_layout(B, 3, N, k, knn_ws, &ws.xx, &ws.xp, &xb, &tiles);
+    if (rc != LPD_OK) return rc;
+    const size_t nbt = (size_t)B * (N / 32);
+    ws.cenp = tiles;
+    ws.cnorm = tiles + nbt * 4;
+    ws.rad = ws.cnorm + nbt;
+    ws.txmax = ws.rad + nbt;
+    return morton_dispatch(xyz, out, perm, B, N, stream, &ws);
+}
diff --git a/lpd-net-pytorch_amd/lpdnet_hip/_lib.py b/lpd-net-pytorch_amd/lpdnet_hip/_lib.py
--- a/lpd-net-pytorch_amd/lpdnet_hip/_lib.py
+++ b/lpd-net-pytorch_amd/lpdnet_hip/_lib.py
@@ -52,6 +52,9 @@
     "lpd_knn_pm_layout": [_c_int, _c_int, _c_int, _c_int, _c_p, _c_p, _c_p, _c_p, _c_p],
     "lpd_lpdnet_front": [_c_p, _c_int, _c_p, _c_p, _c_p, _c_p, _c_p, _c_p, _c_int, _c_f, _c_p, _c_int, _c_int, _c_int, _c_p, _c_p],
     "lpd_knn_pm": [_c_p, _c_int, _c_int, _c_int, _c_int, _c_int, _c_p, _c_p, _c_int, _c_p],
+    "lpd_knn_pm16_fused": [_c_int, _c_int, _c_int, _c_int],
+    "lpd_idx16_offset": [_c_ll, _c_int],
+    "lpd_knn_pm16": [_c_p, _c_int, _c_int, _c_int, _c_int, _c_int, _c_p, _c_p, _c_p, _c_int, _c_p],
     "lpd_knn_workspace_floats": [_c_int, _c_int, _c_int, _c_int],
     "lpd_edge_gather_max": [_c_p, _c_int, _c_p, _c_int, _c_p, _c_p, _c_int, _c_p, _c_p, _c_int, _c_int, _c_int,
                             _c_int, _c_int, _c_f, _c_p],
@@ -81,6 +84,8 @@
     "lpd_mul": [_c_p, _c_p, _c_p, _c_ll, _c_p],
     "lpd_gating": [_c_p, _c_int, _c_p, _c_int, _c_p, _c_p, _c_p, _c_p, _c_int, _c_int, _c_int, _c_p],
     "lpd_morton_sort": [_c_p, _c_p, _c_p, _c_int, _c_int, _c_p],
+    "lpd_morton_sort_knn_applies": [_c_int, _c_int],
+    "lpd_morton_sort_knn": [_c_p, _c_p, _c_p, _c_int, _c_int, _c_int, _c_p, _c_p],
     "lpd_local_features": [_c_p, _c_int, _c_p, _c_int, _c_int, _c_int, _c_p, _c_int, ctypes.c_uint, _c_int, _c_p, _c_int, _c_p, _c_p],
     "lpd_make_submaps": [_c_p, _c_int, _c_p, _c_int, _c_int, _c_int, _c_p, _c_p, _c_p, _c_p, _c_p],
     "lpd_sample_items": [_c_p, _c_p, _c_int, _c_int, _c_int, _c_p, _c_int, _c_p, _c_int, _c_int, _c_int, _c_int, ctypes.c_ulonglong, _c_p, _c_p,
@@ -155,7 +160,7 @@
     "lpd_metric_loss": [_c_p, _c_ll, _c_p, _c_ll, _c_ll, _c_p, _c_ll, _c_ll, _c_p, _c_ll, _c_int, _c_int, _c_int,
                         _c_int, _c_f, _c_f, _c_int, _c_int, _c_int, _c_int, _c_p, _c_p, _c_p, _c_p, _c_p, _c_p, _c_p],
 }
-_RESTYPES = {"lpd_last_error": ctypes.c_char_p, "lpd_stat_ws_bytes": ctypes.c_longlong, "lpd_knn_workspace_floats": ctypes.c_longlong,
+_RESTYPES = {"lpd_last_error": ctypes.c_char_p, "lpd_stat_ws_bytes": ctypes.c_longlong, "lpd_knn_workspace_floats": ctypes.c_longlong, "lpd_idx16_offset": ctypes.c_longlong,
              "lpd_gemm_prep_b_bytes": ctypes.c_longlong, "lpd_gemm_tn_bf16_ws_floats": ctypes.c_longlong, "lpd_gemm_tn_ws_floats": ctypes.c_longlong,
              "lpd_gemm_tn_act_ws_floats": ctypes.c_longlong,
              "lpd_edge_dw_sel_bf16_ws_bytes": ctypes.c_longlong, "lpd_road_planes_workspace_bytes": ctypes.c_longlong}
diff --git a/lpd-net-pytorch_amd/lpdnet_hip/engine.py b/lpd-net-pytorch_amd/lpdnet_hip/engine.py
--- a/lpd-net-pytorch_amd/lpdnet_hip/engine.py
+++ b/lpd-net-pytorch_amd/lpdnet_hip/engine.py
@@ -40,6 +40,12 @@
     if reorder and _morton_order() and 64 <= x.shape[2] <= MORTON_MAX_POINTS:
         return ops.morton_sort(x)
     return x
+
+
+def reorder_points_knn(x, reorder, k):
+    if reorder and _morton_order() and 64 <= x.shape[2] <= MORTON_MAX_POINTS and ops.morton_sort_knn_applies(x.shape[2], k):
+        return ops.morton_sort_knn(x, k)
+    return reorder_points(x, reorder), None
 
 
 _CACHES = __import__("weakref").WeakKeyDictionary()
@@ -369,12 +375,12 @@
 
 def lpdnet_features_eval(net, x, reorder=True, assign=None):
     mfea = getattr(net, "use_mFea", False)
-    x = _check_input(x, 8) if mfea else reorder_points(_check_input(x), reorder)
+    x, xyz_ws = (_check_input(x, 8), None) if mfea else reorder_points_knn(_check_input(x), reorder, net.k)
     B, N = x.shape[0], x.shape[2]
     act = ops.ACT_RELU if net.use_relu else ops.ACT_LEAKY
     side_ok = PANEL_LAYOUT and N % 128 == 0 and _resident_shape(net.k, N, B * N, act)
     light = side_ok and _x1_rides(net, B * N, N)
-    out = _lpdnet_features_eval_body(net, x, mfea, side_ok and _side_mode(x.device, B * N, light), assign)
+    out = _lpdnet_features_eval_body(net, x, mfea, side_ok and _side_mode(x.device, B * N, light), assign, xyz_ws)
     return out if assign is not None else out[:3]
 
 
@@ -386,7 +392,7 @@
     return bool(net.k == 20 and N <= 4096 and _split_planes(net, N) and ops.edge_mlp_x1_applies(M, N, 128, net.convDG2[0].weight.shape[0]))
 
 
-def _lpdnet_features_eval_body(net, x, mfea, use_side, assign=None):
+def _lpdnet_features_eval_body(net, x, mfea, use_side, assign=None, xyz_ws=None):
     B, N = x.shape[0], x.shape[2]
     M = B * N
     k = net.k
@@ -397,13 +403,23 @@
     else:
         xyz = x.view(M, 3)
         p = xyz
+    xyz16 = PANEL_LAYOUT and N % 128 == 0 and _resident_shape(k, N, M, act) and ops.knn_pm16_fused(3, N, k)
+
+    def xyz_graph():
+        if xyz16:
+            return ops.knn_pm16(None if xyz_ws is not None else xyz.reshape(M, 3), B, N, k, want_idx=_TLS.DEBUG_AUX is not None, ws=xyz_ws)
+        return (ops.knn_prepared(xyz_ws, B, N, k, C=3) if xyz_ws is not None else _knn_rows(xyz, B, N, 3, k)), None
+
     side_job = None
     if use_side:
         main, side = torch.cuda.current_stream(), _side_stream(x.device)
         _join(side, main)
+        if xyz_ws is not None:
+            xyz_ws.record_stream(side)
         with torch.cuda.stream(side):
-            idx_x = _knn_rows(xyz, B, N, 3, k)
-            i16_x = ops.pack_idx16(idx_x)
+            idx_x, i16_x = xyz_graph()
+            if i16_x is None:
+                i16_x = ops.pack_idx16(idx_x)
         side_job = (side, idx_x, i16_x)
     knn_ws = None
     if FUSED_FRONT and not (mfea or net.t3d or net.tfea) and N % 128 == 0 and k <= 64:
@@ -475,11 +491,13 @@
             side, idx_x, i16_x = side_job
             main = torch.cuda.current_stream()
             _join(main, side)
-            idx_x.record_stream(main)
+            if idx_x is not None:
+                idx_x.record_stream(main)
             i16_x.record_stream(main)
         else:
-            idx_x = _knn_rows(xyz, B, N, 3, k)
-            i16_x = pack(idx_x)
+            idx_x, i16_x = xyz_graph()
+            if i16_x is None:
+                i16_x = pack(idx_x)
         kagg_p(pq3[:, 0:32], pq3[:, 32:64], i16_x, N, scale=s3, shift=b3, act=act, slope=slope, out=x3v)
         if _TLS.DEBUG_AUX is not None:
             _TLS.DEBUG_AUX.update(F0=f, idx_feat=idx_f, idx_xyz=idx_x, cat=ops.split_to_rows(cat) if split else ops.panels_to_rows(cat))
@@ -505,7 +523,7 @@
         _join(torch.cuda.current_stream(), side)
         idx_x.record_stream(torch.cuda.current_stream())
     else:
-        idx_x = _knn_rows(x.view(B * N, 3), B, N, 3, k)
+        idx_x = xyz_graph()[0]
     pq = ops.linear(cat[:, 128:256], split_edge_weight(net.convSN1, "cat_nc"))
     kagg(pq[:, :256], pq[:, 256:], idx_x, N, scale=s3, shift=b3, act=act, slope=slope, out=cat[:, 256:512])
     if _TLS.DEBUG_AUX is not None:
@@ -519,7 +537,7 @@
 
 def lpdnet_origin_features_eval(net, x, reorder=True):
     mfea = getattr(net, "use_mFea", False)
-    x = _check_input(x, 8) if mfea else reorder_points(_check_input(x), reorder)
+    x, xyz_ws = (_check_input(x, 8), None) if mfea else reorder_points_knn(_check_input(x), reorder, net.k)
     B, N = x.shape[0], x.shape[2]
     M = B * N
     k = net.k
@@ -547,7 +565,7 @@
     s1, b1 = bn_affine(net.convDG1[1])
     s2, b2 = bn_affine(net.convDG2[1])
     g = ops.edge_mlp(pq[:, :64], pq[:, 64:], idx_f, N, s1, b1, _w2d(net.convDG2[0]), s2, b2, act=act, slope=slope)
-    idx_x = _knn_rows(x.view(B * N, 3), B, N, 3, k)
+    idx_x = ops.knn_prepared(xyz_ws, B, N, k, C=3) if xyz_ws is not None else _knn_rows(x.view(B * N, 3), B, N, 3, k)
     pn = ops.linear(g, split_edge_weight(net.convSN1, "nbr"))
     s1, b1 = bn_affine(net.convSN1[1])
     s2, b2 = bn_affine(net.convSN2[1])
diff --git a/lpd-net-pytorch_amd/lpdnet_hip/ops.py b/lpd-net-pytorch_amd/lpdnet_hip/ops.py
--- a/lpd-net-pytorch_amd/lpdnet_hip/ops.py
+++ b/lpd-net-pytorch_amd/lpdnet_hip/ops.py
@@ -177,12 +177,12 @@
 KNN_PM_PREPARED = 256
 
 
-def knn_prepared(ws, B, N, k, impl=None):
+def knn_prepared(ws, B, N, k, impl=None, C=64):
     if impl is None:
         impl = KNN_IMPL
     idx = torch.empty((B, N, k), dtype=torch.int32, device=ws.device)
     lib = _lib.load()
-    _call(f"knn[C=64,k={k}]", lib.lpd_knn_pm, None, 64, B, 64, N, k, _ptr(idx), _ptr(ws), impl | KNN_PM_PREPARED, _stream())
+    _call(f"knn[C={C},k={k}]", lib.lpd_knn_pm, None, C, B, C, N, k, _ptr(idx), _ptr(ws), impl | KNN_PM_PREPARED, _stream())
     return idx
 
 
@@ -198,6 +198,33 @@
     lib = _lib.load()
     _call(f"knn[C={C},k={k}]", lib.lpd_knn_pm, _ptr(x_pm), ld, B, C, N, k, _ptr(idx), _ptr(ws), impl, _stream())
     return idx
+
+
+def knn_pm16_fused(C, N, k, impl=None):
+    return bool(k == 20 and N % 32 == 0 and _lib.load().lpd_knn_pm16_fused(C, N, k, KNN_IMPL if impl is None else impl))
+
+
+def knn_pm16(x_pm, B, N, k, want_idx=True, impl=None, ws=None, C=3):
+    if impl is None:
+        impl = KNN_IMPL
+    if x_pm is None:
+        if ws is None:
+            raise ValueError("knn_pm16: prepared operands need their workspace")
+        ld, M, dev = C, B * N, ws.device
+        impl |= KNN_PM_PREPARED
+    else:
+        ld = _rows(x_pm, "x_pm")
+        M, C = x_pm.shape
+        dev = x_pm.device
+        ws = torch.empty((knn_workspace_floats(B, C, N),), dtype=torch.float32, device=dev)
+    if M != B * N or k != 20 or N % 32:
+        raise ValueError("knn_pm16: rows != B*N, k != 20 or N % 32 != 0")
+    lib = _lib.load()
+    want_idx = bool(want_idx) or not lib.lpd_knn_pm16_fused(C, N, k, impl)
+    idx = torch.empty((B, N, k), dtype=torch.int32, device=dev) if want_idx else None
+    idx16 = torch.empty((M, k), dtype=torch.int16, device=dev)
+    _call(f"knn[C={C},k={k}]", lib.lpd_knn_pm16, _ptr(x_pm), ld, B, C, N, k, _ptr(idx), _ptr(idx16), _ptr(ws), impl, _stream())
+    return idx, idx16
 
 
 GEMM_BF16X3 = __import__("os").environ.get("LPD_GEMM_FP32", "0") != "1"
@@ -927,6 +954,24 @@
     _call("morton_sort", lib.lpd_morton_sort, _ptr(x3), _ptr(out), _ptr(perm), B, N, _stream())
     out = out.view(shape)
     return (out, perm) if want_perm else out
+
+
+def morton_sort_knn_applies(N, k):
+    return bool(_lib.load().lpd_morton_sort_knn_applies(int(N), int(k)))
+
+
+def morton_sort_knn(x, k, want_perm=False):
+    _req(x, "x")
+    shape = x.shape
+    x3 = x.reshape(-1, shape[-2], 3).contiguous()
+    B, N = x3.shape[0], x3.shape[1]
+    out = torch.empty_like(x3)
+    perm = torch.empty((B, N), dtype=torch.int32, device=x.device) if want_perm else None
+    ws = torch.empty((knn_workspace_floats(B, 3, N, k),), dtype=torch.float32, device=x.device)
+    lib = _lib.load()
+    _call("morton_sort", lib.lpd_morton_sort_knn, _ptr(x3), _ptr(out), _ptr(perm), B, N, k, _ptr(ws), _stream())
+    out = out.view(shape)
+    return (out, ws, perm) if want_perm else (out, ws)
 
 
 def local_features(xyz_rows, idx, B, N, *, candidates=None, columns=range(10), copy_xyz=False, want_k=False, out=None):
```

Result: faster. 20600 descriptors/s (median of 6 runs) (+1.9%).
